# enordber/pepr

Measured on AMD Instinct MI355X. Metric: M site-lnL/sec (WAG+G4 full-tree likelihood evaluations x alignment patterns); the gene-trees/sec half of BASELINE.json's metric is search.gene_trees_per_sec, higher is better.
Workload: dtype f64

## Files before the change

pepr_amd/csrc/api.cpp:

```cpp
#include <algorithm>
#include <cstdlib>
#include <cstring>
#include <memory>
#include <new>
#include <thread>

#include "../../include/peprml.h"
#include "api_types.hpp"

using namespace pml;

static thread_local std::string g_err;

static std::mutex g_fp_mu; static unsigned g_fp_seen[16]; static int g_fp_n = 0;
void pml_fpguard::note(unsigned v) {
    v &= ~0x3Fu;
    std::lock_guard<std::mutex> lk(g_fp_mu);
    for (int i = 0; i < g_fp_n; ++i) if (g_fp_seen[i] == v) return;
    if (g_fp_n < 16) g_fp_seen[g_fp_n++] = v;
}

extern "C" {

const char *pml_version(void) { return "peprml 0.2 (gfx950)"; }
// ... 104 lines not shown
    try { return (expr); }                                                                     \
    catch (const std::bad_alloc &) { return b->owner->c.fail(PML_ENOMEM, "host allocation failed"); } \
    catch (const std::exception &e) { return b->owner->c.fail(PML_EINVAL, e.what()); }

int pml_batch_score(pml_batch *b, double *lnl) {
    if (!b || !lnl) return PML_EINVAL;
    pml_fpguard fpg;
    LOCKED(b);
    GUARD(b->b.score(std::vector<char>(), lnl));
}
int pml_batch_score_stored(pml_batch *b, double *lnl) {
    if (!b || !lnl) return PML_EINVAL;
    pml_fpguard fpg;
    LOCKED(b);
    GUARD(b->b.score(std::vector<char>(), lnl, true));
}
int pml_batch_site_lnl(pml_batch *b, int g, double *out) {
    if (!b || !out || g < 0 || g >= (int)b->b.genes.size()) return PML_EINVAL;
    pml_fpguard fpg;
    LOCKED(b);
    GUARD(b->b.site_lnl(g, out));
}
int pml_batch_set_alpha(pml_batch *b, int g, double alpha) {
    if (!b || g >= (int)b->b.genes.size() || !(alpha > 0)) return PML_EINVAL;
    pml_fpguard fpg;
    LOCKED(b);
    if (g < 0) for (int i = 0; i < (int)b->b.genes.size(); ++i) b->b.set_alpha(i, alpha);
    else b->b.set_alpha(g, alpha);
    return PML_OK;
}
int pml_batch_root_derivs(pml_batch *b, double *lnl, double *d1, double *d2) {
    if (!b || !lnl || !d1 || !d2) return PML_EINVAL;
    pml_fpguard fpg;
    LOCKED(b);
    GUARD(b->b.root_derivs(lnl, d1, d2));
}
int pml_batch_optimize(pml_batch *b, const pml_search_opts *opts, double *lnl, double *alpha) {
    if (!b || !lnl) return PML_EINVAL;
    pml_fpguard fpg;
    LOCKED(b);
    const bool oa = opts ? opts->optimize_alpha != 0 : true;
    const double eps = (opts && opts->epsilon > 0) ? opts->epsilon : 1e-4;
    int rc;
    try { rc = b->b.optimize(oa, eps, lnl); }
    catch (const std::exception &e) { return b->owner->c.fail(PML_EINVAL, e.what()); }
    if (rc) return rc;
    if (alpha) for (size_t g = 0; g < b->b.genes.size(); ++g) alpha[g] = b->b.genes[g].alpha;
    return PML_OK;
}
int pml_batch_search(pml_batch *b, const pml_search_opts *opts, double *lnl, double *alpha) {
    if (!b || !lnl) return PML_EINVAL;
    pml_fpguard fpg;
    LOCKED(b);
    int rc;
    try { rc = opts ? b->b.set_constraints(opts->nconstraints, opts->constraint_ntax, opts->constraint_names, opts->constraint_rows) : 0;
          if (!rc) rc = b->b.search(opts ? opts->nni != 0 : true, opts ? opts->spr_radius : 0,
                           opts ? opts->optimize_alpha != 0 : true,
                           (opts && opts->epsilon > 0) ? opts->epsilon : 1e-3, lnl); }
    catch (const std::exception &e) { return b->owner->c.fail(PML_EINVAL, e.what()); }
    if (rc) return rc;
    if (alpha) for (size_t g = 0; g < b->b.genes.size(); ++g) alpha[g] = b->b.genes[g].alpha;
    return PML_OK;
}
int pml_batch_newick(pml_batch *b, int g, int digits, char **out) {
    if (!b || !out || g < 0 || g >= (int)b->b.genes.size()) return PML_EINVAL;
    pml_fpguard fpg;
    LOCKED(b);
    const Gene &G = b->b.genes[g];
    *out = dup_string(G.tree.newick(G.aln.names, digits));
    return *out ? PML_OK : PML_ENOMEM;
}

enum { OP_SCORE, OP_OPTIMIZE, OP_SEARCH };

static size_t gene_bytes_bound(const pml_alignment &a, bool score_only) {
    const size_t mp = ((size_t)std::max(a.nsites, 1) + 31) / 32 * 32, nt = (size_t)std::max(a.ntax, 3);
    const size_t slots = (score_only ? nt - 2 : 3 * (nt - 2)) + NSCRATCH + MAXTAIL;
    return slots * CLV_ROWS * ((mp + 127) / 128 * 128) * 8 + slots * mp * 4 + nt * mp + 64 * mp + (1 << 16);
}

static int oneshot_on(Ctx &c, int op, int n, const pml_alignment *alns, const char *const *newicks,
                      const pml_model *model, const pml_search_opts *opts, int flags, pml_result *const *out, int share) {
    pml_fpguard fpg;
    std::vector<std::string> pstart; std::vector<const char *> pnw;
    static_assert(sizeof(pml_alignment) == sizeof(pml_alignment_view), "alignment view layout");
    if (op == OP_SEARCH && opts && opts->seed != 0) {
        std::vector<int> idx;
        for (int i = 0; i < n; ++i) if (!newicks || !newicks[i]) idx.push_back(i);
        if (!idx.empty()) {
            std::vector<pml_alignment_view> views;
            for (int i : idx) views.push_back(pml_alignment_view{alns[i].ntax, alns[i].nsites, alns[i].names, alns[i].rows});
            std::vector<Tree> trees; std::vector<EncodedAlignment> enc; std::vector<long long> len; std::vector<int> moves;
            if (int prc = parsimony_batch(&c, (int)idx.size(), views.data(), opts->seed, 20, trees, enc, len, moves)) return prc;
            pstart.resize(n); pnw.assign(n, nullptr);
            for (int i = 0; i < n; ++i) if (newicks && newicks[i]) pnw[i] = newicks[i];
            for (size_t k = 0; k < idx.size(); ++k) { pstart[idx[k]] = trees[k].newick(enc[k].names, 6); pnw[idx[k]] = pstart[idx[k]].c_str(); }
            newicks = pnw.data();
        }
    }
    Batch b;
    struct Drop { Batch &b; ~Drop() { b.destroy(); } } drop{b};
    b.share = share;
    int rc;
    try {
        rc = b.create(&c, n, reinterpret_cast<const pml_alignment_view *>(alns), newicks, model ? model->pi_mode : PML_PI_RAXML_3DP,
                      model ? model->ncat : 4, model ? model->alpha : 1.0, op == OP_SCORE);
        if (rc) return rc;
        std::vector<double> lnl(n);
        if (op == OP_SCORE) rc = b.score(std::vector<char>(), lnl.data());
        else if (op == OP_OPTIMIZE)
            rc = b.optimize(opts ? opts->optimize_alpha != 0 : true, (opts && opts->epsilon > 0) ? opts->epsilon : 1e-4, lnl.data());
        else {
            rc = opts ? b.set_constraints(opts->nconstraints, opts->constraint_ntax, opts->constraint_names, opts->constraint_rows) : 0;
            if (!rc) rc = b.search(opts ? opts->nni != 0 : true, opts ? opts->spr_radius : 0, opts ? opts->optimize_alpha != 0 : true,
                                   (opts && opts->epsilon > 0) ? opts->epsilon : 1e-3, lnl.data());
        }
        for (int i = 0; i < n && !rc; ++i) {
            const Gene &G = b.genes[i];
            pml_result &r = *out[i];
            r.lnl = lnl[i]; r.alpha = G.alpha; r.tree_length = G.tree.length();
            r.npatterns = G.aln.npat; r.nsites = G.aln.nsites;
            r.newick = dup_string(G.tree.newick(G.aln.names, op == OP_SCORE ? 10 : 20));
            if (op == OP_SCORE && (flags & PML_WANT_SITE_LNL)) {
                r.site_lnl = (double *)std::malloc(sizeof(double) * (G.aln.nsites > 0 ? G.aln.nsites : 1));
                if (!r.site_lnl) rc = c.fail(PML_ENOMEM, "host allocation failed");
                else rc = b.site_lnl(i, r.site_lnl);
            }
        }
    } catch (const std::bad_alloc &) { rc = c.fail(PML_ENOMEM, "host allocation failed"); }
    catch (const std::exception &e) { rc = c.fail(PML_EINVAL, e.what()); }
    return rc;
}

static Ctx *worker_ctx(pml_ctx *ctx, int k) {
    while ((int)ctx->workers.size() <= k) {
        std::unique_ptr<Ctx> w(new Ctx());
        if (w->init_worker(ctx->c)) { ctx->c.last_error = w->last_error; return nullptr; }
        ctx->workers.push_back(std::move(w));
    }
    return ctx->workers[k].get();
}
static int search_groups(int n, const pml_alignment *alns) {
    static const int env = std::getenv("PML_GROUPS") ? std::atoi(std::getenv("PML_GROUPS")) : 0;
    int maxcols = 0;
    for (int i = 0; i < n; ++i) maxcols = std::max(maxcols, alns[i].nsites);
    const int tiles = (maxcols + 127) / 128;
    int g = env > 0 ? std::min(env, 8) : 2;
    if (env <= 0) { while (g > 1 && n / g < 32) --g; }
    if (!std::getenv("PML_GROUPS_FORCE")) { while (g > 1 && tiles * g > 32) --g; }
    return std::max(g, 1);
}

static int oneshot_chunk(pml_ctx *ctx, int op, int n, const pml_alignment *alns, const char *const *newicks,
                         const pml_model *model, const pml_search_opts *opts, int flags, pml_result *out) {
    const int G = (op == OP_SEARCH) ? search_groups(n, alns) : 1;
    if (G <= 1) {
        std::vector<pml_result *> outs(n);
        for (int i = 0; i < n; ++i) outs[i] = out + i;
        return oneshot_on(ctx->c, op, n, alns, newicks, model, opts, flags, outs.data(), 1);
    }
    for (int k = 0; k < G; ++k) if (!worker_ctx(ctx, k)) return PML_EDEVICE;
    if (ctx->c.arena_cache) { hipFree(ctx->c.arena_cache); ctx->c.arena_cache = nullptr; ctx->c.arena_cache_bytes = 0; }
    std::vector<int> rcs(G, 0);
    std::vector<std::thread> th;
    for (int k = 0; k < G; ++k) th.emplace_back([&, k]() {
        std::vector<pml_alignment> a; std::vector<const char *> nw; std::vector<pml_result *> outs;
// ... 355 lines not shown
```

pepr_amd/csrc/engine.cpp:

```cpp
#include "engine.hpp"

#include <algorithm>
#include <atomic>
#include <chrono>
#include <cmath>
#include <thread>
#include <cstring>

namespace pml {

#define HIPCHK(expr)                                                                          \
    do {                                                                                      \
        hipError_t e_ = (expr);                                                               \
        if (e_ != hipSuccess)                                                                 \
            return ctx->fail(-5, std::string(#expr) + ": " + hipGetErrorString(e_));          \
    } while (0)

int Ctx::init(int dev, bool prof) {
    Ctx *ctx = this;
    int count = 0;
    if (hipGetDeviceCount(&count) != hipSuccess || count <= 0) return fail(-3, "no HIP device available");
    if (dev < 0 || dev >= count) return fail(-3, "device ordinal out of range");
    device = dev; profile = prof;
    HIPCHK(hipSetDevice(device));
// ... 52 lines not shown
    HIPCHK(hipMalloc((void **)&d_gmodel, n * sizeof(ModelDev)));
    HIPCHK(hipMalloc((void **)&d_geig, n * 2 * PFRAG * sizeof(double)));
    HIPCHK(hipMemcpyAsync(d_gmodel, h.data(), n * sizeof(ModelDev), hipMemcpyHostToDevice, ctx->stream));
    launch_eigfrags_n(d_gmodel, d_geig, (int)n, ctx->stream);
    if (int rc = ctx->sync(ctx->stream)) return rc;
    return 0;
}
int Ctx::ensure_model(int pm) {
    Ctx *ctx = this;
    if (pm == 2) return 0;
    if (pm < 0 || pm > 2) return fail(-1, "bad pi_mode");
    if (model_ready[pm]) return 0;
    model[pm].init(pm);
    ModelDev h;
    fill_model_dev(model[pm], h);
    HIPCHK(hipMalloc(&d_model[pm], sizeof(ModelDev)));
    HIPCHK(hipMalloc(&d_eigfrags[pm], sizeof(double) * 2 * PFRAG));
    HIPCHK(hipMemcpy(d_model[pm], &h, sizeof h, hipMemcpyHostToDevice));
    launch_eigfrags(d_model[pm], d_eigfrags[pm], stream);
    if (int rc = sync(stream)) return rc;
    model_ready[pm] = true;
    return 0;
}
hipEvent_t Ctx::get_event() {
    if (!pool.empty()) { hipEvent_t e = pool.back(); pool.pop_back(); return e; }
    hipEvent_t e; hipEventCreate(&e); return e;
}
void Ctx::tic(int kind, double bytes, double flops) {
    stats[kind].launches++; stats[kind].bytes += bytes; stats[kind].flops += flops;
    if (!profile) return;
    Ev ev{kind, get_event(), get_event()};
    hipEventRecord(ev.a, tic_stream ? tic_stream : stream);
    pending.push_back(ev);
}
void Ctx::toc() {
    if (!profile) return;
    hipEventRecord(pending.back().b, tic_stream ? tic_stream : stream);
}
void Ctx::resolve_events() {
    for (auto &e : pending) {
        float ms = 0;
        if (hipEventElapsedTime(&ms, e.a, e.b) == hipSuccess) stats[e.kind].ms += ms;
        pool.push_back(e.a); pool.push_back(e.b);
    }
    pending.clear();
}

static size_t align_up(size_t x, size_t a) { return (x + a - 1) / a * a; }

struct DetRec { int batch, ntax, npat, nsites, kind, a, b, pad; double x, y, z; };
static std::vector<DetRec> *g_det = nullptr;
static std::mutex g_det_mu;
static bool det_on() {
    static const bool on = [] {
        const char *p = std::getenv("PML_DET_LOG");
        if (!p) return false;
        g_det = new std::vector<DetRec>(); g_det->reserve(1 << 22);
        std::atexit([] {
            const char *q = std::getenv("PML_DET_LOG"); FILE *f = q ? std::fopen(q, "w") : nullptr;
            if (!f) return;
            for (const DetRec &r : *g_det) std::fprintf(f, "B%d g%d_%d_%d %c %d %d %a %a %a\n", r.batch, r.ntax, r.npat, r.nsites, (char)r.kind, r.a, r.b, r.x, r.y, r.z);
            std::fclose(f);
        });
        return true;
    }();
    return on;
}
void det_record(int batch, const Gene &G, char kind, int a, int b, double x, double y, double z) {
    if (!det_on()) return;
    std::lock_guard<std::mutex> lk(g_det_mu);
    g_det->push_back(DetRec{batch, G.aln.ntax, G.aln.npat, G.aln.nsites, kind, a, b, 0, x, y, z});
}
static std::atomic<int> g_batch_id{0};
static double now_ms();

int Batch::create(Ctx *c, int n, const pml_alignment_view *alns, const char *const *newicks, int pm, int nc,
                  double alpha, bool score_only) {
    ctx = c; pi_mode = pm; ncat = nc; score_only_batch = score_only;
    det_id = ++g_batch_id;
    virtual_cherries = std::getenv("PML_NO_CHERRY") == nullptr;
    virtual_pitch = virtual_cherries && std::getenv("PML_NO_PITCH") == nullptr;
    if (n <= 0) return ctx->fail(-1, "empty batch");
    if (nc != 1 && nc != 4) return ctx->fail(-1, "ncat must be 1 or 4");
    if (int rc = ctx->ensure_model(pm)) return rc;
    HIPCHK(hipSetDevice(ctx->device));
    genes.resize(n);
    const double t_create0 = now_ms();
    {
        const int nthreads = std::max(1, std::min({n, 16, (int)std::thread::hardware_concurrency()}));
        std::vector<std::string> errs(n);
        std::atomic<int> next{0};
        auto work = [&]() {
            for (int g = next++; g < n; g = next++) {
                Gene &G = genes[g];
                try {
                    if (!G.aln.encode(alns[g].ntax, alns[g].nsites, alns[g].names, alns[g].rows, errs[g])) continue;
                    if (newicks && newicks[g]) { if (!Tree::parse(newicks[g], G.aln.names, G.tree, errs[g])) continue; }
                    else G.tree = nj_tree(G.aln);
                } catch (const std::exception &e) { errs[g] = e.what(); }
            }
        };
        std::vector<std::thread> pool;
        for (int t = 1; t < nthreads; ++t) pool.emplace_back(work);
        work();
        for (auto &t : pool) t.join();
        for (int g = 0; g < n; ++g) if (!errs[g].empty()) return ctx->fail(-2, "gene " + std::to_string(g) + ": " + errs[g]);
    }
    if (std::getenv("PML_TRACE")) fprintf(stderr, "[pml] create: encode + start trees of %d genes %.1f ms\n", n, now_ms() - t_create0);
    if (int rc = layout(alpha, score_only)) return rc;
    return pm == 2 ? build_gene_models() : 0;
}

int Batch::layout(double alpha, bool score_only) {
    const int n = (int)genes.size();
    size_t total = 0;
    std::vector<size_t> off(n);
    for (int g = 0; g < n; ++g) {
        Gene &G = genes[g];
        const int nt = G.aln.ntax, mp = G.aln.mpad, ndir = 3 * (nt - 2);
        G.slot_cap = score_only ? (nt - 2) : ndir;
        G.slot_of.assign(ndir, -1); G.valid.assign(ndir, 0); G.pend_level.assign(ndir, -1);
        G.mark_all();
        off[g] = total;
        total += align_up((size_t)nt * mp, 256);
        total += align_up((size_t)mp * 8, 256);
        total += (size_t)(G.slot_cap + NSCRATCH) * clv_doubles(mp) * 8;
        total += align_up((size_t)(G.slot_cap + NSCRATCH) * mp * 4, 256);
        total += (size_t)MAXTAIL * clv_doubles(mp) * 8;
        total += (size_t)MAXTAIL * align_up((size_t)mp * 4, 256);
        total += (size_t)MAXTAIL * align_up((size_t)mp * 8, 256);
    }
    arena_bytes = total;
    const double t_alloc0 = now_ms();
    if (ctx->arena_cache && ctx->arena_cache_bytes >= total) {
        arena = ctx->arena_cache; arena_bytes = ctx->arena_cache_bytes;
        ctx->arena_cache = nullptr; ctx->arena_cache_bytes = 0;
    } else {
        if (ctx->arena_cache) { hipFree(ctx->arena_cache); ctx->arena_cache = nullptr; ctx->arena_cache_bytes = 0; }
        if (hipMalloc((void **)&arena, total) != hipSuccess) {
            arena = nullptr;
            return ctx->fail(-4, "device arena of " + std::to_string(total >> 20) + " MiB does not fit");
        }
    }
    if (std::getenv("PML_POISON_ARENA")) HIPCHK(hipMemsetAsync(arena, 0xFF, total, ctx->stream));
    for (int g = 0; g < n; ++g) {
        Gene &G = genes[g];
        const int nt = G.aln.ntax, mp = G.aln.mpad;
        char *p = arena + off[g];
        G.d_codes = (uint8_t *)p; p += align_up((size_t)nt * mp, 256);
        G.d_weight = (double *)p; p += align_up((size_t)mp * 8, 256);
        G.d_clv = (double *)p; p += (size_t)(G.slot_cap + NSCRATCH) * clv_doubles(mp) * 8;
        G.d_scl = (int *)p; p += align_up((size_t)(G.slot_cap + NSCRATCH) * mp * 4, 256);
        for (int k = 0; k < MAXTAIL; ++k) { G.d_sumtab[k] = (double *)p; p += clv_doubles(mp) * 8; }
        for (int k = 0; k < MAXTAIL; ++k) { G.d_sumscl[k] = (int *)p; p += align_up((size_t)mp * 4, 256); }
        for (int k = 0; k < MAXTAIL; ++k) { G.d_patlnl[k] = (double *)p; p += align_up((size_t)mp * 8, 256); }
        if (!G.aln.codes.empty()) {
            HIPCHK(hipMemcpyAsync(G.d_codes, G.aln.codes.data(), (size_t)nt * mp, hipMemcpyHostToDevice, ctx->stream));
            HIPCHK(hipMemcpyAsync(G.d_weight, G.aln.weight.data(), (size_t)mp * 8, hipMemcpyHostToDevice, ctx->stream));
        }
        set_alpha(g, alpha);
    }
    scalars_doubles = (size_t)8 * MAXTAIL * n;
    HIPCHK(hipMalloc((void **)&d_scalars, sizeof(double) * scalars_doubles));
    HIPCHK(hipHostMalloc((void **)&h_scalars, sizeof(double) * scalars_doubles, hipHostMallocDefault));
    std::memset(h_scalars, 0, sizeof(double) * scalars_doubles);
    { if (int rc_ = ctx->sync(ctx->stream)) return rc_; }
    if (std::getenv("PML_TRACE")) fprintf(stderr, "[pml] layout: arena %.1f GiB allocated + uploaded in %.1f ms\n", (double)total / (1 << 30), now_ms() - t_alloc0);
    return 0;
}

void Batch::destroy() {
    if (!ctx) return;
    hipSetDevice(ctx->device);
    if (arena) {
        if (ctx->arena_cache_bytes < arena_bytes) {
            if (ctx->arena_cache) hipFree(ctx->arena_cache);
            ctx->arena_cache = arena; ctx->arena_cache_bytes = arena_bytes;
        } else hipFree(arena);
    }
    if (h_stage) hipHostFree(h_stage);
    if (d_stage) hipFree(d_stage);
    if (d_frags) hipFree(d_frags);
    if (d_nsync) hipFree(d_nsync);
    if (d_nctl) {
        if (std::getenv("PML_TRACE")) {
            NewtonCtl h[2];
            if (hipMemcpy(h, d_nctl, sizeof h, hipMemcpyDeviceToHost) == hipSuccess && h[0].n_requests)
                fprintf(stderr, "[pml] branch Newton: %llu requests, %.2f evaluations each\n", h[0].n_requests, (double)h[0].n_evals / (double)h[0].n_requests);
        }
        hipFree(d_nctl); d_nctl = nullptr;
    }
    if (d_gmodel) { hipFree(d_gmodel); d_gmodel = nullptr; }
    if (d_geig) { hipFree(d_geig); d_geig = nullptr; }
    if (ev_stagger) { hipEventDestroy(ev_stagger); ev_stagger = nullptr; }
    if (d_nsync2) hipFree(d_nsync2);
    if (d_frags2) hipFree(d_frags2);
    d_nsync = d_nsync2 = nullptr; d_frags2 = nullptr; nsync_cap = nsync_cap2 = 0; frag_cap2 = 0;
    if (plan.h) hipHostFree(plan.h);
    if (plan.d) hipFree(plan.d);
    plan = Plan();
    if (h_scalars) hipHostFree(h_scalars);
    if (d_scalars) hipFree(d_scalars);
    if (h_chain) hipHostFree(h_chain);
    if (d_chain) hipFree(d_chain);
    if (d_lenpool) hipFree(d_lenpool);
    if (d_tailpool) { hipFree(d_tailpool); d_tailpool = nullptr; tailpool_cap = 0; }
    if (d_site2pat) { hipFree(d_site2pat); d_site2pat = nullptr; }
    h_chain = d_chain = nullptr; d_lenpool = nullptr; chain_cap = 0;
    arena = nullptr; h_stage = d_stage = nullptr; d_frags = nullptr; d_scalars = h_scalars = nullptr;
}

int GeneStore::create(Ctx *c, int n, const pml_alignment_view *alns) {
    ctx = c;
    HIPCHK(hipSetDevice(ctx->device));
    items.resize(n);
    std::vector<std::string> errs(n);
    std::atomic<int> next{0};
    auto work = [&]() {
        for (int g = next++; g < n; g = next++) {
            try { if (items[g].aln.encode(alns[g].ntax, alns[g].nsites, alns[g].names, alns[g].rows, errs[g])) pair_counts(items[g].aln, items[g].cmp, items[g].diff); }
            catch (const std::exception &e) { errs[g] = e.what(); }
        }
    };
    const int nthreads = std::max(1, std::min({n, 16, (int)std::thread::hardware_concurrency()}));
    std::vector<std::thread> pool;
    for (int t = 1; t < nthreads; ++t) pool.emplace_back(work);
    work();
    for (auto &t : pool) t.join();
    for (int g = 0; g < n; ++g) if (!errs[g].empty()) return ctx->fail(-2, "gene " + std::to_string(g) + ": " + errs[g]);
    size_t total = 0;
    for (auto &it : items) total += align_up((size_t)it.aln.ntax * it.aln.mpad, 256) + align_up((size_t)it.aln.mpad * 8, 256);
    if (hipMalloc((void **)&arena, total) != hipSuccess) { arena = nullptr; return ctx->fail(-4, "gene store does not fit on the device"); }
    char *p = arena;
    for (auto &it : items) {
        it.d_codes = (uint8_t *)p; p += align_up((size_t)it.aln.ntax * it.aln.mpad, 256);
        it.d_w = (double *)p; p += align_up((size_t)it.aln.mpad * 8, 256);
        HIPCHK(hipMemcpyAsync(it.d_codes, it.aln.codes.data(), (size_t)it.aln.ntax * it.aln.mpad, hipMemcpyHostToDevice, ctx->stream));
        HIPCHK(hipMemcpyAsync(it.d_w, it.aln.weight.data(), (size_t)it.aln.mpad * 8, hipMemcpyHostToDevice, ctx->stream));
    }
    { if (int rc_ = ctx->sync(ctx->stream)) return rc_; }
    return 0;
}
void GeneStore::destroy() { if (arena) { hipSetDevice(ctx->device); hipFree(arena); arena = nullptr; } items.clear(); }

int Batch::create_replicates(Ctx *c, const GeneStore &store, const std::vector<std::vector<int>> &sel, int pm, int nc, double alpha) {
    ctx = c; pi_mode = pm; ncat = nc; score_only_batch = false;
    virtual_cherries = std::getenv("PML_NO_CHERRY") == nullptr;
    virtual_pitch = virtual_cherries && std::getenv("PML_NO_PITCH") == nullptr;
    const int n = (int)sel.size();
    if (n <= 0) return ctx->fail(-1, "empty batch");
    if (pm == 2) return ctx->fail(-1, "PROTGAMMAWAGF (empirical frequencies) is built for score / optimize / search calls, not for device-gathered replicates");
    if (int rc = ctx->ensure_model(pm)) return rc;
    HIPCHK(hipSetDevice(ctx->device));
    genes.resize(n);
    struct SegH { int rep, gene, off; size_t rowmap_off; };
    std::vector<SegH> segs; std::vector<int> rowmaps;
    int max_npat = 0;
    for (int r = 0; r < n; ++r) {
        Gene &G = genes[r]; EncodedAlignment &A = G.aln;
        std::vector<std::string> names;
        for (int g : sel[r]) {
            if (g < 0 || g >= (int)store.items.size()) return ctx->fail(-1, "gene index out of range");
            names.insert(names.end(), store.items[g].aln.names.begin(), store.items[g].aln.names.end());
        }
        std::sort(names.begin(), names.end()); names.erase(std::unique(names.begin(), names.end()), names.end());
        const int nt = (int)names.size();
        if (nt < 3) return ctx->fail(-2, "replicate " + std::to_string(r) + ": fewer than 3 taxa");
        A.ntax = nt; A.names = names; A.nsites = 0; A.npat = 0;
        std::vector<int64_t> cmp((size_t)nt * nt, 0), diff((size_t)nt * nt, 0);
        for (int g : sel[r]) {
            const GeneStore::Item &it = store.items[g];
            std::vector<int> local(it.aln.ntax);
            SegH sh{r, g, A.npat, rowmaps.size()};
            rowmaps.resize(rowmaps.size() + nt, -1);
            for (int i = 0; i < it.aln.ntax; ++i) {
                local[i] = (int)(std::lower_bound(names.begin(), names.end(), it.aln.names[i]) - names.begin());
                rowmaps[sh.rowmap_off + local[i]] = i;
            }
            for (int i = 0; i < it.aln.ntax; ++i) for (int j = 0; j < it.aln.ntax; ++j) {
                cmp[(size_t)local[i] * nt + local[j]] += it.cmp[(size_t)i * it.aln.ntax + j]; diff[(size_t)local[i] * nt + local[j]] += it.diff[(size_t)i * it.aln.ntax + j];
            }
            segs.push_back(sh);
            A.npat += it.aln.npat; A.nsites += it.aln.nsites; max_npat = std::max(max_npat, it.aln.npat);
        }
        A.mpad = (A.npat + 31) / 32 * 32;
        G.tree = nj_from_counts(nt, cmp, diff);
    }
    if (int rc = layout(alpha, false)) return rc;
    for (auto &G : genes) {
        HIPCHK(hipMemsetAsync(G.d_codes, NCODES - 1, (size_t)G.aln.ntax * G.aln.mpad, ctx->stream));
        HIPCHK(hipMemsetAsync(G.d_weight, 0, (size_t)G.aln.mpad * 8, ctx->stream));
    }
    std::vector<GatherSeg> hs(segs.size());
    void *d_buf = nullptr;
    const size_t seg_bytes = align_up(hs.size() * sizeof(GatherSeg), 256), map_bytes = rowmaps.size() * sizeof(int);
    HIPCHK(hipMalloc(&d_buf, seg_bytes + map_bytes));
    const int *d_maps = (const int *)((char *)d_buf + seg_bytes);
    for (size_t i = 0; i < segs.size(); ++i) {
        const GeneStore::Item &it = store.items[segs[i].gene]; Gene &G = genes[segs[i].rep];
        hs[i] = GatherSeg{it.d_codes, it.d_w, G.d_codes, G.d_weight, d_maps + segs[i].rowmap_off, it.aln.mpad, it.aln.npat, G.aln.mpad, segs[i].off, G.aln.ntax, 0};
    }
    hipError_t e1 = hipMemcpyAsync(d_buf, hs.data(), hs.size() * sizeof(GatherSeg), hipMemcpyHostToDevice, ctx->stream);
    hipError_t e2 = hipMemcpyAsync((char *)d_buf + seg_bytes, rowmaps.data(), map_bytes, hipMemcpyHostToDevice, ctx->stream);
    if (e1 == hipSuccess && e2 == hipSuccess) launch_gather((const GatherSeg *)d_buf, (int)hs.size(), max_npat, ctx->stream);
    hipError_t e3 = ctx->sync(ctx->stream) ? hipErrorUnknown : hipSuccess;
    hipFree(d_buf);
    if (e1 != hipSuccess || e2 != hipSuccess || e3 != hipSuccess) return ctx->fail(-4, "replicate gather failed");
    return 0;
}

int Batch::fetch_results(bool pooled) {
    HIPCHK(hipMemcpyAsync(h_scalars, d_scalars, sizeof(double) * scalars_doubles, hipMemcpyDeviceToHost, ctx->stream));
    if (pooled && results_used > 0 && d_chain)
        HIPCHK(hipMemcpyAsync(h_chain, d_chain, sizeof(double) * 4 * results_used, hipMemcpyDeviceToHost, ctx->stream));
    return 0;
}
int Batch::chain_sync() {
    if (int rc = flush_deferred()) return rc;
    if (lanes_active) { if (int rc_ = ctx->sync(ctx->stream2)) return rc_; }
    if (int rc = fetch_results(true)) return rc;
    { if (int rc_ = ctx->sync(ctx->stream)) return rc_; }
    { if (int rc_ = ctx->sync(ctx->stream2)) return rc_; }
    HIPCHK(hipGetLastError());
    ctx->resolve_events();
    chain_off = 0;
    return 0;
}
int Batch::ensure_results(size_t nresults) {
    if (nresults > chain_cap) {
        if (h_chain) hipHostFree(h_chain);
        if (d_chain) hipFree(d_chain);
        h_chain = d_chain = nullptr; chain_cap = 0;
        const size_t cap = nresults * 3 / 2 + 64;
        HIPCHK(hipMalloc((void **)&d_chain, cap * 4 * sizeof(double)));
        HIPCHK(hipHostMalloc((void **)&h_chain, cap * 4 * sizeof(double), hipHostMallocDefault));
        chain_cap = cap;
    }
    results_used = nresults;
    return 0;
}
int Batch::ensure_tailpool(size_t bytes) {
    if (bytes <= tailpool_cap) return 0;
    if (d_tailpool) hipFree(d_tailpool);
    d_tailpool = nullptr; tailpool_cap = 0;
    if (hipMalloc((void **)&d_tailpool, bytes) != hipSuccess) { d_tailpool = nullptr; return ctx->fail(-4, "sumtable pool of " + std::to_string(bytes >> 20) + " MiB does not fit"); }
    tailpool_cap = bytes;
    return 0;
}
int Batch::chain_begin(size_t nresults) {
    if (int rc = ensure_results(nresults)) return rc;
    if (!d_lenpool) {
        size_t tot = 0; for (auto &G : genes) tot += (size_t)G.tree.nnodes() * 3;
        HIPCHK(hipMalloc((void **)&d_lenpool, tot * sizeof(double)));
        tot = 0; for (auto &G : genes) { G.d_len = d_lenpool + tot; tot += (size_t)G.tree.nnodes() * 3; }
    }
    for (auto &G : genes) G.len_pending.assign((size_t)G.tree.nnodes() * 3, 0);
    if (int rc = ensure_stage(std::min<size_t>(nresults * 4096 + (1 << 20), (size_t)256 << 20))) return rc;
    chain = true; chain_off = 0; flush_quota = 1;
    return 0;
}
int Batch::ensure_stage(size_t bytes) {
    if (bytes <= h_cap) return 0;
    if (chain) { if (int rc = chain_sync()) return rc; }
    const size_t cap = std::max(bytes * 3 / 2, (size_t)1 << 20);
    if (h_stage) hipHostFree(h_stage);
    if (d_stage) hipFree(d_stage);
    h_stage = d_stage = nullptr; h_cap = d_cap = 0;
    HIPCHK(hipHostMalloc(&h_stage, cap));
    HIPCHK(hipMalloc(&d_stage, cap));
    h_cap = d_cap = cap;
    return 0;
}
int Batch::ensure_frags(size_t sets) {
    double *&fr = lane ? d_frags2 : d_frags; size_t &fc = lane ? frag_cap2 : frag_cap;
    if (sets <= fc) return 0;
    if (chain) { if (int rc = chain_sync()) return rc; }
    const size_t cap = std::max(sets * 5 / 4, (size_t)256);
    if (fr) hipFree(fr);
    fr = nullptr; fc = 0;
    if (!lane) plan.valid = false;
    HIPCHK(hipMalloc((void **)&fr, cap * FRAG_STRIDE * sizeof(double)));
    fc = cap;
    return 0;
}

void Batch::set_alpha(int g, double a) {
    Gene &G = genes[g];
    a = std::min(std::max(a, ALPHA_MIN), ALPHA_MAX);
    G.alpha = a;
    if (ncat == 1) { for (double &r : G.rates) r = 1.0; }
    else gamma_rates(a, NCAT, G.rates);
    ++G.rates_epoch;
    invalidate_all(g);
}
void Batch::invalidate_all(int g) {
    Gene &G = genes[g];
    std::fill(G.valid.begin(), G.valid.end(), 0);
    if (G.slot_cap < (int)G.slot_of.size()) { std::fill(G.slot_of.begin(), G.slot_of.end(), -1); G.next_slot = 0; }
}
static void invalidate_from(Gene &G, int v, int from) {
    std::vector<std::pair<int, int>> st{{v, from}};
    const int nt = G.aln.ntax;
    while (!st.empty()) {
        auto [x, f] = st.back(); st.pop_back();
        if (x < nt) continue;
        for (int k = 0; k < 3; ++k) {
            const int w = G.tree.nbr[x][k];
            if (w == f || w < 0) continue;
            G.valid[(x - nt) * 3 + k] = 0;
            st.push_back({w, x});
        }
    }
}
void Batch::branch_changed(int g, int a, int b) {
    invalidate_from(genes[g], a, b); invalidate_from(genes[g], b, a);
}
int Batch::slot_for(Gene &G, int idx) {
    int s = G.slot_of[idx];
    if (s < 0) { if (G.next_slot >= G.slot_cap) return -1; s = G.slot_of[idx] = G.next_slot++; }
    return s;
}

bool Batch::is_cherry(int g, int node, int toward) const {
    const Gene &G = genes[g];
    const int nt = G.aln.ntax;
    if (!virtual_cherries || node < nt) return false;
    for (int k = 0; k < 3; ++k) { const int w = G.tree.nbr[node][k]; if (w != toward && w >= nt) return false; }
    return true;
}
int Batch::virt_kind(int g, int node, int toward) const {
    if (is_cherry(g, node, toward)) return 1;
    if (!virtual_pitch) return 0;
    const Gene &G = genes[g];
    const int nt = G.aln.ntax;
    if (node < nt) return 0;
    int ntip = 0, inner = -1;
    for (int k = 0; k < 3; ++k) { const int w = G.tree.nbr[node][k]; if (w == toward) continue; if (w < nt) ++ntip; else inner = w; }
    return (ntip == 1 && inner >= 0 && is_cherry(g, inner, node)) ? 2 : 0;
}
Side Batch::msg(int g, int node, int toward) const {
    const Gene &G = genes[g];
    if (node < G.aln.ntax) return {SIDE_TIP, node};
    const int idx = (node - G.aln.ntax) * 3 + G.tree.slot(node, toward);
    const int vk = virt_kind(g, node, toward);
    return {vk == 1 ? SIDE_CHERRY : (vk == 2 ? SIDE_PITCH : SIDE_MSG), idx};
}

int Batch::need(int g, int v, int to, std::vector<PendingOp> &ops) {
    Gene &G = genes[g];
    const int nt = G.aln.ntax;
    if (v < nt || virt_kind(g, v, to)) return 0;
    {
        const int idx0 = (v - nt) * 3 + G.tree.slot(v, to);
        if (G.valid[idx0]) return 0;
        if (G.pend_level[idx0] >= 0) return G.pend_level[idx0];
    }
    struct Frame { int v, to, k, stage, lv[2]; };
    std::vector<Frame> st;
    st.reserve(64);
    st.push_back({v, to, G.tree.slot(v, to), 0, {0, 0}});
    int ret = 0;
    while (!st.empty()) {
        Frame &f = st.back();
        const int idx = (f.v - nt) * 3 + f.k;
        if (f.stage == 0) {
            if (G.valid[idx]) { ret = 0; st.pop_back(); continue; }
            if (G.pend_level[idx] >= 0) { ret = G.pend_level[idx]; st.pop_back(); continue; }
        }
        int ch[2], ci = 0;
        for (int q = 0; q < 3; ++q) if (q != f.k) ch[ci++] = G.tree.nbr[f.v][q];
        if (f.stage >= 1) f.lv[f.stage - 1] = ret;
        if (f.stage < 2) {
            const int c = ch[f.stage];
            f.stage++;
            if (c < nt || virt_kind(g, c, f.v)) { ret = 0; continue; }
            const int fv = f.v;
            st.push_back({c, fv, G.tree.slot(c, fv), 0, {0, 0}});
            continue;
        }
        const int lvl = std::max(f.lv[0], f.lv[1]) + 1;
        PendingOp op; op.gene = g; op.out_kind = SIDE_MSG; op.out_id = idx; op.level = lvl; ci = 0;
        for (int q = 0; q < 3; ++q) if (q != f.k) { op.child[ci] = msg(g, G.tree.nbr[f.v][q], f.v); op.t[ci] = G.tree.len[f.v][q]; ci++; }
        ops.push_back(op);
        G.pend_level[idx] = lvl;
        ret = lvl;
        st.pop_back();
    }
    return ret;
}

static double now_ms() {
    return std::chrono::duration<double, std::milli>(std::chrono::steady_clock::now().time_since_epoch()).count();
}

void Batch::newton_gave_up() {
    ++ctx->newton_giveups;
    if (std::getenv("PML_TRACE") && d_nctl) {
        NewtonCtl h[2];
        if (hipMemcpy(h, d_nctl, sizeof h, hipMemcpyDeviceToHost) == hipSuccess)
            fprintf(stderr, "[pml] k_newton exchange gave up: slice %d of %d, evaluation %d, arrived mask %08x%08x, tickets taken in its partition %d, (left * 1024 + partition) %d; tickets %d %d done %d %d oticket %d %d %d %d %d %d %d %d odone %d\n",
                    h[0].dbg[1], h[0].dbg[2], h[0].dbg[3], (unsigned)h[0].dbg[5], (unsigned)h[0].dbg[4], (unsigned)h[0].dbg[6], h[0].dbg[7], h[0].ticket[0], h[0].ticket[1], h[0].done[0], h[0].done[1],
                    h[0].oticket[0], h[0].oticket[1], h[0].oticket[2], h[0].oticket[3], h[0].oticket[4], h[0].oticket[5], h[0].oticket[6], h[0].oticket[7], h[0].odone);
        hipMemset(&d_nctl[0].dbg[0], 0, sizeof(int));
    }
    safe_left = safe_hold; safe_hold = std::min(safe_hold * 2, 1024);
}
int Batch::clear_abort() {
    if (!d_nctl) return 0;
    for (int l = 0; l < 2; ++l) HIPCHK(hipMemsetAsync(&d_nctl[l].abort, 0, sizeof(int), l ? ctx->stream2 : ctx->stream));
    { if (int rc_ = ctx->sync(ctx->stream2)) return rc_; }
    { if (int rc_ = ctx->sync(ctx->stream)) return rc_; }
    return 0;
}

int Batch::flush_deferred() {
    if (deferred.empty()) return 0;
    struct Guard { Batch *b; ~Guard() { b->deferred.clear(); b->ctx->tic_stream = nullptr; } } guard{this};
    const size_t lo = deferred.front().base, hi = deferred.back().base + deferred.back().bytes;
    const hipStream_t cs = deferred.front().lane ? ctx->stream2 : ctx->stream;
    HIPCHK(hipMemcpyAsync((char *)d_stage + lo, (char *)h_stage + lo, hi - lo, hipMemcpyHostToDevice, cs));
    const ModelDev *md = pi_mode < 2 ? ctx->d_model[pi_mode] : nullptr;
    static const bool serialize = std::getenv("PML_SERIALIZE") != nullptr;
#define PML_SER() do { if (serialize) hipStreamSynchronize(st); } while (0)
    if (serialize) hipStreamSynchronize(cs);
    for (const Deferred &L : deferred) {
        const hipStream_t st = L.lane ? ctx->stream2 : ctx->stream;
        double *const frags_buf = L.lane ? d_frags2 : d_frags;
        char *ds = (char *)d_stage + L.base;
        ctx->tic_stream = st;
        if (L.nreq) {
            ctx->tic(K_PMAT, (double)L.nreq * PFRAG * 8);
            launch_pmat(md, (const PmatReq *)(ds + L.o_req), frags_buf, (int)L.nreq, st, d_gmodel != nullptr);
            ctx->toc(); PML_SER();
        }
        if (L.nruns) {
            ctx->tic(K_NEWVIEW, L.algo_bytes, L.algo_flops);
            launch_oplist((const NvOp *)(ds + L.o_ops), (const GeneRun *)(ds + L.o_runs), (int)L.nruns, L.max_mpad, L.any_pitch, L.any_chain, st, L.fused ? d_nctl + L.lane : nullptr);
            ctx->toc(); PML_SER();
        }
        if (L.stagger) hipEventRecord(ev_stagger, st);
        if (L.neval) {
            ctx->tic(K_REDUCE, 0);
            launch_reduce((const ReduceReq *)(ds + L.o_red), (int)L.neval, st);
            ctx->toc(); PML_SER();
        }
        if (L.nt_reg + L.nt_stream > 0) {
            ctx->tic(K_NEWTON, L.newton_bytes);
            if (L.seq) { launch_newton_seq(md, (const NewtonReq *)(ds + L.o_newt), (const int *)(ds + L.o_tick), L.nt_reg, L.nt_stream, d_nctl + L.lane, st); ++ctx->newton_seq_launches; }
            else launch_newton(md, (const NewtonReq *)(ds + L.o_newt), (const int *)(ds + L.o_tick), L.nt_reg, L.nt_stream, d_nctl + L.lane, st);
            ctx->toc(); PML_SER();
        }
        ctx->tic_stream = nullptr;
        if (hipError_t e = hipGetLastError(); e != hipSuccess) return ctx->fail(-5, std::string("kernel launch: ") + hipGetErrorString(e));
    }
#undef PML_SER
    static const size_t flush_max = std::getenv("PML_FLUSH_MAX") ? (size_t)std::atoi(std::getenv("PML_FLUSH_MAX")) : 8;
    flush_quota = std::min<size_t>(flush_quota * 2, flush_max);
    return 0;
}

int Batch::run(std::vector<PendingOp> &ops, const std::vector<Tail> &tails) {
    const double t_begin = now_ms();
    HIPCHK(hipSetDevice(ctx->device));
    std::stable_sort(ops.begin(), ops.end(), [](const PendingOp &a, const PendingOp &b) { return a.gene != b.gene ? a.gene < b.gene : a.part < b.part; });
    const size_t nops = ops.size(), ntail = tails.size();
    size_t neval = 0, nnewton = 0;
    for (auto &t : tails) { if (t.mode == MODE_EVALUATE) neval++; else if (t.mode != MODE_EVALUATE_CAT) nnewton++; }
    size_t nreq_max = 10 * nops + 9 * ntail;
    {
        std::vector<char> seen(genes.size(), 0);
        size_t keyed = 0, loose = 0;
        for (auto &o : ops) { if (!seen[o.gene]) { seen[o.gene] = 1; keyed += 5 * (size_t)genes[o.gene].aln.ntax; }
                              if (o.out_kind != SIDE_MSG) loose += (o.bv[0] < 0) + (o.bv[1] < 0); }
        for (auto &t : tails) { if (!seen[t.gene]) { seen[t.gene] = 1; keyed += 5 * (size_t)genes[t.gene].aln.ntax; }
                                if (t.mode >= MODE_EVALUATE && t.bv < 0) loose += 1; }
        nreq_max = std::min(nreq_max, keyed + loose);
    }
    bool any_pitch = false, any_chain = false;
    if (int rc = ensure_frags(std::max(nreq_max, (size_t)1))) return rc;
    double *&nsync_buf = lane ? d_nsync2 : d_nsync; size_t &nsync_c = lane ? nsync_cap2 : nsync_cap;
    if (nnewton > nsync_c) {
        if (chain) { if (int rc = chain_sync()) return rc; }
        if (nsync_buf) hipFree(nsync_buf);
        nsync_buf = nullptr; nsync_c = 0;
        const size_t cap = std::max(nnewton * 2, (size_t)256);
        HIPCHK(hipMalloc((void **)&nsync_buf, cap * NEWTON_SYNC_DOUBLES * sizeof(double)));
        HIPCHK(hipMemsetAsync(nsync_buf, 0, cap * NEWTON_SYNC_DOUBLES * sizeof(double), ctx->stream));
        { if (int rc_ = ctx->sync(ctx->stream)) return rc_; }
        nsync_c = cap;
    }
    if (nnewton && !d_nctl) {
        HIPCHK(hipMalloc((void **)&d_nctl, 2 * sizeof(NewtonCtl)));
        HIPCHK(hipMemsetAsync(d_nctl, 0, 2 * sizeof(NewtonCtl), ctx->stream));
        { if (int rc_ = ctx->sync(ctx->stream)) return rc_; }
    }
    const hipStream_t st = lane ? ctx->stream2 : ctx->stream;
    double *const frags_buf = lane ? d_frags2 : d_frags;
    ctx->tic_stream = st;
    const size_t ngenes = genes.size();
    std::vector<int> &nparts = run_nparts; nparts.assign(ngenes, 1);
    for (auto &o : ops) nparts[o.gene] = std::max(nparts[o.gene], o.part + 1);
    for (auto &t : tails) nparts[t.gene] = std::max(nparts[t.gene], t.part + 1);
    std::vector<size_t> &koff = run_koff; koff.assign(ngenes + 1, 0);
    for (size_t g = 0; g < ngenes; ++g) koff[g + 1] = koff[g] + (size_t)nparts[g];
    const size_t nkeys = koff[ngenes];
    const size_t o_req = 0;
    const size_t o_ops = align_up(o_req + nreq_max * sizeof(PmatReq), 256);
    const size_t o_runs = align_up(o_ops + (nops + ntail) * sizeof(NvOp), 256);
    const size_t o_red = align_up(o_runs + nkeys * sizeof(GeneRun), 256);
    const size_t o_newt = align_up(o_red + neval * sizeof(ReduceReq), 256);
    size_t ntick_max = 0;
    for (auto &t : tails) if (t.mode == MODE_SUMTABLE) ntick_max += (size_t)newton_split(genes[t.gene].aln.mpad);
    const size_t o_tick = align_up(o_newt + nnewton * sizeof(NewtonReq), 256);
    const size_t bytes = align_up(o_tick + ntick_max * sizeof(int), 256);
    if (chain && chain_off + bytes > h_cap) { if (int rc = chain_sync()) return rc; }
    if (int rc = ensure_stage(bytes)) return rc;
    const size_t base = chain ? chain_off : 0;
    if (chain) chain_off += bytes;
    char *hs = (char *)h_stage + base, *ds = (char *)d_stage + base;
    PmatReq *hreq = (PmatReq *)(hs + o_req);
    NvOp *hops = (NvOp *)(hs + o_ops);
    GeneRun *hruns = (GeneRun *)(hs + o_runs);
    ReduceReq *hred = (ReduceReq *)(hs + o_red);
    NewtonReq *hnewt = (NewtonReq *)(hs + o_newt);
    int *htick = (int *)(hs + o_tick);
    if (nnewton) ++newton_launch_seq;
    const unsigned tag_base = (newton_launch_seq & 0x3FFFFFu) << 10;
    static const bool fuse_env = std::getenv("PML_NO_FUSE") == nullptr && !(std::getenv("PML_CHAIN") && std::atoi(std::getenv("PML_CHAIN")) == 0);
    bool fuse_ok = fuse_env && !newton_safe_mode();
    if (fuse_ok && nnewton && !fuse_big_genes()) {
        int mm = 0; size_t nr = 0;
        std::vector<char> seen(genes.size(), 0);
        for (auto &o : ops) if (!seen[o.gene]) { seen[o.gene] = 1; nr += (size_t)nparts[o.gene]; mm = std::max(mm, genes[o.gene].aln.mpad); }
        for (auto &t : tails) if (!seen[t.gene]) { seen[t.gene] = 1; nr += (size_t)nparts[t.gene]; mm = std::max(mm, genes[t.gene].aln.mpad); }
        const size_t bpg = (size_t)(mm + TILE_PAT - 1) / TILE_PAT;
        if (bpg > 32 && nr * bpg > (size_t)fused_oplist_capacity()) fuse_ok = false;
    }
    std::vector<char> fused_req(nnewton, 0);
    bool any_fused = false;
    std::vector<int> tail_req(ntail, -1);

    size_t nout = 0, nruns = 0, ie = 0, in = 0, ireq = 0, iop = 0;
    last_src.clear();
    int max_mpad = 0, newton_maxm = 0;
    double algo_bytes = 0, algo_flops = 0;
    bool req_ok = req_off.size() == genes.size() + 1;
    for (size_t g = 0; req_ok && g < genes.size(); ++g) req_ok = req_off[g + 1] - req_off[g] == (size_t)9 * genes[g].tree.nnodes();
    if (!req_ok) {
        req_off.assign(genes.size() + 1, 0);
        for (size_t g = 0; g < genes.size(); ++g) req_off[g + 1] = req_off[g] + (size_t)3 * 3 * genes[g].tree.nnodes();
        req_stamp.assign(req_off.back(), 0); req_ptr.assign(req_off.back(), nullptr); req_launch = 0;
        val_bucket.assign(genes.size() * 3, {}); val_stamp.assign(genes.size() * 3, 0);
    }
    if (++req_launch == 0) {
        std::fill(req_stamp.begin(), req_stamp.end(), 0u); std::fill(val_stamp.begin(), val_stamp.end(), 0u); req_launch = 1;
    }
    bool req_overflow = false;
    auto add_req = [&](size_t g, double t, int kind, int v, int q) -> const double * {
        uint64_t tbits = 0; size_t key = 0;
        std::vector<std::pair<uint64_t, const double *>> *bucket = nullptr;
        if (!record_plan) {
            if (v >= 0) {
                const Tree &T = genes[g].tree;
                const int w = T.nbr[v][q], a = v * 3 + q, b = w * 3 + T.slot(w, v);
                key = req_off[g] + (size_t)kind * 3 * T.nnodes() + (size_t)std::min(a, b);
                if (req_stamp[key] == req_launch) return req_ptr[key];
            } else {
                std::memcpy(&tbits, &t, 8);
                const size_t bi = g * 3 + (size_t)kind;
                if (val_stamp[bi] != req_launch) { val_bucket[bi].clear(); val_stamp[bi] = req_launch; }
                bucket = &val_bucket[bi];
                for (auto &e : *bucket) if (e.first == tbits) return e.second;
            }
        }
        if (ireq >= nreq_max) { req_overflow = true; return frags_buf; }
        PmatReq &r = hreq[ireq];
        r.t = t; std::memcpy(r.rates, genes[g].rates, sizeof r.rates); r.kind = kind; r.pad = 0;
        r.tp = (chain && v >= 0 && genes[g].len_pending[(size_t)v * 3 + q]) ? genes[g].d_len + (size_t)v * 3 + q : nullptr;
        r.md = d_gmodel ? d_gmodel + g : nullptr;
        last_src.push_back({(int)g, v, q, kind});
        const double *out = frags_buf + (ireq++) * FRAG_STRIDE;
        if (!record_plan) { if (v >= 0) { req_stamp[key] = req_launch; req_ptr[key] = out; } else bucket->push_back({tbits, out}); }
        return out;
    };
    struct Resolved { OpSide s; int kind; const int *scl; double bytes; double flops = 0; bool inner = true; };
    auto resolve = [&](size_t g, const Side &sd, Resolved &R) -> int {
        Gene &G = genes[g];
        const int mp = G.aln.mpad, nt = G.aln.ntax;
        R.s = OpSide{nullptr, nullptr, nullptr, nullptr, nullptr, nullptr, nullptr}; R.scl = nullptr;
        R.flops = 0; R.inner = true;
        if (sd.kind == SIDE_TIP) { R.kind = SK_TIP; R.s.p0 = G.d_codes + (size_t)sd.id * mp; R.bytes = 1; R.inner = false; return 0; }
        if (sd.kind == SIDE_CHERRY) {
            const int v = nt + sd.id / 3, k = sd.id % 3;
            int tips[2], qs[2], ci = 0;
            for (int q = 0; q < 3; ++q) if (q != k) { tips[ci] = G.tree.nbr[v][q]; qs[ci] = q; ++ci; }
            R.kind = SK_CHERRY;
            R.s.p0 = G.d_codes + (size_t)tips[0] * mp; R.s.p1 = G.d_codes + (size_t)tips[1] * mp;
            R.s.t0 = add_req(g, G.tree.len[v][qs[0]], PM_TIPTABLE, v, qs[0]);
            R.s.t1 = add_req(g, G.tree.len[v][qs[1]], PM_TIPTABLE, v, qs[1]);
            R.bytes = 640 + 642;
            R.flops = 80;
            return 0;
        }
        if (sd.kind == SIDE_PITCH) {
            const int X = nt + sd.id / 3, k = sd.id % 3;
            int qc = -1, qC = -1;
            for (int q = 0; q < 3; ++q) if (q != k) { if (G.tree.nbr[X][q] < nt) qc = q; else qC = q; }
            const int C = G.tree.nbr[X][qC], kC = G.tree.slot(C, X);
            int tips[2], qs[2], ci = 0;
            for (int q = 0; q < 3; ++q) if (q != kC) { tips[ci] = G.tree.nbr[C][q]; qs[ci] = q; ++ci; }
            R.kind = SK_PITCH;
            R.s.p0 = G.d_codes + (size_t)tips[0] * mp; R.s.p1 = G.d_codes + (size_t)tips[1] * mp;
            R.s.p2 = G.d_codes + (size_t)G.tree.nbr[X][qc] * mp;
            R.s.t0 = add_req(g, G.tree.len[C][qs[0]], PM_TIPTABLE, C, qs[0]);
            R.s.t1 = add_req(g, G.tree.len[C][qs[1]], PM_TIPTABLE, C, qs[1]);
            R.s.t2 = add_req(g, G.tree.len[X][qc], PM_TIPTABLE, X, qc);
            R.s.f = add_req(g, G.tree.len[X][qC], PM_FRAGS, X, qC);
            any_pitch = true;
            R.bytes = 640 + (640 + 642) + 1 + 640;
            R.flops = 80 + 3280;
            return 0;
        }
        const int slot = sd.kind == SIDE_MSG ? G.slot_of[sd.id] : G.slot_cap + sd.id;
        if (slot < 0) return -1;
        R.kind = SK_CLV; R.s.p0 = G.d_clv + (size_t)slot * clv_doubles(mp); R.scl = G.d_scl + (size_t)slot * mp; R.bytes = 640;
        return 0;
    };

    std::vector<std::vector<int>> &tails_of = run_tails_of;
    if (tails_of.size() < nkeys) tails_of.resize(nkeys);
    for (auto &v : tails_of) v.clear();
    for (size_t i = 0; i < ntail; ++i) {
        if (tails[i].slot < 0 || tails[i].slot >= MAXTAIL) return ctx->fail(-1, "internal: bad tail slot");
        tails_of[koff[tails[i].gene] + (size_t)tails[i].part].push_back((int)i);
    }
    for (size_t g = 0; g < ngenes; ++g) for (int part = 0; part < nparts[g]; ++part) {
        const size_t key = koff[g] + (size_t)part;
        const bool has_ops = iop < nops && ops[iop].gene == (int)g && ops[iop].part == part;
        if (!has_ops && tails_of[key].empty()) continue;
        Gene &G = genes[g];
        const int mp = G.aln.mpad;
        GeneRun &run = hruns[nruns++];
        run.op_begin = (int)nout;
        max_mpad = std::max(max_mpad, mp);
        static const int chain_env = std::getenv("PML_CHAIN") ? std::atoi(std::getenv("PML_CHAIN")) : 2;
        const bool chain_reads = chain_env == 2 || (chain_env == 1 && record_plan), chain_nostore = chain_env >= 1 && record_plan && !record_stored;
        long last_nv = -1, last_nv_op = -1;
        auto chained_from = [&](const Side &sd, int kind) {
            return chain_reads && last_nv >= 0 && kind == SK_CLV && sd.kind == ops[last_nv_op].out_kind && sd.id == ops[last_nv_op].out_id;
        };
        auto consume_last = [&]() {
            any_chain = true;
            if (chain_nostore || ops[last_nv_op].transient) { hops[last_nv].flags |= OPF_NO_STORE; ops[last_nv_op].unstored = true; }
        };
        auto emit_tail = [&](const Tail &t) -> int {
            NvOp &d = hops[nout++];
            std::memset(&d, 0, sizeof d);
            Resolved L, R;
            if (resolve(g, t.a, L) || resolve(g, t.b, R)) return ctx->fail(-5, "internal: tail message has no slot");
            d.l = L.s; d.r = R.s; d.l_scl = L.scl; d.r_scl = R.scl;
            d.flags = L.kind | (R.kind << 2); d.mpad = mp; d.mode = t.mode;
            if (chained_from(t.a, L.kind)) { d.flags |= OPF_CHAIN_L; consume_last(); }
            else if (t.mode >= MODE_EVALUATE && chained_from(t.b, R.kind)) { d.flags |= OPF_CHAIN_R; consume_last(); }
            double *result = t.result_dev ? t.result_dev : d_scalars + 8 * (g * MAXTAIL + t.slot);
            if (t.mode == MODE_EVALUATE_CAT) {
                if (!t.patlnl_dev || !t.scl_dev) return ctx->fail(-1, "internal: table slice missing");
                d.pl = d.pr = add_req(g, t.t0, PM_FRAGS_PI, t.bv, t.bq);
                d.out = t.patlnl_dev; d.out_scl = t.scl_dev;
                algo_bytes += (double)G.aln.npat * (L.bytes + R.bytes + 36);
                algo_flops += (double)G.aln.npat * (3360 + L.flops + R.flops);
            } else if (t.mode == MODE_EVALUATE) {
                d.pl = d.pr = add_req(g, t.t0, PM_FRAGS_PI, t.bv, t.bq);
                double *pl = t.patlnl_dev ? t.patlnl_dev : G.d_patlnl[t.slot];
                d.out = pl; d.out_scl = nullptr;
                ReduceReq &rr = hred[ie++];
                rr.patlnl = pl; rr.weight = G.d_weight; rr.out = result; rr.mpad = mp; rr.pad = 0;
                algo_bytes += (double)G.aln.npat * (L.bytes + R.bytes + 8);
                algo_flops += (double)G.aln.npat * (3360 + L.flops + R.flops);
            } else {
                d.pl = eig_of((int)g); d.pr = d.pl + PFRAG;
                double *stab = t.sumtab_dev ? t.sumtab_dev : G.d_sumtab[t.slot];
                int *sscl = t.sumtab_dev ? reinterpret_cast<int *>(t.sumtab_dev + clv_doubles(mp)) : G.d_sumscl[t.slot];
                d.out = stab; d.out_scl = sscl;
                NewtonReq &nr = hnewt[in];
                nr.md = model_of((int)g); nr.tag_base = tag_base; nr.pad0 = 0;
                static const bool fuse_multi = !(std::getenv("PML_FUSE_MULTI") && std::atoi(std::getenv("PML_FUSE_MULTI")) == 0);
                if (fuse_ok && (fuse_multi || (tails_of[key].size() == 1 && t.after < 0)) && !t.patlnl_dev && newton_reg_form(mp)) {
                    d.flags |= OPF_FUSED_NEWTON; d.aux = (const NewtonReq *)(ds + o_newt) + in;
                    fused_req[in] = 1; any_fused = true; any_chain = true;
                }
                last_nv = -1; last_nv_op = -1;
                tail_req[&t - tails.data()] = (int)in;
                nr.ticket0 = 0; nr.pad = 0;
                nr.sumtab = stab; nr.weight = G.d_weight; nr.scl = sscl;
                std::memcpy(nr.rates, G.rates, sizeof nr.rates);
                nr.t0 = t.t0; nr.tol = newton_tol; nr.out = result; nr.mpad = mp; nr.max_iter = t.max_iter;
                nr.t_dev0 = t.t_dev0; nr.t_dev1 = t.t_dev1; nr.patlnl = t.patlnl_dev;
                nr.sync = nsync_buf + (size_t)in * NEWTON_SYNC_DOUBLES; newton_maxm = std::max(newton_maxm, mp);
                algo_bytes += (double)G.aln.npat * (L.bytes + R.bytes + 640);
                algo_flops += (double)G.aln.npat * (6480 + L.flops + R.flops);
                in++;
            }
            return 0;
        };
        size_t ti = 0; int emitted = 0;
        auto flush_tails = [&](bool all) -> int {
            while (ti < tails_of[key].size()) {
                const Tail &t = tails[tails_of[key][ti]];
                if (!all && (t.after < 0 || t.after > emitted)) break;
                if (int rc = emit_tail(t)) return rc;
                ++ti;
            }
            return 0;
        };
        if (int rc = flush_tails(false)) return rc;
        for (; iop < nops && ops[iop].gene == (int)g && ops[iop].part == part; ++iop) {
            PendingOp &o = ops[iop];
            const int s = o.out_kind == SIDE_MSG ? slot_for(G, o.out_id) : G.slot_cap + o.out_id;
            if (s < 0) return ctx->fail(-4, "CLV slots exhausted (score-only batch used for a multi-root request)");
            NvOp &d = hops[nout++];
            std::memset(&d, 0, sizeof d);
            d.mode = MODE_NEWVIEW;
            d.out = G.d_clv + (size_t)s * clv_doubles(mp);
            d.out_scl = G.d_scl + (size_t)s * mp;
            Resolved S[2];
            if (resolve(g, o.child[0], S[0]) || resolve(g, o.child[1], S[1])) return ctx->fail(-5, "internal: child message has no slot");
            d.mpad = mp;
            d.flags = S[0].kind | (S[1].kind << 2);
            const double *pm[2];
            for (int c = 0; c < 2; ++c) {
                int bv = o.bv[c], bq = o.bq[c];
                if (o.out_kind == SIDE_MSG) {
                    bv = G.aln.ntax + o.out_id / 3; const int k = o.out_id % 3;
                    int seen = 0;
                    for (bq = 0; bq < 3; ++bq) if (bq != k) { if (seen == c) break; ++seen; }
                }
                pm[c] = add_req(g, o.t[c], PM_FRAGS, bv, bq);
            }
            Side ch[2] = {o.child[0], o.child[1]};
            if (chained_from(ch[1], S[1].kind)) { std::swap(S[0], S[1]); std::swap(pm[0], pm[1]); std::swap(ch[0], ch[1]); }
            d.flags = S[0].kind | (S[1].kind << 2);
            if (chained_from(ch[0], S[0].kind)) { d.flags |= OPF_CHAIN_L; consume_last(); }
            d.l = S[0].s; d.r = S[1].s; d.l_scl = S[0].scl; d.r_scl = S[1].scl; d.pl = pm[0]; d.pr = pm[1];
            algo_bytes += (double)G.aln.npat * (S[0].bytes + S[1].bytes + 640);
            algo_flops += (double)G.aln.npat * ((S[0].inner && S[1].inner ? 6480 : (S[0].inner || S[1].inner ? 3280 : 80)) + S[0].flops + S[1].flops);
            last_nv = (long)nout - 1; last_nv_op = (long)iop;
            ++emitted;
            if (int rc = flush_tails(false)) return rc;
        }
        if (int rc = flush_tails(true)) return rc;
        run.op_end = (int)nout;
        static const int nt_policy = std::getenv("PML_NT_STORE") ? std::atoi(std::getenv("PML_NT_STORE")) : 1;
        const bool small_gene = mp <= 16 * TILE_PAT;
        for (int i = run.op_begin; i < run.op_end; ++i) {
            NvOp &d = hops[i];
            if (d.mode != MODE_NEWVIEW || nt_policy == 0 || (nt_policy == 1 && !small_gene)) continue;
            bool next_reads = false;
            if (nt_policy == 3 && i + 1 < run.op_end) {
                const NvOp &nx = hops[i + 1];
                next_reads = ((nx.flags & 3) == SK_CLV && nx.l.p0 == d.out) || (((nx.flags >> 2) & 3) == SK_CLV && nx.r.p0 == d.out);
            }
            if (!next_reads) d.flags |= OPF_NT_STORE;
        }
    }

    if (req_overflow) return ctx->fail(-5, "internal: transition-matrix request bound exceeded");
    int nt_reg = 0, nt_stream = 0;
    const bool seq_launch = nnewton > 0 && newton_safe_mode();
    {
        int cur = 0;
        for (int pass = 0; pass < 2; ++pass) {
            for (size_t i = 0; i < nnewton; ++i) {
                if (fused_req[i] || newton_reg_form(hnewt[i].mpad) != (pass == 0)) continue;
                const int S = seq_launch ? 1 : newton_split(hnewt[i].mpad);
                hnewt[i].ticket0 = cur - (pass == 0 ? 0 : nt_reg);
                for (int k = 0; k < S; ++k) htick[cur++] = (int)i;
            }
            if (pass == 0) nt_reg = cur; else nt_stream = cur - nt_reg;
        }
        if (nnewton && safe_left > 0 && !safe_now) --safe_left;
    }
    double newton_bytes = 0;
    for (size_t i = 0; i < ntail; ++i) if (tails[i].mode == MODE_SUMTABLE && !fused_req[tail_req[i]]) newton_bytes += (double)genes[tails[i].gene].aln.npat * 640;
    Deferred L;
    L.base = base; L.bytes = bytes; L.o_req = o_req; L.o_ops = o_ops; L.o_runs = o_runs; L.o_red = o_red; L.o_newt = o_newt;
    L.o_tick = o_tick; L.nt_reg = nt_reg; L.nt_stream = nt_stream; L.seq = seq_launch; L.fused = any_fused;
    L.nreq = ireq; L.nruns = nruns; L.neval = neval; L.nnewton = nnewton; L.max_mpad = max_mpad; L.newton_maxm = newton_maxm;
    L.any_pitch = any_pitch; L.any_chain = any_chain; L.algo_bytes = algo_bytes; L.algo_flops = algo_flops; L.newton_bytes = newton_bytes; L.lane = lane; L.stagger = record_stagger;
    record_stagger = false;
    deferred.push_back(L);
    const bool defer = chain && !lanes_active;
    if (!defer || deferred.size() >= flush_quota) { if (int rc = flush_deferred()) return rc; }
    ctx->tic_stream = nullptr;
    const double t_launched = now_ms();
    ctx->stats[K_HOST_BUILD].launches++; ctx->stats[K_HOST_BUILD].ms += t_launched - t_begin;
    if (!chain) {
        bool pooled = false;
        for (auto &t : tails) pooled = pooled || t.result_host != nullptr;
        if (int rc = fetch_results(pooled)) return rc;
        { if (int rc_ = ctx->sync(ctx->stream)) return rc_; }
        HIPCHK(hipGetLastError());
        const double t_done = now_ms();
        ctx->stats[K_HOST_WAIT].launches++; ctx->stats[K_HOST_WAIT].ms += t_done - t_launched;
        host_phase_ms[HP_RUN_SYNCED] += t_launched - t_begin;
        ctx->resolve_events();
        auto result_of = [&](const Tail &t) { return t.result_host ? t.result_host : (t.result_dev ? (const double *)nullptr : res(t.gene, t.slot)); };
        std::vector<int> bad;
        for (size_t i = 0; i < ntail; ++i) {
            const Tail &t = tails[i];
            if (t.mode != MODE_SUMTABLE) continue;
            const double *h = result_of(t);
            if (h && !std::isfinite(h[1])) bad.push_back(tail_req[i]);
        }
        bool bad_fused = false;
        for (int i : bad) bad_fused = bad_fused || fused_req[i];
        if (bad_fused && !in_retry) {
            newton_gave_up(); ctx->newton_reissued += (long long)bad.size();
            if (int rc = clear_abort()) return rc;
            for (auto &o : ops) { o.unstored = false; if (o.out_kind == SIDE_MSG) genes[o.gene].pend_level[o.out_id] = -1; }
            in_retry = true;
            const int rc = run(ops, tails);
            in_retry = false;
            return rc;
        }
        if (!bad.empty() && !seq_launch && !bad_fused) {
            newton_gave_up(); ctx->newton_reissued += (long long)bad.size();
            int nr = 0, ns = 0;
            for (int pass = 0; pass < 2; ++pass) for (int i : bad) if (newton_reg_form(hnewt[i].mpad) == (pass == 0)) { htick[nr + ns] = i; ++(pass == 0 ? nr : ns); }
            if (int rc = clear_abort()) return rc;
            HIPCHK(hipMemcpyAsync(ds + o_tick, hs + o_tick, bad.size() * sizeof(int), hipMemcpyHostToDevice, ctx->stream));
            launch_newton_seq(nullptr, (const NewtonReq *)(ds + o_newt), (const int *)(ds + o_tick), nr, ns, d_nctl + lane, ctx->stream);
            ++ctx->newton_seq_launches;
            if (int rc = fetch_results(pooled)) return rc;
            { if (int rc_ = ctx->sync(ctx->stream)) return rc_; }
            HIPCHK(hipGetLastError());
        }
        for (auto &t : tails) {
            if (t.mode == MODE_EVALUATE_CAT) continue;
            const double *h = result_of(t);
#ifndef ABL_KEEP_GOING
            if (h && !std::isfinite(t.mode == MODE_EVALUATE ? h[0] : h[1]))
                return ctx->fail(-5, t.mode == MODE_EVALUATE ? "device returned a non-finite likelihood" : "k_newton: non-finite branch likelihood (also from the no-exchange form)");
#endif
        }
    }
    for (auto &o : ops) if (o.out_kind == SIDE_MSG) { Gene &G = genes[o.gene]; G.valid[o.out_id] = o.unstored ? 0 : 1; G.pend_level[o.out_id] = -1; }
    if (record_plan) {
        record_plan = false;
        Plan &P = plan;
        if (P.bytes < bytes) {
            if (P.h) hipHostFree(P.h);
            if (P.d) hipFree(P.d);
            P.h = P.d = nullptr; P.bytes = 0;
            HIPCHK(hipHostMalloc(&P.h, bytes)); HIPCHK(hipMalloc(&P.d, bytes)); P.bytes = bytes;
        }
        std::memcpy(P.h, hs, bytes);
        HIPCHK(hipMemcpyAsync(P.d, ds, bytes, hipMemcpyDeviceToDevice, ctx->stream));
        P.o_req = o_req; P.o_ops = o_ops; P.o_runs = o_runs; P.o_red = o_red;
        P.nreq = ireq; P.nruns = nruns; P.neval = neval; P.max_mpad = max_mpad; P.algo_bytes = algo_bytes; P.algo_flops = algo_flops; P.stored = record_stored; P.any_pitch = any_pitch; P.any_chain = any_chain;
        P.rates_seen.resize(genes.size()); for (size_t g = 0; g < genes.size(); ++g) P.rates_seen[g] = genes[g].rates_epoch;
        P.src = last_src; P.outs.clear();
        for (auto &o : ops) if (o.out_kind == SIDE_MSG && !o.unstored) P.outs.push_back({o.gene, o.out_id});
        P.epoch = topo_epoch; P.valid = true;
    }
    return 0;
}

int Batch::replay_plan(double *lnl) {
    const double t_begin = now_ms();
    Plan &P = plan;
    HIPCHK(hipSetDevice(ctx->device));
    PmatReq *hreq = (PmatReq *)((char *)P.h + P.o_req);
    std::vector<char> moved(genes.size(), 0);
// ... 46 lines not shown
        const int r = G.tree.nbr[0][0];
        need(g, r, 0, ops);
        tails.push_back({g, msg(g, 0, r), msg(g, r, 0), MODE_EVALUATE, G.tree.len[0][0], 0, 0, -1, 0, 0});
    }
    if (int rc = run(ops, tails)) return rc;
    for (auto &t : tails) lnl[t.gene] = res(t.gene)[0];
    for (auto &t : tails) det_record(det_id, genes[t.gene], 'E', 0, 0, lnl[t.gene], genes[t.gene].alpha, 0);
    return 0;
}
int Batch::score(const std::vector<char> &active, double *lnl, bool stored) {
    for (int g = 0; g < (int)genes.size(); ++g) if (active.empty() || active[g]) invalidate_all(g);
    bool all = true;
    for (char a : active) all = all && a;
    if (all && !score_only_batch) {
        if (plan.valid && plan.epoch == topo_epoch && plan.stored == stored) return replay_plan(lnl);
        record_plan = true; record_stored = stored;
    }
    const int rc = evaluate(active, lnl);
    record_plan = false; record_stored = false;
    return rc;
}
int Batch::site_lnl(int g, double *out) {
    Gene &G = genes[g];
    if ((int)G.aln.site2pat.size() != G.aln.nsites) return ctx->fail(-1, "per-site lnL is not available for device-gathered replicates");
    std::vector<char> act(genes.size(), 0); act[g] = 1;
    std::vector<double> l(genes.size());
    if (int rc = evaluate(act, l.data())) return rc;
    std::vector<double> pat(G.aln.mpad);
    HIPCHK(hipMemcpy(pat.data(), G.d_patlnl[0], sizeof(double) * G.aln.mpad, hipMemcpyDeviceToHost));
    for (int s = 0; s < G.aln.nsites; ++s) out[s] = pat[G.aln.site2pat[s]];
    return 0;
}
int Batch::root_derivs(double *lnl, double *d1, double *d2) {
    std::vector<PendingOp> ops; std::vector<Tail> tails;
    for (int g = 0; g < (int)genes.size(); ++g) {
        Gene &G = genes[g];
        const int r = G.tree.nbr[0][0];
        need(g, r, 0, ops);
        tails.push_back({g, msg(g, 0, r), msg(g, r, 0), MODE_SUMTABLE, G.tree.len[0][0], 0});
    }
    if (int rc = run(ops, tails)) return rc;
    for (int g = 0; g < (int)genes.size(); ++g) { lnl[g] = res(g)[1]; d1[g] = res(g)[2]; d2[g] = res(g)[3]; }
    return 0;
}

int Batch::smooth_pass(const std::vector<char> &active, std::vector<double> &maxdelta, double thr) {
    const int n = (int)genes.size();
    maxdelta.assign(n, 0.0);
    struct SafeOff { bool &f; ~SafeOff() { f = false; } } safe_off{safe_now};
    double hp_t = now_ms();
    std::vector<std::vector<std::pair<int, int>>> &order = pass_order;
    std::vector<std::vector<uint8_t>> &next = pass_next;
    if ((int)order.size() != n) { order.assign(n, {}); next.assign(n, {}); }
    size_t maxlen = 0;
    struct F { int v, from, k; };
    std::vector<F> st; st.reserve(256);
    for (int g = 0; g < n; ++g) {
        order[g].clear();
        if (!active[g]) { next[g].clear(); continue; }
        Gene &G = genes[g];
        const Tree &T = G.tree; const int nt = T.ntax;
        if (G.dirty.size() != (size_t)T.nnodes() * 3) G.mark_all();
        next[g].assign((size_t)T.nnodes() * 3, 0);
        st.clear(); st.push_back({0, -1, 0});
        while (!st.empty()) {
            F &f = st.back();
            if (f.k >= 3) { st.pop_back(); continue; }
            const int k = f.k, w = T.nbr[f.v][k]; f.k++;
            if (w < 0 || w == f.from) continue;
            if (G.dirty[f.v * 3 + k]) order[g].push_back({f.v, w});
            if (w >= nt) { const int fv = f.v; st.push_back({w, fv, 0}); }
        }
        maxlen = std::max(maxlen, order[g].size());
    }
    ++cnt_passes;
    host_phase_ms[HP_PASS_SETUP] += now_ms() - hp_t; hp_t = now_ms();
    static const bool no_chain = std::getenv("PML_NO_CHAIN") != nullptr;
    size_t nres = 0; for (int g = 0; g < n; ++g) nres += order[g].size();
    struct Done { int gene, v, w; double old; size_t idx; };
    std::vector<Done> done; done.reserve(nres);
    for (int attempt = 0; attempt < 2; ++attempt) {
    done.clear();
    if (!no_chain) { if (int rc = chain_begin(nres)) return rc; }
    auto fail_out = [&](int rc) { if (chain) { chain_sync(); chain = false; } return rc; };
    static const bool lanes_on = std::getenv("PML_LANES") != nullptr;
    int nact = 0; for (int g = 0; g < n; ++g) nact += active[g] && !order[g].empty();
    const bool two_lanes = chain && lanes_on && nact >= 16;
    lanes_active = two_lanes;
    for (size_t step = 0; step < maxlen; ++step) {
        ++cnt_smooth;
        const size_t first = done.size();
        for (int ln = 0; ln < (two_lanes ? 2 : 1); ++ln) {
            std::vector<PendingOp> ops; std::vector<Tail> tails;
            for (int g = 0; g < n; ++g) {
                if (!active[g] || step >= order[g].size()) continue;
                if (two_lanes && (g & 1) != ln) continue;
                auto [v, w] = order[g][step];
                Gene &G = genes[g];
                need(g, v, w, ops); need(g, w, v, ops);
                Tail t{g, msg(g, v, w), msg(g, w, v), MODE_SUMTABLE, G.tree.len[v][G.tree.slot(v, w)], 32};
                if (chain) {
                    t.result_dev = d_chain + 4 * done.size();
                    t.t_dev0 = G.d_len + (size_t)v * 3 + G.tree.slot(v, w); t.t_dev1 = G.d_len + (size_t)w * 3 + G.tree.slot(w, v);
                }
                done.push_back({g, v, w, t.t0, done.size()});
                tails.push_back(t);
            }
            if (tails.empty()) continue;
            lane = ln;
            if (two_lanes && step == 0) {
                if (!ev_stagger) hipEventCreateWithFlags(&ev_stagger, hipEventDisableTiming);
                if (ln == 0) record_stagger = true;
                else hipStreamWaitEvent(ctx->stream2, ev_stagger, 0);
            }
            const int rc = run(ops, tails);
            lane = 0;
            if (rc) return fail_out(rc);
        }
        if (chain) {
            for (size_t i = first; i < done.size(); ++i) {
                Gene &G = genes[done[i].gene]; const int v = done[i].v, w = done[i].w;
                G.len_pending[(size_t)v * 3 + G.tree.slot(v, w)] = 1; G.len_pending[(size_t)w * 3 + G.tree.slot(w, v)] = 1;
                branch_changed(done[i].gene, v, w);
            }
        } else {
            for (size_t i = first; i < done.size(); ++i) {
                Gene &G = genes[done[i].gene]; const int v = done[i].v, w = done[i].w;
                const double nl = res(done[i].gene)[0], old = done[i].old, dl = std::fabs(nl - old);
                maxdelta[done[i].gene] = std::max(maxdelta[done[i].gene], dl);
                if (nl != old) { G.tree.set_len(v, w, nl); branch_changed(done[i].gene, v, w); }
                if (dl > thr) { std::swap(G.dirty, next[done[i].gene]); G.mark_node(v); G.mark_node(w); std::swap(G.dirty, next[done[i].gene]); }
            }
        }
    }
    host_phase_ms[HP_PASS_STEPS] += now_ms() - hp_t;
    if (chain) {
        const double t0 = now_ms();
        if (int rc = chain_sync()) { chain = false; return rc; }
        ctx->stats[K_HOST_WAIT].launches++; ctx->stats[K_HOST_WAIT].ms += now_ms() - t0;
        host_phase_ms[HP_PASS_SYNC] += now_ms() - t0; hp_t = now_ms();
        chain = false; lanes_active = false;
        bool gave_up = false;
        for (auto &d : done) gave_up = gave_up || !std::isfinite(h_chain[4 * d.idx + 1]);
        if (gave_up) {
            if (attempt == 1 || safe_now) return ctx->fail(-5, "k_newton: non-finite branch likelihood (also from the no-exchange form)");
            newton_gave_up(); ctx->newton_reissued += (long long)done.size();
            if (int rc = clear_abort()) return rc;
            for (int g = 0; g < n; ++g) if (active[g]) { std::fill(genes[g].len_pending.begin(), genes[g].len_pending.end(), 0); invalidate_all(g); }
            safe_now = true;
            continue;
        }
        for (auto &d : done) {
            Gene &G = genes[d.gene];
            const double nl = h_chain[4 * d.idx], dl = std::fabs(nl - d.old);
            det_record(det_id, G, 'S', d.v, d.w, d.old, nl, h_chain[4 * d.idx + 1]);
            maxdelta[d.gene] = std::max(maxdelta[d.gene], dl);
            G.tree.set_len(d.v, d.w, nl);
            if (dl > thr) { std::swap(G.dirty, next[d.gene]); G.mark_node(d.v); G.mark_node(d.w); std::swap(G.dirty, next[d.gene]); }
        }
        for (auto &G : genes) std::fill(G.len_pending.begin(), G.len_pending.end(), 0);
    }
    break;
    }
    safe_now = false;
    for (int g = 0; g < n; ++g) if (active[g]) genes[g].dirty.swap(next[g]);
    host_phase_ms[HP_PASS_POST] += now_ms() - hp_t;
    return 0;
}

int Batch::gamma20(std::vector<double> &lnl20, std::vector<double> &alpha20, std::vector<double> &rescale20) {
    const int n = (int)genes.size();
    HIPCHK(hipSetDevice(ctx->device));
    double rates[G20_RATES]; g20_rates(rates);
    std::vector<size_t> off(n); size_t bytes = 0;
    for (int g = 0; g < n; ++g) { off[g] = bytes; bytes += align_up((size_t)genes[g].aln.mpad * (G20_RATES * 8 + (G20_RATES / 4) * 4), 256); }
    if (int rc = ensure_tailpool(bytes)) return rc;
    auto table = [&](int g) { return reinterpret_cast<double *>(d_tailpool + off[g]); };
    auto counts = [&](int g) { return reinterpret_cast<int *>(d_tailpool + off[g] + (size_t)genes[g].aln.mpad * G20_RATES * 8); };
    struct RatesBack { Batch *b; ~RatesBack() { for (int g = 0; g < (int)b->genes.size(); ++g) b->set_alpha(g, b->genes[g].alpha); } };
    for (int j = 0; j < G20_RATES / 4; ++j) {
        RatesBack back{this};
        std::vector<PendingOp> ops; std::vector<Tail> tails;
        for (int g = 0; g < n; ++g) {
            Gene &G = genes[g];
            for (int c = 0; c < 4; ++c) G.rates[c] = rates[4 * j + c];
            ++G.rates_epoch; invalidate_all(g);
            const int r = G.tree.nbr[0][0];
            need(g, r, 0, ops);
            Tail t{g, msg(g, 0, r), msg(g, r, 0), MODE_EVALUATE_CAT, G.tree.len[0][0], 0, 0, -1, 0, 0};
            t.patlnl_dev = table(g) + (size_t)4 * j * G.aln.mpad; t.scl_dev = counts(g) + (size_t)j * G.aln.mpad;
            tails.push_back(t);
        }
        if (int rc = run(ops, tails)) return rc;
    }
    if (int rc = ensure_results((size_t)n)) return rc;
    if (int rc = ensure_stage((size_t)n * sizeof(G20Req))) return rc;
    std::vector<double> la(n, 0.0), lm(n, 0.0), f(n, 0.0);
    auto objective = [&](const std::vector<char> &act) -> int {
        G20Req *h = (G20Req *)h_stage; int k = 0;
        std::vector<int> who;
        for (int g = 0; g < n; ++g) {
            if (!act[g]) continue;
            G20Req &r = h[k++];
            r.table = table(g); r.cnt = counts(g); r.weight = genes[g].d_weight; r.out = d_chain + 4 * g; r.patlnl = nullptr;
            r.mpad = genes[g].aln.mpad; r.pad = 0;
            g20_weights(std::exp(la[g]), std::exp(lm[g]), r.w);
            who.push_back(g);
        }
        if (!k) return 0;
        HIPCHK(hipMemcpyAsync(d_stage, h_stage, (size_t)k * sizeof(G20Req), hipMemcpyHostToDevice, ctx->stream));
        launch_g20((const G20Req *)d_stage, k, ctx->stream);
        results_used = (size_t)n;
        if (int rc = fetch_results(true)) return rc;
        { if (int rc_ = ctx->sync(ctx->stream)) return rc_; }
        HIPCHK(hipGetLastError());
        for (int g : who) { f[g] = -h_chain[4 * g]; if (!std::isfinite(f[g])) return ctx->fail(-5, "device returned a non-finite Gamma20 likelihood"); }
        return 0;
    };
    std::vector<char> all(n, 1), active(n, 1);
    if (int rc = objective(all)) return rc;
    const double LO = std::log(0.01), HI = std::log(10.0), TOL = 1e-3;
    for (int round = 0; round < 10; ++round) {
        bool any = false; for (char a : active) any |= a;
        if (!any) break;
// ... 100 lines not shown
```

pepr_amd/csrc/engine.hpp:

```cpp
#pragma once
#include <hip/hip_runtime.h>

#include <mutex>
#include <string>
#include <vector>

#include "host.hpp"
#include "kernels.h"

namespace pml {

constexpr int MAXTAIL = 4;

enum { K_PMAT = 0, K_NEWVIEW = 1, K_EVALUATE = 2, K_SUMTABLE = 3, K_NEWTON = 4, K_REDUCE = 5, K_HOST_BUILD = 6, K_HOST_WAIT = 7, K_COUNT = 8 };

struct Ctx {
    int device = 0;
    bool profile = false;
    hipStream_t stream = nullptr;
    hipStream_t stream2 = nullptr;
    std::mutex mu;
    std::string last_error;
    Model model[2];
    bool model_ready[2] = {false, false};
    ModelDev *d_model[2] = {nullptr, nullptr};
    double *d_eigfrags[2] = {nullptr, nullptr};
    struct KStat { long long launches = 0; double ms = 0; double bytes = 0; double flops = 0; } stats[K_COUNT];
    long long newton_giveups = 0, newton_reissued = 0, newton_seq_launches = 0;
    struct Ev { int kind; hipEvent_t a, b; };
    std::vector<Ev> pending;
    std::vector<hipEvent_t> pool;
    char *arena_cache = nullptr; size_t arena_cache_bytes = 0;

    int init(int dev, bool prof);
    int init_worker(const Ctx &parent);
    bool owns_stream = true;
    hipEvent_t ev_sync = nullptr;
    int sync(hipStream_t s);
    void destroy();
    int ensure_model(int pi_mode);
    hipEvent_t get_event();
    hipStream_t tic_stream = nullptr;
    void tic(int kind, double bytes, double flops = 0);
    void toc();
    void resolve_events();
    int fail(int code, const std::string &msg) { last_error = msg; return code; }
};

struct Gene {
    EncodedAlignment aln;
    Tree tree;
    double alpha = 1.0;
    double rates[NCAT] = {1, 1, 1, 1};
    unsigned rates_epoch = 0;
    uint8_t *d_codes = nullptr;
    double *d_weight = nullptr;
    double *d_clv = nullptr;
    int *d_scl = nullptr;
    double *d_sumtab[MAXTAIL] = {};
    int *d_sumscl[MAXTAIL] = {};
    double *d_patlnl[MAXTAIL] = {};
    int slot_cap = 0, next_slot = 0;
    std::vector<int> slot_of;
    std::vector<uint8_t> valid;
    std::vector<int> pend_level;
    std::vector<Constraint> cons;
    std::vector<uint8_t> dirty;
    double *d_len = nullptr;
    std::vector<uint8_t> len_pending;
    void mark_node(int v) { for (int k = 0; k < 3; ++k) { const int w = tree.nbr[v][k]; if (w < 0) continue; dirty[v * 3 + k] = 1; dirty[w * 3 + tree.slot(w, v)] = 1; } }
    void mark_all() { dirty.assign((size_t)tree.nnodes() * 3, 1); }
    void mark_none() { dirty.assign((size_t)tree.nnodes() * 3, 0); }
};

void det_record(int batch, const Gene &G, char kind, int a, int b, double x, double y, double z);

struct pml_alignment_view { int ntax, nsites; const char *const *names; const char *const *rows; };

struct GeneStore {
    struct Item { EncodedAlignment aln; std::vector<int64_t> cmp, diff; uint8_t *d_codes = nullptr; double *d_w = nullptr; };
    Ctx *ctx = nullptr; std::vector<Item> items; char *arena = nullptr;
    int create(Ctx *c, int n, const pml_alignment_view *alns);
    void destroy();
};

constexpr int NNI_PARTS = 6;
constexpr int NSCRATCH = 4 * NNI_PARTS > 8 ? 4 * NNI_PARTS : 8;
enum { SIDE_TIP = 0, SIDE_MSG = 1, SIDE_SCRATCH = 2, SIDE_CHERRY = 3, SIDE_PITCH = 4 };
struct Side { int kind, id; };
struct PendingOp { int gene, out_kind, out_id, level; Side child[2]; double t[2]; int bv[2] = {-1, -1}, bq[2] = {0, 0};
                   bool unstored = false;
                   bool transient = false;
                   int part = 0;  };

struct Batch {
    Ctx *ctx = nullptr;
    int pi_mode = 0, ncat = 4, det_id = 0;
    ModelDev *d_gmodel = nullptr; double *d_geig = nullptr;
    const ModelDev *model_of(int g) const { return d_gmodel ? d_gmodel + g : ctx->d_model[pi_mode]; }
    const double *eig_of(int g) const { return d_geig ? d_geig + (size_t)g * 2 * PFRAG : ctx->d_eigfrags[pi_mode]; }
    int build_gene_models();
    int share = 1;
    double newton_tol = 1e-8;
    std::vector<Gene> genes;
    char *arena = nullptr; size_t arena_bytes = 0;
    void *h_stage = nullptr; size_t h_cap = 0;
    void *d_stage = nullptr; size_t d_cap = 0;
    double *d_frags = nullptr; size_t frag_cap = 0;
    double *d_frags2 = nullptr; size_t frag_cap2 = 0;
    double *d_nsync2 = nullptr; size_t nsync_cap2 = 0;
    int lane = 0;
    hipEvent_t ev_stagger = nullptr; bool record_stagger = false;
    double *d_scalars = nullptr; double *h_scalars = nullptr;
    size_t scalars_doubles = 0, results_used = 0;
    int fetch_results(bool pooled);
    double *d_nsync = nullptr; size_t nsync_cap = 0;
    NewtonCtl *d_nctl = nullptr;
    int safe_left = 0, safe_hold = 4; bool safe_now = false;
    unsigned newton_launch_seq = 0;
    bool in_retry = false;
    bool newton_safe_mode() { return safe_now || safe_left > 0; }
    void newton_gave_up();
    int clear_abort();
    struct ReqSrc { int gene, v, q, fold; };
    struct Plan {
        bool valid = false; unsigned epoch = 0;
        void *h = nullptr, *d = nullptr; size_t bytes = 0;
        size_t o_req = 0, o_ops = 0, o_runs = 0, o_red = 0, nreq = 0, nruns = 0, neval = 0;
        int max_mpad = 0; double algo_bytes = 0, algo_flops = 0; bool any_pitch = false, any_chain = false;
        bool stored = false;
        std::vector<ReqSrc> src; std::vector<std::pair<int, int>> outs;
        std::vector<unsigned> rates_seen;
    } plan;
    long cnt_smooth = 0, cnt_nni = 0, cnt_spr = 0, cnt_eval = 0, cnt_passes = 0;
    enum { HP_PASS_SETUP, HP_PASS_STEPS, HP_PASS_SYNC, HP_PASS_POST, HP_NNI_BUILD, HP_NNI_RUN, HP_NNI_SELECT, HP_ALPHA_HOST, HP_RUN_SYNCED, HP_N };
    double host_phase_ms[HP_N] = {0};
    unsigned topo_epoch = 0;
    bool score_only_batch = false;
    int replay_plan(double *lnl);
    bool record_plan = false, record_stored = false;
    std::vector<ReqSrc> last_src;
    std::vector<size_t> req_off; std::vector<uint32_t> req_stamp; std::vector<const double *> req_ptr; uint32_t req_launch = 0;
    std::vector<std::vector<int>> run_tails_of; std::vector<int> run_nparts; std::vector<size_t> run_koff;
    std::vector<std::vector<std::pair<int, int>>> pass_order; std::vector<std::vector<uint8_t>> pass_next;
    std::vector<std::vector<std::pair<uint64_t, const double *>>> val_bucket; std::vector<uint32_t> val_stamp;
    bool chain = false; size_t chain_off = 0;
    double *d_lenpool = nullptr;
    double *d_chain = nullptr, *h_chain = nullptr; size_t chain_cap = 0;
    struct Deferred { size_t base, bytes, o_req, o_ops, o_runs, o_red, o_newt, o_tick, nreq, nruns, neval, nnewton; int nt_reg, nt_stream; bool seq, fused;
                      int max_mpad, newton_maxm, lane; bool any_pitch, any_chain, stagger; double algo_bytes, newton_bytes, algo_flops; };
    std::vector<Deferred> deferred; size_t flush_quota = 1; bool lanes_active = false;
    int flush_deferred();
    int chain_begin(size_t nresults);
    int ensure_results(size_t nresults);
    char *d_tailpool = nullptr; size_t tailpool_cap = 0;
    int ensure_tailpool(size_t bytes);
    int chain_sync();

    int create(Ctx *c, int n, const pml_alignment_view *alns, const char *const *newicks,
               int pi_mode, int ncat, double alpha, bool score_only);
    int create_replicates(Ctx *c, const GeneStore &store, const std::vector<std::vector<int>> &sel, int pi_mode, int ncat, double alpha);
    int layout(double alpha, bool score_only);
    void destroy();

    void set_alpha(int g, double alpha);
    void invalidate_all(int g);
    void branch_changed(int g, int a, int b);
    int evaluate(const std::vector<char> &active, double *lnl);
    int score(const std::vector<char> &active, double *lnl, bool stored = false);
    int site_lnl(int g, double *out);
    int root_derivs(double *lnl, double *d1, double *d2);
    int smooth_pass(const std::vector<char> &active, std::vector<double> &maxdelta, double thr);
    int opt_alpha(const std::vector<char> &active, double *lnl, double tol = 1e-4);
    int optimize(bool opt_alpha_flag, double eps, double *lnl, const std::vector<char> *mask = nullptr);
    int light_smooth(const std::vector<char> &active, double *lnl);
    int nni_round(const std::vector<char> &active, std::vector<double> &lnl, std::vector<int> &applied);
    int spr_round(const std::vector<char> &active, int radius, std::vector<double> &lnl, std::vector<int> &moves);
    int search(bool nni, int spr_radius, bool opt_alpha_flag, double eps, double *lnl);
    int gamma20(std::vector<double> &lnl20, std::vector<double> &alpha20, std::vector<double> &rescale20);
    int sh_support(int nboot, unsigned long long seed, std::vector<std::vector<double>> &support, std::vector<std::vector<std::pair<int, int>>> &edges_out);
    int *d_site2pat = nullptr; std::vector<size_t> site2pat_off;
    int set_constraints(int ncons, int ntax, const char *const *names, const char *const *rows);

    int need(int g, int v, int to, std::vector<PendingOp> &ops);
    struct Tail { int gene; Side a, b; int mode; double t0; int max_iter; int slot = 0; int after = -1;
                  int bv = -1, bq = 0;
                  double *result_dev = nullptr;
                  double *t_dev0 = nullptr, *t_dev1 = nullptr;
                  double *patlnl_dev = nullptr;
                  double *sumtab_dev = nullptr;
                  int *scl_dev = nullptr;
                  const double *result_host = nullptr;
                  int part = 0;                                };
    double *res(int g, int slot = 0) const { return h_scalars + 8 * ((size_t)g * MAXTAIL + slot); }
    Side msg(int g, int node, int toward) const;
    bool is_cherry(int g, int node, int toward) const;
    int virt_kind(int g, int node, int toward) const;
    bool virtual_pitch = true;
    bool virtual_cherries = true;
    int run(std::vector<PendingOp> &ops, const std::vector<Tail> &tails);
    int ensure_stage(size_t bytes);
    int ensure_frags(size_t sets);
    int slot_for(Gene &g, int idx);
};

int parsimony_batch(Ctx *ctx, int n, const pml_alignment_view *alns, unsigned seed, int radius, std::vector<Tree> &trees_out,
                    std::vector<EncodedAlignment> &alns_out, std::vector<long long> &lengths_out, std::vector<int> &moves_out);

}
```

pepr_amd/csrc/kernels.h:

```cpp
#pragma once
#include <hip/hip_runtime.h>
#include <cstdint>

namespace pml {

constexpr int NS = 20;
constexpr int NCAT = 4;
constexpr int CLV_ROWS = NCAT * NS;
constexpr int PFRAG = NCAT * 25 * 16;
constexpr int PAT_PER_WAVE = 32;
constexpr int TILE_PAT = 128;
constexpr size_t clv_doubles(int mpad) { return (size_t)((mpad + TILE_PAT - 1) / TILE_PAT) * TILE_PAT * (NCAT * NS); }
constexpr size_t clv_index(int row, int p) { return ((size_t)(p >> 7) * (NCAT * NS) + (size_t)row) * TILE_PAT + (size_t)(p & (TILE_PAT - 1)); }
constexpr int NCODES = 23;
constexpr int TIPTAB_KK = 6;
constexpr int TIPTAB_DOUBLES = NCAT * NCODES * 4 * TIPTAB_KK;
constexpr int FRAG_STRIDE = TIPTAB_DOUBLES;

struct ModelDev {
    double eval[NS];
    double U[NS * NS];
    double Uinv[NS * NS];
    double pi[NS];
    double UinvT[NS * NS];
};

struct PmatReq {
    double t;
    double rates[NCAT];
    int kind;
    int pad;
    const double *tp;
    const ModelDev *md;
};
enum { PM_FRAGS = 0, PM_FRAGS_PI = 1, PM_TIPTABLE = 2 };

enum { SK_CLV = 0, SK_TIP = 1, SK_CHERRY = 2, SK_PITCH = 3 };
constexpr int OPF_NT_STORE = 16;
constexpr int OPF_CHAIN_L = 32, OPF_CHAIN_R = 64, OPF_NO_STORE = 128;
constexpr int OPF_FUSED_NEWTON = 256;
struct OpSide {
    const void *p0, *p1, *p2;
    const double *t0, *t1, *t2;
    const double *f;
};

struct NvOp {
    double *out;
    OpSide l, r;
    int *out_scl;
    const int *l_scl;
    const int *r_scl;
    const double *pl;
    const double *pr;
    int mpad;
    int flags;
    int mode;
    int pad;
    const void *aux;
};
static_assert(sizeof(NvOp) == 184, "NvOp layout");

struct GeneRun {
    int op_begin, op_end;
};

struct ReduceReq {
    const double *patlnl;
    const double *weight;
    double *out;
    int mpad;
    int pad;
};

struct NewtonReq {
    const double *sumtab;
    const double *weight;
    const int *scl;
    double rates[NCAT];
    double t0;
    double tol;
    double *out;
    double *sync;
    const ModelDev *md;
    unsigned tag_base;
    unsigned pad0;
    double *t_dev0, *t_dev1;
    double *patlnl;
    int mpad;
    int max_iter;
    int ticket0;
    int pad;
};
constexpr int NEWTON_MAX_SPLIT = 64;
constexpr int NEWTON_SLICE_PAT = 128;
__host__ __device__ constexpr int newton_split(int mpad) { return (mpad + NEWTON_SLICE_PAT - 1) / NEWTON_SLICE_PAT < NEWTON_MAX_SPLIT ? ((mpad + NEWTON_SLICE_PAT - 1) / NEWTON_SLICE_PAT < 1 ? 1 : (mpad + NEWTON_SLICE_PAT - 1) / NEWTON_SLICE_PAT) : NEWTON_MAX_SPLIT; }
__host__ __device__ constexpr int newton_slice(int mpad) { return mpad <= NEWTON_SLICE_PAT * NEWTON_MAX_SPLIT ? NEWTON_SLICE_PAT : ((mpad / 32 + newton_split(mpad) - 1) / newton_split(mpad)) * 32; }
__host__ __device__ constexpr bool newton_reg_form(int mpad) { return newton_slice(mpad) <= NEWTON_SLICE_PAT; }
struct NewtonCtl { int ticket[2]; int done[2]; int abort; int odone; int pad[2]; int oticket[8]; int dbg[8];
                   unsigned long long n_requests, n_evals; };
constexpr int NEWTON_SYNC_DOUBLES = 2 * NEWTON_MAX_SPLIT * 6;

enum { MODE_NEWVIEW = 0, MODE_SUMTABLE = 1, MODE_EVALUATE = 2, MODE_EVALUATE_CAT = 3 };

constexpr int G20_RATES = 20;
struct G20Req {
    const double *table;
    const int *cnt;
    const double *weight;
    double w[G20_RATES];
    double *out;
    double *patlnl;
    int mpad, pad;
};
void launch_g20(const G20Req *reqs, int n, hipStream_t s);

struct GatherSeg {
    const uint8_t *src; const double *w; uint8_t *dst; double *dst_w; const int *rowmap;
    int src_mpad, npat, dst_mpad, dst_off, ntax_dst, pad;
};
void launch_gather(const GatherSeg *segs, int nsegs, int max_npat, hipStream_t s);

struct ShReq { const double *l0, *l1, *l2; const int *site2pat; double *out; unsigned long long seed; int nsites, nboot; };
void launch_sh(const ShReq *reqs, int n, hipStream_t s);

void launch_pmat(const ModelDev *model, const PmatReq *reqs, double *frags, int n, hipStream_t s, bool per_request = false);
void launch_eigfrags(const ModelDev *model, double *frags2, hipStream_t s);
void launch_eigfrags_n(const ModelDev *models, double *frags2, int n, hipStream_t s);
void launch_oplist(const NvOp *ops, const GeneRun *runs, int nruns, int max_mpad, bool any_pitch, bool chained, hipStream_t s, NewtonCtl *ctl = nullptr);
int fused_oplist_capacity();
bool fuse_big_genes();
void launch_reduce(const ReduceReq *reqs, int n, hipStream_t s);
void launch_newton(const ModelDev *model, const NewtonReq *reqs, const int *tickets, int nreg, int nstream, NewtonCtl *ctl, hipStream_t s);
void launch_newton_seq(const ModelDev *model, const NewtonReq *reqs, const int *req_list, int nreg, int nstream, NewtonCtl *ctl, hipStream_t s);

}
```

pepr_amd/csrc/kernels.hip:

```cpp
#include "kernels.h"

#include <algorithm>
#include <cstdlib>

namespace pml {

#define TWO_P256 1.15792089237316195423570985008687907853269984665640564039457584007913129639936e77
#define TWO_M256 8.63616855509444462538635186280017219262570580443837358382049248904e-78
#define LOG_2_256 177.445678223345993274051579105116

__device__ __forceinline__ double mfma4(double a, double b, double c) {
#ifdef ABL_NO_MFMA
    return __builtin_fma(a, b, c);
#endif
    return __builtin_amdgcn_mfma_f64_4x4x4f64(a, b, c, 0, 0, 0);
}

__device__ __forceinline__ unsigned code_mask(unsigned code) {
    return code < 20u ? (1u << code) : (code == 20u ? 0xCu : (code == 21u ? 0x60u : 0xFFFFFu));
}

template <int CTRL>
__device__ __forceinline__ double quad_swap(double v) {
    int lo = __double2loint(v), hi = __double2hiint(v);
    lo = __builtin_amdgcn_update_dpp(0, lo, CTRL, 0xF, 0xF, true);
    hi = __builtin_amdgcn_update_dpp(0, hi, CTRL, 0xF, 0xF, true);
    return __hiloint2double(hi, lo);
}
__device__ __forceinline__ double quad_sum(double v) { v += quad_swap<0xB1>(v); v += quad_swap<0x4E>(v); return v; }

__device__ __forceinline__ void frag_decode(int idx, int &c, int &row, int &col) {
    const int e = idx & 15, f = idx >> 4;
    c = f / 25;
    const int st = (f % 25) / 5, kk = f % 5;
    row = 4 * st + (e & 3); col = 4 * kk + (e >> 2);
}

constexpr int PMAT_THREADS = 256;
template <bool PER_REQ>
__global__ __launch_bounds__(PMAT_THREADS, 2) void k_pmat(const ModelDev *__restrict__ md0,
                                                          const PmatReq *__restrict__ reqs,
                                                          double *__restrict__ frags, int n) {
    __shared__ double sE[PMAT_THREADS / 64][NCAT * NS];
    const int lane = threadIdx.x & 63;
    const int wv = __builtin_amdgcn_readfirstlane(threadIdx.x >> 6);
    const int i4 = lane & 3, k4 = lane >> 4, cb = (lane >> 2) & 3;
    double Au[5][5], Bu[5][5];
    double lam0, lam1, pi_row[5];
    const int cat0 = lane / NS, cat1 = (64 + (lane & 15)) / NS;
    auto load_model = [&](const ModelDev *__restrict__ md) {
#pragma unroll
        for (int a = 0; a < 5; ++a)
#pragma unroll
            for (int b = 0; b < 5; ++b) {
                Au[a][b] = md->U[(4 * a + i4) * NS + 4 * b + k4];
                Bu[a][b] = md->Uinv[(4 * a + k4) * NS + 4 * b + i4];
            }
        lam0 = md->eval[lane % NS]; lam1 = md->eval[(64 + (lane & 15)) % NS];
#pragma unroll
        for (int a = 0; a < 5; ++a) pi_row[a] = md->pi[4 * a + k4];
    };
    if (!PER_REQ) load_model(md0);
    const int nwaves = gridDim.x * (PMAT_THREADS / 64);
    for (int rq = blockIdx.x * (PMAT_THREADS / 64) + wv; rq < n; rq += nwaves) {
        const PmatReq &req = reqs[rq];
        if (PER_REQ) load_model(req.md);
        const double tlen = req.tp ? *req.tp : req.t;
        const int kind = req.kind;
        double *sEw = sE[wv];
        sEw[lane] = exp(lam0 * (tlen * req.rates[cat0]));
        if (lane < 16) sEw[64 + lane] = exp(lam1 * (tlen * req.rates[cat1]));
        __builtin_amdgcn_fence(__ATOMIC_RELEASE, "wavefront");
        __builtin_amdgcn_wave_barrier();
        double ek[5];
#pragma unroll
        for (int kk = 0; kk < 5; ++kk) ek[kk] = sEw[cb * NS + 4 * kk + k4];
        __builtin_amdgcn_wave_barrier();
        double *out = frags + (size_t)rq * FRAG_STRIDE;
        double T[5][5];
#pragma unroll
        for (int st = 0; st < 5; ++st) {
            double a[5];
#pragma unroll
            for (int kk = 0; kk < 5; ++kk) a[kk] = Au[st][kk] * ek[kk];
#pragma unroll
            for (int nt = 0; nt < 5; ++nt) {
                double d = 0.0;
#pragma unroll
                for (int kk = 0; kk < 5; ++kk) d = mfma4(a[kk], Bu[kk][nt], d);
                T[st][nt] = d < 0.0 ? 0.0 : d;
            }
        }
        if (kind != PM_TIPTABLE) {
#pragma unroll
            for (int st = 0; st < 5; ++st) {
                const double scale = kind == PM_FRAGS_PI ? pi_row[st] : 1.0;
#pragma unroll
                for (int nt = 0; nt < 5; ++nt)
                    out[((cb * 25 + st * 5 + nt) << 4) + (i4 << 2) + k4] = T[st][nt] * scale;
            }
        } else {
            auto put = [&](int code, double v0, double v1, double v2, double v3, double v4) {
                typedef double dv2 __attribute__((ext_vector_type(2)));
                dv2 *rec = reinterpret_cast<dv2 *>(out + ((cb * NCODES + code) * 4 + k4) * TIPTAB_KK);
                rec[0] = (dv2){v0, v1}; rec[1] = (dv2){v2, v3}; rec[2] = (dv2){v4, 0.0};
            };
#pragma unroll
            for (int nt = 0; nt < 5; ++nt) put(4 * nt + i4, T[0][nt], T[1][nt], T[2][nt], T[3][nt], T[4][nt]);
            double bz[5], zq[5], any[5];
#pragma unroll
            for (int st = 0; st < 5; ++st) {
                bz[st] = T[st][0] + quad_swap<0xB1>(T[st][0]);
                zq[st] = T[st][1] + quad_swap<0xD8>(T[st][1]);
                any[st] = quad_sum(T[st][0] + T[st][1] + T[st][2] + T[st][3] + T[st][4]);
            }
            if (i4 == 2) put(20, bz[0], bz[1], bz[2], bz[3], bz[4]);
            if (i4 == 1) put(21, zq[0], zq[1], zq[2], zq[3], zq[4]);
            if (i4 == 0) put(22, any[0], any[1], any[2], any[3], any[4]);
        }
    }
}

__global__ __launch_bounds__(256) void k_eigfrags(const ModelDev *__restrict__ models,
                                                  double *__restrict__ frags2_all) {
    const ModelDev *__restrict__ md = models + blockIdx.x;
    double *__restrict__ frags2 = frags2_all + (size_t)blockIdx.x * 2 * PFRAG;
    for (int idx = threadIdx.x; idx < PFRAG; idx += 256) {
        int c, i, s;
        frag_decode(idx, c, i, s);
        frags2[idx] = md->pi[s] * md->U[s * NS + i];
        frags2[PFRAG + idx] = md->Uinv[i * NS + s];
    }
}

#define PML_TMIN 1.0e-6
#define PML_TMAX 34.5

typedef unsigned long long u64;
typedef __attribute__((address_space(1))) u64 gu64;
#ifdef PML_OPTIME
extern __device__ unsigned long long g_optime[256][2];
#endif
__device__ __forceinline__ void st_granule(u64 *p, u64 v) {
    __hip_atomic_store((gu64 *)p, v, __ATOMIC_RELAXED, __HIP_MEMORY_SCOPE_AGENT);
}
__device__ __forceinline__ u64 ld_granule(const u64 *p) {
    return __hip_atomic_load((const gu64 *)p, __ATOMIC_RELAXED, __HIP_MEMORY_SCOPE_AGENT);
}

__device__ __forceinline__ double uni(double v) {
    return __hiloint2double(__builtin_amdgcn_readfirstlane(__double2hiint(v)), __builtin_amdgcn_readfirstlane(__double2loint(v)));
}
__device__ __forceinline__ double wave_sum(double v) {
#pragma unroll
    for (int o = 32; o > 0; o >>= 1) v += __shfl_down(v, o);
    return v;
}

__device__ __forceinline__ void newton_term(double x, double e, double lr, double &f, double &f1, double &f2) {
#pragma clang fp contract(off)
    const double xe = x * e;
    const double xl = xe * lr;
    f = f + xe; f1 = f1 + xl; f2 = __builtin_fma(xl, lr, f2);
}
__device__ __forceinline__ void newton_finish(double f, double f1, double f2, double w, double ss, double &a0, double &a1, double &a2) {
#pragma clang fp contract(off)
    const double r1 = f1 / f;
    const double lg = log(f * 0.25);
    a0 = w * (lg - ss * LOG_2_256); a1 = w * r1; a2 = w * (f2 / f - r1 * r1);
}

__device__ __forceinline__ bool newton_exchange(u64 *gran, int S, int wg, int nevals, unsigned tag_base, double (&tot)[3],
                                                NewtonCtl *ctl, long long timeout_ticks) {
    const int lane = threadIdx.x & 63;
    const u64 want = (u64)(tag_base + (unsigned)nevals + 1u);
    u64 *slot = gran + (size_t)((nevals & 1) * NEWTON_MAX_SPLIT) * 6;
    if (lane < 6) {
        const int c = lane >> 1;
        const u64 bits = (u64)__double_as_longlong(c == 0 ? tot[0] : (c == 1 ? tot[1] : tot[2]));
        st_granule(slot + wg * 6 + lane, (want << 32) | ((lane & 1) ? (bits >> 32) : (bits & 0xFFFFFFFFull)));
    }
    u64 x[6] = {0, 0, 0, 0, 0, 0};
#ifdef PML_OPTIME
    const long long t_poll0 = clock64();
#endif
    const long long t_start = wall_clock64();
    unsigned polls = 0;
    bool bad = false;
    for (;;) {
        bool ok = true;
        if (lane < S) {
#pragma unroll
            for (int k = 0; k < 6; ++k) { x[k] = ld_granule(slot + lane * 6 + k); ok = ok && (x[k] >> 32) == want; }
        }
        if (__all(ok)) break;
        ++polls;
        if (polls < 16u) __builtin_amdgcn_s_sleep(1);
        else if (polls < 32u) __builtin_amdgcn_s_sleep(8);
        else if (polls < 64u) __builtin_amdgcn_s_sleep(32);
        else __builtin_amdgcn_s_sleep(127);
        if ((polls & 15u) == 0u || timeout_ticks == 0) {
            if (__hip_atomic_load(&ctl->abort, __ATOMIC_RELAXED, __HIP_MEMORY_SCOPE_AGENT) != 0) { bad = true; break; }
// ... 122 lines not shown
#pragma unroll
    for (int st = 0; st < 5; ++st) {
        if (st + PML_FRAG_AHEAD < 5) {
#pragma unroll
            for (int kk = 0; kk < 5; ++kk) a[(st + PML_FRAG_AHEAD) % 3][kk] = FRAG_RD(frag_c[((st + PML_FRAG_AHEAD) * 5 + kk) * 16]);
        }
        double acc0 = 0.0, acc1 = 0.0;
#pragma unroll
        for (int kk = 0; kk < 5; ++kk) {
            acc0 = mfma4(a[st % 3][kk], o.v[kk].x, acc0);
            acc1 = mfma4(a[st % 3][kk], o.v[kk].y, acc1);
#if PML_CONSUME_LATE
            if (kk == 0 && st > 0) consume(st - 1, p0, p1);
#endif
        }
#if PML_CONSUME_LATE
        p0 = acc0; p1 = acc1;
#else
        consume(st, acc0, acc1);
#endif
        __builtin_amdgcn_sched_barrier(0);
    }
#if PML_CONSUME_LATE
    consume(4, p0, p1);
#endif
}

struct Rows5 { dvec2 a, b; double c; };
__device__ __forceinline__ Rows5 load_rows(const double *tab, unsigned code, int c, int q) {
#ifdef ABL_NO_ROWS
    { Rows5 r1; r1.a = (dvec2){0.9, 0.9}; r1.b = (dvec2){0.9, 0.9}; r1.c = 0.9 + 1e-9 * code; return r1; }
#endif
    gcptr p = (gcptr)tab + (size_t)((c * NCODES + code) * 4 + q) * (TIPTAB_KK * 8);
    Rows5 r;
    r.a = *reinterpret_cast<const GLOBAL_AS dvec2 *>(p);
    r.b = *reinterpret_cast<const GLOBAL_AS dvec2 *>(p + 16);
    r.c = *reinterpret_cast<const GLOBAL_AS double *>(p + 32);
    return r;
}
__device__ __forceinline__ void load_cherry(Operand &o, const OpSide &sd, unsigned ca, unsigned cb, int c, int q) {
    const Rows5 a0 = load_rows(sd.t0, ca & 0xFFu, c, q), a1 = load_rows(sd.t0, ca >> 8, c, q);
    const Rows5 b0 = load_rows(sd.t1, cb & 0xFFu, c, q), b1 = load_rows(sd.t1, cb >> 8, c, q);
    o.v[0] = (dvec2){a0.a.x * b0.a.x, a1.a.x * b1.a.x};
    o.v[1] = (dvec2){a0.a.y * b0.a.y, a1.a.y * b1.a.y};
    o.v[2] = (dvec2){a0.b.x * b0.b.x, a1.b.x * b1.b.x};
    o.v[3] = (dvec2){a0.b.y * b0.b.y, a1.b.y * b1.b.y};
    o.v[4] = (dvec2){a0.c * b0.c, a1.c * b1.c};
}
struct CherryRaw { Rows5 a0, a1, b0, b1; };
__device__ __forceinline__ void issue_cherry(CherryRaw &r, const OpSide &sd, unsigned ca, unsigned cb, int c, int q) {
    r.a0 = load_rows(sd.t0, ca & 0xFFu, c, q); r.a1 = load_rows(sd.t0, ca >> 8, c, q);
    r.b0 = load_rows(sd.t1, cb & 0xFFu, c, q); r.b1 = load_rows(sd.t1, cb >> 8, c, q);
}
__device__ __forceinline__ void finish_cherry(Operand &o, const CherryRaw &r) {
    o.v[0] = (dvec2){r.a0.a.x * r.b0.a.x, r.a1.a.x * r.b1.a.x};
    o.v[1] = (dvec2){r.a0.a.y * r.b0.a.y, r.a1.a.y * r.b1.a.y};
    o.v[2] = (dvec2){r.a0.b.x * r.b0.b.x, r.a1.b.x * r.b1.b.x};
    o.v[3] = (dvec2){r.a0.b.y * r.b0.b.y, r.a1.b.y * r.b1.b.y};
    o.v[4] = (dvec2){r.a0.c * r.b0.c, r.a1.c * r.b1.c};
}
template <bool EARLY = true>
__device__ __forceinline__ void load_pitch(Operand &o, const OpSide &sd, const double *__restrict__ f_inner,
                                           unsigned ca, unsigned cb, unsigned cc, int c, int q) {
    Operand w;
    load_cherry(w, sd, ca, cb, c, q);
    Rows5 r0, r1;
    if (EARLY) { r0 = load_rows(sd.t2, cc & 0xFFu, c, q); r1 = load_rows(sd.t2, cc >> 8, c, q); }
    double v[5][2];
    contract(v, f_inner + c * 25 * 16, w);
    if (!EARLY) { r0 = load_rows(sd.t2, cc & 0xFFu, c, q); r1 = load_rows(sd.t2, cc >> 8, c, q); }
    o.v[0] = (dvec2){v[0][0] * r0.a.x, v[0][1] * r1.a.x};
    o.v[1] = (dvec2){v[1][0] * r0.a.y, v[1][1] * r1.a.y};
    o.v[2] = (dvec2){v[2][0] * r0.b.x, v[2][1] * r1.b.x};
    o.v[3] = (dvec2){v[3][0] * r0.b.y, v[3][1] * r1.b.y};
    o.v[4] = (dvec2){v[4][0] * r0.c, v[4][1] * r1.c};
}

#ifndef PML_CHAIN_UNROLL
#define PML_CHAIN_UNROLL 1
#endif
#ifndef PML_TIPLOOK
#define PML_TIPLOOK 1
#endif
template <bool PREFETCH, bool CHAIN, bool FUSE>
__device__ __forceinline__ void chunk_op(const NvOp &op, const double *__restrict__ sP, const unsigned char *__restrict__ sT,
                                         int p, int lane, Operand (&X)[4], ivec2 &xsc) {
    const int q = lane >> 4;
    constexpr size_t rowbytes = (size_t)TILE_PAT * 8;
    const size_t tabrow = (size_t)op.mpad * 8;
    const unsigned lane_off = (unsigned)(p >> 7) * (unsigned)(CLV_ROWS * rowbytes) + (unsigned)((size_t)q * rowbytes) + (unsigned)(p & (TILE_PAT - 1)) * 8u;
    const int lk = op.flags & 3, rk = (op.flags >> 2) & 3;
    const bool nt_store = (op.flags & OPF_NT_STORE) != 0;
    const int mode = op.mode;
    const bool chL = CHAIN && (op.flags & OPF_CHAIN_L) != 0, chR = CHAIN && (op.flags & OPF_CHAIN_R) != 0;
    const bool fusedN = FUSE && (op.flags & OPF_FUSED_NEWTON) != 0;
    const bool keep = !(CHAIN && (op.flags & OPF_NO_STORE) != 0) && !fusedN;
    constexpr bool TIPLOOK = PML_TIPLOOK != 0;
    constexpr bool PF_L = PREFETCH && !CHAIN;
#ifndef PML_PIN_DESC
#define PML_PIN_DESC 1
#endif
    OpSide sdl = op.l, sdr = op.r;
    const int *l_scl = op.l_scl, *r_scl = op.r_scl; int *out_scl = op.out_scl; double *outp = op.out;
#if PML_PIN_DESC
#define PML_PIN(x) asm volatile("" : "+s"(x))
    PML_PIN(sdl.p0); PML_PIN(sdl.p1); PML_PIN(sdl.p2); PML_PIN(sdl.t0); PML_PIN(sdl.t1); PML_PIN(sdl.t2); PML_PIN(sdl.f);
    PML_PIN(sdr.p0); PML_PIN(sdr.p1); PML_PIN(sdr.p2); PML_PIN(sdr.t0); PML_PIN(sdr.t1); PML_PIN(sdr.t2); PML_PIN(sdr.f);
    PML_PIN(l_scl); PML_PIN(r_scl); PML_PIN(out_scl); PML_PIN(outp);
#endif
    gcptr Lp = (gcptr)sdl.p0, Rp = (gcptr)sdr.p0;
    gptr O = (gptr)outp;
    const __amdgpu_buffer_rsrc_t orsrc = __builtin_amdgcn_make_buffer_rsrc((void *)outp, 0, 0x7FFFFFFF, 0x00020000);
    const double *fL = sP + (q * 4 + (lane & 3));
    const double *fR = fL + PFRAG;
    unsigned mx0 = 0u, mx1 = 0u;
    double site0 = 0.0, site1 = 0.0;
    unsigned cl = 0, cl2 = 0, cl3 = 0, cr = 0, cr2 = 0, cr3 = 0;
    const double *fLi = fL + 2 * PFRAG;
    const bool both_pitch = lk == SK_PITCH && rk == SK_PITCH;
    const double *fRg = sdr.f + (q * 4 + (lane & 3));
#ifdef ABL_NO_CODES
#define CODE_LD(ptr) ((((unsigned)p * 5u + 1u + (unsigned)(size_t)(ptr)) % 20u) | ((((unsigned)p * 3u + 2u) % 20u) << 8))
#else
#define CODE_LD(ptr) (*reinterpret_cast<const GLOBAL_AS unsigned short *>(ptr))
#endif
    if (lk != SK_CLV) cl = CODE_LD(Lp + p);
    if (lk >= SK_CHERRY) cl2 = CODE_LD((gcptr)sdl.p1 + p);
    if (lk == SK_PITCH) cl3 = CODE_LD((gcptr)sdl.p2 + p);
    if (rk != SK_CLV) cr = CODE_LD(Rp + p);
    if (rk >= SK_CHERRY) cr2 = CODE_LD((gcptr)sdr.p1 + p);
    if (rk == SK_PITCH) cr3 = CODE_LD((gcptr)sdr.p2 + p);

    const bool lookL = TIPLOOK && mode < MODE_EVALUATE && lk == SK_TIP && !__any((cl & 0xFFu) >= 20u || (cl >> 8) >= 20u);
    const bool lookR = TIPLOOK && mode < MODE_EVALUATE && rk == SK_TIP && !__any((cr & 0xFFu) >= 20u || (cr >> 8) >= 20u);
    const double *tL0 = sP + ((cl & 0xFFu) >> 2) * 16 + (cl & 3u) * 4 + q, *tL1 = sP + ((cl >> 8) >> 2) * 16 + ((cl >> 8) & 3u) * 4 + q;
    const double *tR0 = sP + PFRAG + ((cr & 0xFFu) >> 2) * 16 + (cr & 3u) * 4 + q, *tR1 = sP + PFRAG + ((cr >> 8) >> 2) * 16 + ((cr >> 8) & 3u) * 4 + q;
    Operand curL, curR, nxtL, nxtR;
    CherryRaw rawR;
    if (lk == SK_TIP && !lookL) load_tip(curL, sT, cl, q);
    else if (lk == SK_CLV && !chL) load_clv(curL, Lp, lane_off, rowbytes, 0);
    if (rk == SK_TIP && !lookR) load_tip(curR, sT, cr, q);
    else if (rk == SK_CLV && !chR) load_clv(curR, Rp, lane_off, rowbytes, 0);
    constexpr int CAT_UNROLL = (CHAIN && PML_CHAIN_UNROLL) ? NCAT : 1;
#pragma unroll CAT_UNROLL
    for (int c = 0; c < NCAT; ++c) {
        Operand Y;
        constexpr bool DIRECT = CHAIN && CAT_UNROLL == NCAT;
#ifndef PML_DIRECT_FUSE
#define PML_DIRECT_FUSE 0
#endif
        constexpr bool DIRECT_IN = DIRECT && (!FUSE || PML_DIRECT_FUSE);
        if (CHAIN && !DIRECT_IN) {
            if (CAT_UNROLL == NCAT) { if (chL) curL = X[c]; if (chR) curR = X[c]; }
            else { if (chL) curL = X[0]; if (chR) curR = X[0]; }
        }
        if (PREFETCH && c + 1 < NCAT) {
            if (PF_L && lk == SK_CLV && !chL) load_clv(nxtL, Lp, lane_off, rowbytes, c + 1);
            if (rk == SK_CLV && !chR) load_clv(nxtR, Rp, lane_off, rowbytes, c + 1);
        }
#ifndef PML_PF_ROWS
#define PML_PF_ROWS 0
#endif
        constexpr bool PF_ROWS = PML_PF_ROWS && DIRECT && !FUSE;
        const bool pfR = PF_ROWS && rk == SK_CHERRY && lk == SK_CLV && mode < MODE_EVALUATE;
#if PML_PF_ROWS == 1
        if (pfR) { if (c == 0) issue_cherry(rawR, sdr, cr, cr2, 0, q); finish_cherry(curR, rawR); }
#else
        if (pfR) issue_cherry(rawR, sdr, cr, cr2, c, q);
#endif
        if (lk == SK_CHERRY) load_cherry(curL, sdl, cl, cl2, c, q);
        else if (lk == SK_PITCH) load_pitch<!FUSE>(curL, sdl, fLi, cl, cl2, cl3, c, q);
        if (pfR) {}
        else if (rk == SK_CHERRY) load_cherry(curR, sdr, cr, cr2, c, q);
        else if (rk == SK_PITCH) { if (both_pitch) load_pitch<!FUSE>(curR, sdr, fRg, cr, cr2, cr3, c, q); else load_pitch<!FUSE>(curR, sdr, fLi, cr, cr2, cr3, c, q); }
        if (mode >= MODE_EVALUATE) {
            if (DIRECT_IN && chL) contract_stream(fR + c * 25 * 16, curR, [&](int st, double y0, double y1) { site0 += X[c].v[st].x * y0; site1 += X[c].v[st].y * y1; });
            else if (DIRECT_IN && chR) contract_stream(fR + c * 25 * 16, X[c], [&](int st, double y0, double y1) { site0 += curL.v[st].x * y0; site1 += curL.v[st].y * y1; });
            else contract_stream(fR + c * 25 * 16, curR, [&](int st, double y0, double y1) {
                site0 += curL.v[st].x * y0; site1 += curL.v[st].y * y1;
            });
            if (mode == MODE_EVALUATE_CAT) {
                double a0 = site0, a1 = site1;
                a0 += __shfl_xor(a0, 16); a0 += __shfl_xor(a0, 32);
                a1 += __shfl_xor(a1, 16); a1 += __shfl_xor(a1, 32);
                if (q == 0) *reinterpret_cast<GLOBAL_AS dvec2 *>(O + (size_t)c * tabrow + 8 * p) = (dvec2){a0, a1};
                site0 = 0.0; site1 = 0.0;
            }
        } else {
// ... 46 lines not shown
    }
    if (mode == MODE_NEWVIEW) {
        mx0 = max(mx0, (unsigned)__shfl_xor((int)mx0, 16)); mx0 = max(mx0, (unsigned)__shfl_xor((int)mx0, 32));
        mx1 = max(mx1, (unsigned)__shfl_xor((int)mx1, 16)); mx1 = max(mx1, (unsigned)__shfl_xor((int)mx1, 32));
        constexpr unsigned HI_TWO_M256 = (1023u - 256u) << 20;
        const bool n0 = mx0 < HI_TWO_M256, n1 = mx1 < HI_TWO_M256;
        if (__any(n0 || n1)) {
            if (CHAIN) {
                const double f0 = n0 ? TWO_P256 : 1.0, f1 = n1 ? TWO_P256 : 1.0;
#pragma unroll
                for (int c = 0; c < NCAT; ++c)
#pragma unroll
                    for (int k = 0; k < 5; ++k) { X[c].v[k].x *= f0; X[c].v[k].y *= f1; }
            }
            if (keep && (n0 || n1)) {
#pragma unroll 1
                for (int r = 0; r < NCAT * 5; ++r) {
                    GLOBAL_AS dvec2 *ptr = reinterpret_cast<GLOBAL_AS dvec2 *>(O + (size_t)((r / 5) * NS + (r % 5) * 4) * rowbytes + lane_off);
                    dvec2 v = *ptr;
                    if (n0) v.x *= TWO_P256;
                    if (n1) v.y *= TWO_P256;
                    *ptr = v;
                }
            }
        }
        if (q == 0) { sc.x += n0 ? 1 : 0; sc.y += n1 ? 1 : 0; if (keep) *reinterpret_cast<GLOBAL_AS ivec2 *>((gptr)out_scl + 4 * p) = sc; }
        if (CHAIN) xsc = sc;
    } else if (mode == MODE_SUMTABLE || mode == MODE_EVALUATE_CAT) {
        if (fusedN) xsc = sc;
        else if (q == 0) *reinterpret_cast<GLOBAL_AS ivec2 *>((gptr)out_scl + 4 * p) = sc;
    } else {
        site0 += __shfl_xor(site0, 16); site0 += __shfl_xor(site0, 32);
        site1 += __shfl_xor(site1, 16); site1 += __shfl_xor(site1, 32);
        if (q == 0) {
            const double l0 = log(site0 * 0.25) - sc.x * LOG_2_256;
            const double l1 = log(site1 * 0.25) - sc.y * LOG_2_256;
            *reinterpret_cast<GLOBAL_AS dvec2 *>(O + 8 * p) = (dvec2){l0, l1};
        }
    }
}

constexpr int PAT_PER_WG = 4 * PAT_PER_WAVE;
constexpr int TIPTAB = NCODES * NS;

__device__ __forceinline__ void stage_frags_dma(const NvOp &op, double *dst, int lane, int wave) {
    for (int i = wave; i < 25; i += 4) {
        const int e = i * 128 + lane * 2;
        const double *g = (e < PFRAG) ? (op.pl ? op.pl : op.pr) + e : (op.pr ? op.pr : op.pl) + (e - PFRAG);
        __builtin_amdgcn_global_load_lds((const GLOBAL_AS void *)g, (__attribute__((address_space(3))) void *)(dst + i * 128), 16, 0, 0);
    }
}

#ifndef PML_CHAIN_WAVES
#define PML_CHAIN_WAVES 2
#endif
__device__ __forceinline__ void dma_chunk(const double *set, double *lds_set, int k, int lane) {
    const GLOBAL_AS char *src = (const GLOBAL_AS char *)set + k * 4096 + lane * 16;
    __attribute__((address_space(3))) char *dst = (__attribute__((address_space(3))) char *)lds_set + k * 4096;
    if (k < 3) {
        __builtin_amdgcn_global_load_lds((const GLOBAL_AS void *)src, (__attribute__((address_space(3))) void *)dst, 16, 0, 0);
        __builtin_amdgcn_global_load_lds((const GLOBAL_AS void *)src, (__attribute__((address_space(3))) void *)dst, 16, 1024, 0);
        __builtin_amdgcn_global_load_lds((const GLOBAL_AS void *)src, (__attribute__((address_space(3))) void *)dst, 16, 2048, 0);
        __builtin_amdgcn_global_load_lds((const GLOBAL_AS void *)src, (__attribute__((address_space(3))) void *)dst, 16, 3072, 0);
    } else if (lane < 32) __builtin_amdgcn_global_load_lds((const GLOBAL_AS void *)src, (__attribute__((address_space(3))) void *)dst, 16, 0, 0);
}
__device__ __forceinline__ void stage_frags_dma3(const NvOp &op, double *dst, int lane, int wave) {
    const int wv = __builtin_amdgcn_readfirstlane(wave);
    const double *pl = op.pl, *pr = op.pr;
    const int lk = op.flags & 3, rk = (op.flags >> 2) & 3;
    const double *inner = (lk == SK_PITCH) ? op.l.f : (rk == SK_PITCH) ? op.r.f : nullptr;
    dma_chunk(pl ? pl : pr, dst, wv, lane);
    dma_chunk(pr ? pr : pl, dst + PFRAG, (wv + 1) & 3, lane);
    if (inner != nullptr) dma_chunk(inner, dst + 2 * PFRAG, (wv + 2) & 3, lane);
}

struct FusedShared {
    double exl[NCAT * NS][2];
    double red[3];
    double fb[3][PAT_PER_WAVE * 4];
    double ss[PAT_PER_WAVE * 4];
    double bc[4];
};
static_assert(sizeof(FusedShared) <= PFRAG * sizeof(double), "fused Newton scratch fits one fragment region");
__device__ __forceinline__ void newton_fused(const NvOp &op, double *scratch, const Operand (&X)[4], const ivec2 xsc,
                                             bool active, int blk, NewtonCtl *ctl, long long timeout_ticks) {
    const NewtonReq &r = *reinterpret_cast<const NewtonReq *>(op.aux);
    FusedShared &sh = *reinterpret_cast<FusedShared *>(scratch);
    const int tid = threadIdx.x, lane = tid & 63, wave = tid >> 6, q = lane >> 4, pl = wave * PAT_PER_WAVE + 2 * (lane & 15);
    const int mpad = r.mpad, S = newton_split(mpad);
    const ModelDev *__restrict__ md = r.md;
    u64 *gran = reinterpret_cast<u64 *>(r.sync);
    __syncthreads();
    if (q == 0) { sh.ss[pl] = active ? (double)xsc.x : 0.0; sh.ss[pl + 1] = active ? (double)xsc.y : 0.0; }
    if (tid == 0) sh.bc[3] = 0.0;
    double sw = 0.0;
    if (wave < 2) { const int pf = blk * (PAT_PER_WAVE * 4) + wave * 64 + lane; if (pf < mpad) sw = r.weight[pf]; }
    int nevals = 0;
    auto eval_at = [&](double t, double &L, double &d1, double &d2) -> bool {
        if (tid < NCAT * NS) {
            const double lr = md->eval[tid % NS] * r.rates[tid / NS];
            sh.exl[tid][0] = exp(lr * t); sh.exl[tid][1] = lr;
        }
        __syncthreads();
        double fa = 0.0, fa1 = 0.0, fa2 = 0.0, fb = 0.0, fb1 = 0.0, fb2 = 0.0;
#pragma unroll
        for (int c = 0; c < NCAT; ++c)
#pragma unroll
            for (int st = 0; st < 5; ++st) {
                const int row = c * NS + 4 * st + q;
                const double e = sh.exl[row][0], lr = sh.exl[row][1];
                newton_term(X[c].v[st].x, e, lr, fa, fa1, fa2);
                newton_term(X[c].v[st].y, e, lr, fb, fb1, fb2);
            }
        fa += __shfl_xor(fa, 16); fa += __shfl_xor(fa, 32); fa1 += __shfl_xor(fa1, 16); fa1 += __shfl_xor(fa1, 32); fa2 += __shfl_xor(fa2, 16); fa2 += __shfl_xor(fa2, 32);
        fb += __shfl_xor(fb, 16); fb += __shfl_xor(fb, 32); fb1 += __shfl_xor(fb1, 16); fb1 += __shfl_xor(fb1, 32); fb2 += __shfl_xor(fb2, 16); fb2 += __shfl_xor(fb2, 32);
        if (q == 0) {
            sh.fb[0][pl] = fa; sh.fb[1][pl] = fa1; sh.fb[2][pl] = fa2;
            sh.fb[0][pl + 1] = fb; sh.fb[1][pl + 1] = fb1; sh.fb[2][pl + 1] = fb2;
        }
        __syncthreads();
        double tot[3] = {0.0, 0.0, 0.0};
        if (wave < 2) {
            double a0 = 0.0, a1 = 0.0, a2 = 0.0;
            if (sw != 0.0) {
                const int j = wave * 64 + lane;
                newton_finish(sh.fb[0][j], sh.fb[1][j], sh.fb[2][j], sw, sh.ss[j], a0, a1, a2);
            }
            tot[0] = wave_sum(a0); tot[1] = wave_sum(a1); tot[2] = wave_sum(a2);
            if (wave == 0 && lane == 0) { sh.red[0] = tot[0]; sh.red[1] = tot[1]; sh.red[2] = tot[2]; }
        }
        __syncthreads();
        if (wave == 1) {
#pragma unroll
            for (int i = 0; i < 3; ++i) tot[i] = sh.red[i] + __shfl(tot[i], 0);
            bool bad = false;
            if (S > 1) bad = newton_exchange(gran, S, blk, nevals, r.tag_base, tot, ctl, timeout_ticks);
            if (lane == 0) { sh.bc[0] = tot[0]; sh.bc[1] = tot[1]; sh.bc[2] = tot[2]; if (bad) sh.bc[3] = 1.0; }
        }
        __syncthreads();
        ++nevals;
        L = uni(sh.bc[0]); d1 = uni(sh.bc[1]); d2 = uni(sh.bc[2]);
        return sh.bc[3] == 0.0;
    };
    double t, L, d1, d2;
    const bool ok = newton_drive(r.t0, r.max_iter, r.tol, eval_at, t, L, d1, d2);
    if (tid == 64 && blk == 0) {
        atomicAdd(&ctl->n_requests, 1ull); atomicAdd(&ctl->n_evals, (unsigned long long)nevals);
        if (!ok) { t = r.t0; L = __builtin_nan(""); }
        r.out[0] = t; r.out[1] = L; r.out[2] = d1; r.out[3] = d2;
        if (r.t_dev0) { *r.t_dev0 = t; *r.t_dev1 = t; }
    }
}

#ifdef PML_OPTIME
__device__ unsigned long long g_optime[256][2];
}
extern "C" void pml_abl_optime(unsigned long long *out, int reset) {
    (void)hipDeviceSynchronize();
    (void)hipMemcpyFromSymbol(out, HIP_SYMBOL(pml::g_optime), sizeof(unsigned long long) * 512);
    if (reset) { static unsigned long long z[512]; (void)hipMemcpyToSymbol(HIP_SYMBOL(pml::g_optime), z, sizeof z); }
}
namespace pml {
#endif
template <int VARIANT>
__global__ __launch_bounds__(256, (VARIANT == 1) ? 4 : (VARIANT >= 8) ? PML_CHAIN_WAVES : 3) void k_oplist(
        const NvOp *__restrict__ ops, const GeneRun *__restrict__ runs, int nruns, int blocks_per_gene, int any_pitch,
        NewtonCtl *ctl, long long timeout_ticks) {
#ifdef PML_OPTIME
    const long long t_life0 = clock64();
#endif
    constexpr bool PREFETCH = !(VARIANT & 1);
    constexpr bool CHAIN = VARIANT >= 8;
    constexpr bool FUSE = VARIANT == 15;
    constexpr bool DBUF3 = CHAIN && (VARIANT & 2) != 0;
    constexpr bool DBUF = ((VARIANT & 2) != 0 && VARIANT < 4) || DBUF3;
    constexpr int PARITY_STRIDE = (DBUF3 ? 3 : 2) * PFRAG;
    Operand X[4]; ivec2 xsc = {0, 0};
#pragma unroll
    for (int c = 0; c < 4; ++c)
#pragma unroll
        for (int k = 0; k < 5; ++k) X[c].v[k] = (dvec2){0.0, 0.0};
    extern __shared__ double sP[];
    const int nfrag_regions = DBUF3 ? 6 : (DBUF ? 4 : 2) + (any_pitch ? 1 : 0);
    unsigned char *sT = reinterpret_cast<unsigned char *>(sP + nfrag_regions * PFRAG);
    const int tid = threadIdx.x, lane = tid & 63, wave = tid >> 6;
    const bool one_part = blocks_per_gene < 0;
    if (one_part) blocks_per_gene = -blocks_per_gene;
    const int xcd = one_part ? 0 : (blockIdx.x & 7);
    int slot = one_part ? (int)blockIdx.x : (int)(blockIdx.x >> 3);
    const bool ticketed = FUSE && ctl != nullptr;
    if (ticketed) {
        __shared__ int s_slot;
        if (tid == 0) s_slot = __hip_atomic_fetch_add(&ctl->oticket[xcd], 1, __ATOMIC_RELAXED, __HIP_MEMORY_SCOPE_AGENT);
        __syncthreads();
        slot = s_slot;
    }
    auto leave = [&]() {
        if (!ticketed) return;
        __syncthreads();
        if (tid == 0) {
            const int d = __hip_atomic_fetch_add(&ctl->odone, 1, __ATOMIC_RELAXED, __HIP_MEMORY_SCOPE_AGENT);
            if (d == (int)gridDim.x - 1) {
#pragma unroll
                for (int k = 0; k < 8; ++k) __hip_atomic_store(&ctl->oticket[k], 0, __ATOMIC_RELAXED, __HIP_MEMORY_SCOPE_AGENT);
                __hip_atomic_store(&ctl->odone, 0, __ATOMIC_RELAXED, __HIP_MEMORY_SCOPE_AGENT);
            }
        }
    };
    const int gi = one_part ? slot / blocks_per_gene : xcd + 8 * (slot / blocks_per_gene), blk = slot % blocks_per_gene;
    if (gi >= nruns) { leave(); return; }
    const GeneRun run = runs[gi];
    if (run.op_begin >= run.op_end) { leave(); return; }
    const int mpad = ops[run.op_begin].mpad;
    if (blk * PAT_PER_WG >= mpad) { leave(); return; }
    const int p = (blk * 4 + wave) * PAT_PER_WAVE + 2 * (lane & 15);
    const bool active = (blk * 4 + wave) * PAT_PER_WAVE < mpad;

#ifdef PML_OPTIME
    const long long t_start1 = clock64();
#endif
    for (int i = tid; i < TIPTAB; i += 256) sT[i] = (unsigned char)((code_mask(i / NS) >> (i % NS)) & 1u);
    if (DBUF) { if (DBUF3) stage_frags_dma3(ops[run.op_begin], sP, lane, wave); else stage_frags_dma(ops[run.op_begin], sP, lane, wave); }
    __syncthreads();
#ifdef PML_OPTIME
    const long long t_start2 = clock64();
    long long t_newton = 0, t_bar = 0, t_ops = 0;
#endif
    for (int oi = run.op_begin; oi < run.op_end; ++oi) {
        const NvOp &op = ops[oi];
        const double *buf = sP;
        if (DBUF) {
            const int par = (oi - run.op_begin) & 1;
            buf = sP + par * PARITY_STRIDE;
            if (oi + 1 < run.op_end) {
                if (DBUF3) stage_frags_dma3(ops[oi + 1], sP + (par ^ 1) * PARITY_STRIDE, lane, wave);
                else stage_frags_dma(ops[oi + 1], sP + (par ^ 1) * PARITY_STRIDE, lane, wave);
            }
        } else {
            if (oi > run.op_begin) __syncthreads();
            const double2 *gl = reinterpret_cast<const double2 *>(op.pl);
            const double2 *gr = reinterpret_cast<const double2 *>(op.pr);
            double2 *s2 = reinterpret_cast<double2 *>(sP);
            for (int i = tid; i < PFRAG / 2; i += 256) {
                if (op.mode < MODE_EVALUATE && op.pl) s2[i] = gl[i];
                if (op.pr) s2[PFRAG / 2 + i] = gr[i];
            }
            if (any_pitch) {
                const int lk = op.flags & 3, rk = (op.flags >> 2) & 3;
                const double2 *il = reinterpret_cast<const double2 *>(op.l.f), *ir = reinterpret_cast<const double2 *>(op.r.f);
                for (int i = tid; i < PFRAG / 2; i += 256) {
                    if (lk == SK_PITCH) s2[PFRAG + i] = il[i];
                    else if (rk == SK_PITCH) s2[PFRAG + i] = ir[i];
                }
            }
            __syncthreads();
        }
#ifdef PML_OPTIME
        const long long t_op0 = clock64();
#endif
#ifndef ABL_NO_OP
        if (active) chunk_op<PREFETCH, CHAIN, FUSE>(op, buf, sT, p, lane, X, xsc);
#endif
#ifdef PML_OPTIME
        if (lane == 0 && active) {
            const int k = (op.flags & 15) | ((op.mode & 3) << 4) | ((op.flags & (OPF_CHAIN_L | OPF_CHAIN_R)) ? 64 : 0) | ((op.flags & OPF_NO_STORE) ? 128 : 0);
            atomicAdd(&g_optime[k][0], (unsigned long long)(clock64() - t_op0)); atomicAdd(&g_optime[k][1], 1ull);
        }
        t_ops += clock64() - t_op0;
        const long long t_n0 = clock64();
#endif
        if (FUSE && (op.flags & OPF_FUSED_NEWTON) != 0) {
            if (__hip_atomic_load(&ctl->abort, __ATOMIC_RELAXED, __HIP_MEMORY_SCOPE_AGENT) != 0) {
                const NewtonReq &r = *reinterpret_cast<const NewtonReq *>(op.aux);
                if (tid == 0 && blk == 0) { r.out[0] = r.t0; r.out[1] = __builtin_nan(""); r.out[2] = 0.0; r.out[3] = 0.0; }
            } else newton_fused(op, const_cast<double *>(buf), X, xsc, active, blk, ctl, timeout_ticks);
        }
#ifdef PML_OPTIME
        const long long t_b0 = clock64(); t_newton += t_b0 - t_n0;
#endif
#ifndef ABL_NO_BARRIER
        if (DBUF) __syncthreads();
#endif
#ifdef PML_OPTIME
        t_bar += clock64() - t_b0;
#endif
    }
#ifdef PML_OPTIME
    if (lane == 0 && active) {
        const int b = FUSE ? 230 : 238;
        const long long t_end = clock64();
        atomicAdd(&g_optime[b][0], (unsigned long long)(t_end - t_life0)); atomicAdd(&g_optime[b][1], 1ull);
        atomicAdd(&g_optime[b + 1][0], (unsigned long long)(t_start1 - t_life0)); atomicAdd(&g_optime[b + 2][0], (unsigned long long)(t_start2 - t_start1));
        atomicAdd(&g_optime[b + 3][0], (unsigned long long)t_ops); atomicAdd(&g_optime[b + 4][0], (unsigned long long)t_newton); atomicAdd(&g_optime[b + 5][0], (unsigned long long)t_bar);
    }
#endif
    leave();
}

struct Operand1 { double v[5]; };

__device__ __forceinline__ void load_clv1(Operand1 &o, gcptr base, unsigned lane_off, size_t rowbytes, int c) {
#pragma unroll
    for (int kk = 0; kk < 5; ++kk)
        o.v[kk] = __builtin_nontemporal_load(reinterpret_cast<const GLOBAL_AS double *>(base + (size_t)(c * NS + kk * 4) * rowbytes + lane_off));
}
__device__ __forceinline__ void load_tip1(Operand1 &o, const unsigned char *__restrict__ T, unsigned code, int q) {
    const unsigned char *t0 = T + code * NS + q;
#pragma unroll
    for (int kk = 0; kk < 5; ++kk) o.v[kk] = (double)t0[kk * 4];
}
__device__ __forceinline__ void contract1(double (&acc)[5], const double *__restrict__ frag_c, const Operand1 &o) {
#pragma unroll
    for (int st = 0; st < 5; ++st) acc[st] = 0.0;
#pragma unroll
    for (int kk = 0; kk < 5; ++kk) {
        double a[5];
#pragma unroll
        for (int st = 0; st < 5; ++st) a[st] = frag_c[(st * 5 + kk) * 16];
#pragma unroll
        for (int st = 0; st < 5; ++st) acc[st] = mfma4(a[st], o.v[kk], acc[st]);
        __builtin_amdgcn_sched_barrier(0);
    }
}
template <typename F>
__device__ __forceinline__ void contract_stream1(const double *__restrict__ frag_c, const Operand1 &o, F &&consume) {
#pragma unroll
    for (int st = 0; st < 5; ++st) {
        double a[5];
#pragma unroll
        for (int kk = 0; kk < 5; ++kk) a[kk] = frag_c[(st * 5 + kk) * 16];
        double acc = 0.0;
#pragma unroll
        for (int kk = 0; kk < 5; ++kk) acc = mfma4(a[kk], o.v[kk], acc);
        consume(st, acc);
        __builtin_amdgcn_sched_barrier(0);
    }
}
__device__ __forceinline__ void load_cherry1(Operand1 &o, const OpSide &sd, unsigned ca, unsigned cb, int c, int q) {
    const Rows5 a = load_rows(sd.t0, ca, c, q), b = load_rows(sd.t1, cb, c, q);
    o.v[0] = a.a.x * b.a.x; o.v[1] = a.a.y * b.a.y; o.v[2] = a.b.x * b.b.x; o.v[3] = a.b.y * b.b.y; o.v[4] = a.c * b.c;
}
__device__ __forceinline__ void load_pitch1(Operand1 &o, const OpSide &sd, const double *__restrict__ f_inner,
                                            unsigned ca, unsigned cb, unsigned cc, int c, int q) {
    Operand1 w;
    load_cherry1(w, sd, ca, cb, c, q);
    double v[5];
    contract1(v, f_inner + c * 25 * 16, w);
    const Rows5 r = load_rows(sd.t2, cc, c, q);
    o.v[0] = v[0] * r.a.x; o.v[1] = v[1] * r.a.y; o.v[2] = v[2] * r.b.x; o.v[3] = v[3] * r.b.y; o.v[4] = v[4] * r.c;
}

__device__ __forceinline__ void chunk_op1(const NvOp &op, const double *__restrict__ sP, const unsigned char *__restrict__ sT,
                                          int p, int lane, Operand1 (&X)[4], int &xsc) {
    const int q = lane >> 4;
    constexpr size_t rowbytes = (size_t)TILE_PAT * 8;
    const size_t tabrow = (size_t)op.mpad * 8;
    const unsigned lane_off = (unsigned)(p >> 7) * (unsigned)(CLV_ROWS * rowbytes) + (unsigned)((size_t)q * rowbytes) + (unsigned)(p & (TILE_PAT - 1)) * 8u;
    const int lk = op.flags & 3, rk = (op.flags >> 2) & 3;
    const bool nt_store = (op.flags & OPF_NT_STORE) != 0;
    const int mode = op.mode;
    const bool chL = (op.flags & OPF_CHAIN_L) != 0, chR = (op.flags & OPF_CHAIN_R) != 0;
    const bool keep = (op.flags & OPF_NO_STORE) == 0;
    gcptr Lp = (gcptr)op.l.p0, Rp = (gcptr)op.r.p0;
    gptr O = (gptr)op.out;
    const __amdgpu_buffer_rsrc_t orsrc = __builtin_amdgcn_make_buffer_rsrc((void *)op.out, 0, 0x7FFFFFFF, 0x00020000);
    const double *fL = sP + (q * 4 + (lane & 3));
    const double *fR = fL + PFRAG;
    double mx = 0.0, site = 0.0;
// ... 411 lines not shown
    if (delta > 0.0) {
        const unsigned long long base = (r.seed + 1ull) * 0x9E3779B97F4A7C15ull, ns = (unsigned long long)r.nsites;
        for (int b = tid; b < r.nboot; b += 256) {
            double s0 = 0.0, s1 = 0.0, s2 = 0.0;
            const unsigned long long k0 = base + (unsigned long long)b * ns;
            for (int j = 0; j < r.nsites; ++j) {
                const int p = r.site2pat[(int)(mix64(k0 + (unsigned long long)j) % ns)];
                s0 += r.l0[p]; s1 += r.l1[p]; s2 += r.l2[p];
            }
            s0 -= orig[0]; s1 -= orig[1]; s2 -= orig[2];
            const double best = fmax(s0, fmax(s1, s2));
            const double second = (best == s0) ? fmax(s1, s2) : (best == s1 ? fmax(s0, s2) : fmax(s0, s1));
            if (best - second < delta) cnt[0] += 1.0;
        }
    }
    __shared__ double red1[1][4];
    block_sum<1, 4>(cnt, red1);
    if (tid == 0) *r.out = (r.nboot > 0) ? cnt[0] / (double)r.nboot : 0.0;
}

__global__ __launch_bounds__(256) void k_g20(const G20Req *__restrict__ reqs) {
    __shared__ double red[1][4];
    __shared__ double w[G20_RATES];
    const G20Req &r = reqs[blockIdx.x];
    if (threadIdx.x < G20_RATES) w[threadIdx.x] = r.w[threadIdx.x];
    __syncthreads();
    const size_t M = (size_t)r.mpad;
    double acc[1] = {0.0};
    for (int p = threadIdx.x; p < r.mpad; p += 256) {
        const double wt = r.weight[p];
        double l = 0.0;
        if (wt != 0.0) {
            int m = r.cnt[p];
#pragma unroll
            for (int j = 1; j < G20_RATES / 4; ++j) m = min(m, r.cnt[(size_t)j * M + p]);
            double sum = 0.0;
#pragma unroll
            for (int j = 0; j < G20_RATES / 4; ++j) {
                const int d = r.cnt[(size_t)j * M + p] - m;
                const double f = ldexp(1.0, -256 * d);
#pragma unroll
                for (int c = 0; c < 4; ++c) sum += w[4 * j + c] * r.table[(size_t)(4 * j + c) * M + p] * f;
            }
            l = log(sum) - m * LOG_2_256;
            acc[0] += wt * l;
        }
        if (r.patlnl) r.patlnl[p] = l;
    }
    block_sum<1, 4>(acc, red);
    if (threadIdx.x == 0) *r.out = acc[0];
}

void launch_g20(const G20Req *reqs, int n, hipStream_t s) {
    if (n <= 0) return;
    hipLaunchKernelGGL(k_g20, dim3((unsigned)n), dim3(256), 0, s, reqs);
}
void launch_sh(const ShReq *reqs, int n, hipStream_t s) {
    if (n <= 0) return;
    hipLaunchKernelGGL(k_sh, dim3((unsigned)n), dim3(256), 0, s, reqs);
}
void launch_gather(const GatherSeg *segs, int nsegs, int max_npat, hipStream_t s) {
    if (nsegs <= 0 || max_npat <= 0) return;
    hipLaunchKernelGGL(k_gather, dim3((unsigned)nsegs, (unsigned)((max_npat + 255) / 256)), dim3(256), 0, s, segs);
}
void launch_pmat(const ModelDev *model, const PmatReq *reqs, double *frags, int n, hipStream_t s, bool per_request) {
    if (n <= 0) return;
    const int per_block = PMAT_THREADS / 64;
    const int blocks = std::min((n + per_block - 1) / per_block, 512);
    if (per_request) hipLaunchKernelGGL(k_pmat<true>, dim3(blocks), dim3(PMAT_THREADS), 0, s, model, reqs, frags, n);
    else hipLaunchKernelGGL(k_pmat<false>, dim3(blocks), dim3(PMAT_THREADS), 0, s, model, reqs, frags, n);
}
void launch_eigfrags(const ModelDev *model, double *frags2, hipStream_t s) {
    hipLaunchKernelGGL(k_eigfrags, dim3(1), dim3(256), 0, s, model, frags2);
}
void launch_eigfrags_n(const ModelDev *models, double *frags2, int n, hipStream_t s) {
    if (n > 0) hipLaunchKernelGGL(k_eigfrags, dim3((unsigned)n), dim3(256), 0, s, models, frags2);
}
static int oplist_variant() {
    static int v = -1;
    if (v < 0) { const char *e = getenv("PML_OPLIST_VARIANT"); v = e ? atoi(e) : 1; }
    return v;
}
static long long newton_timeout_ticks();
static void launch_oplist_one(const NvOp *ops, const GeneRun *runs, int nruns, int bpg, bool one_part, bool any_pitch, bool chained, hipStream_t s, NewtonCtl *ctl);
int fused_oplist_capacity();
bool fuse_big_genes();
void launch_oplist(const NvOp *ops, const GeneRun *runs, int nruns, int max_mpad, bool any_pitch, bool chained, hipStream_t s, NewtonCtl *ctl) {
    if (nruns <= 0) return;
    const int bpg = (max_mpad + PAT_PER_WG - 1) / PAT_PER_WG;
    if (!ctl) { launch_oplist_one(ops, runs, nruns, bpg, false, any_pitch, chained, s, nullptr); return; }
    if (bpg <= 32) { launch_oplist_one(ops, runs, nruns, bpg, false, any_pitch, true, s, ctl); return; }
    if (fuse_big_genes()) { launch_oplist_one(ops, runs, nruns, bpg, true, any_pitch, true, s, ctl); return; }
    const int cap = fused_oplist_capacity();
    const int genes_per_launch = std::max(1, cap / bpg);
    for (int off = 0; off < nruns; off += genes_per_launch)
        launch_oplist_one(ops, runs + off, std::min(genes_per_launch, nruns - off), bpg, true, any_pitch, true, s, ctl);
}
bool fuse_big_genes() {
    static const bool on = !(std::getenv("PML_FUSE_BIG") && std::atoi(std::getenv("PML_FUSE_BIG")) == 0);
    return on;
}
int fused_oplist_capacity() {
    static const int cap = [] {
        int dev = 0, cus = 256, nb = 2; hipDeviceProp_t p;
        if (hipGetDevice(&dev) == hipSuccess && hipGetDeviceProperties(&p, dev) == hipSuccess) cus = p.multiProcessorCount;
        const size_t lds15 = (size_t)6 * PFRAG * sizeof(double) + 512;
        (void)hipFuncSetAttribute(reinterpret_cast<const void *>(k_oplist<15>), hipFuncAttributeMaxDynamicSharedMemorySize, (int)lds15);
        if (hipOccupancyMaxActiveBlocksPerMultiprocessor(&nb, reinterpret_cast<const void *>(k_oplist<15>), 256, lds15) != hipSuccess || nb < 1) nb = 1;
        if (nb > 2) nb = 2;
        return cus * nb;
    }();
    return cap;
}
static void launch_oplist_one(const NvOp *ops, const GeneRun *runs, int nruns, int bpg_in, bool one_part, bool any_pitch, bool chained, hipStream_t s, NewtonCtl *ctl) {
    const long long to = newton_timeout_ticks();
    const int bpg = one_part ? -bpg_in : bpg_in;
    const dim3 grid((unsigned)(one_part ? nruns * bpg_in : ((nruns + 7) / 8) * 8 * bpg_in)), block(256);
    int v = oplist_variant();
    if (any_pitch && (v == 2 || v == 3)) v = 1;
    if (chained) {
        static const int cv = std::getenv("PML_CHAIN_VARIANT") ? std::atoi(std::getenv("PML_CHAIN_VARIANT")) : 11;
        v = cv == 9 ? 9 : (cv == 16 ? 16 : (cv == 10 ? 10 : 11));
        if (ctl) v = 15;
    }
    if (v == 16) {
        const size_t lds16 = (size_t)6 * PFRAG * sizeof(double) + 512;
        static const hipError_t big16 = hipFuncSetAttribute(reinterpret_cast<const void *>(k_oplist16), hipFuncAttributeMaxDynamicSharedMemorySize, (int)lds16);
        if (big16 == hipSuccess) {
            hipLaunchKernelGGL(k_oplist16, grid, dim3(OPL16_THREADS), lds16, s, ops, runs, nruns, bpg_in);
            return;
        }
        v = 11;
    }
    const bool dbuf = (v == 2 || v == 3);
    size_t lds = (size_t)((dbuf ? 4 : 2) + (any_pitch ? 1 : 0)) * PFRAG * sizeof(double) + 512;
    if (v == 11 || v == 15 || v == 10) {
        lds = (size_t)6 * PFRAG * sizeof(double) + 512;
        static const hipError_t big11 = [&] {
            const hipError_t a = hipFuncSetAttribute(reinterpret_cast<const void *>(k_oplist<11>), hipFuncAttributeMaxDynamicSharedMemorySize, (int)lds);
            const hipError_t b = hipFuncSetAttribute(reinterpret_cast<const void *>(k_oplist<15>), hipFuncAttributeMaxDynamicSharedMemorySize, (int)lds);
            (void)hipFuncSetAttribute(reinterpret_cast<const void *>(k_oplist<10>), hipFuncAttributeMaxDynamicSharedMemorySize, (int)lds);
            return a != hipSuccess ? a : b;
        }();
        if (big11 != hipSuccess && v == 11) {
            v = 9; lds = (size_t)(2 + (any_pitch ? 1 : 0)) * PFRAG * sizeof(double) + 512;
        }
    }
    const int ap = any_pitch ? 1 : 0;
    switch (v) {
        case 0: hipLaunchKernelGGL(k_oplist<0>, grid, block, lds, s, ops, runs, nruns, bpg, ap, ctl, to); break;
        case 2: hipLaunchKernelGGL(k_oplist<2>, grid, block, lds, s, ops, runs, nruns, bpg, ap, ctl, to); break;
        case 3: hipLaunchKernelGGL(k_oplist<3>, grid, block, lds, s, ops, runs, nruns, bpg, ap, ctl, to); break;
        case 5: hipLaunchKernelGGL(k_oplist<5>, grid, block, lds, s, ops, runs, nruns, bpg, ap, ctl, to); break;
        case 9: hipLaunchKernelGGL(k_oplist<9>, grid, block, lds, s, ops, runs, nruns, bpg, ap, ctl, to); break;
        case 10: hipLaunchKernelGGL(k_oplist<10>, grid, block, lds, s, ops, runs, nruns, bpg, ap, ctl, to); break;
        case 11: hipLaunchKernelGGL(k_oplist<11>, grid, block, lds, s, ops, runs, nruns, bpg, ap, ctl, to); break;
        case 15: hipLaunchKernelGGL(k_oplist<15>, grid, block, lds, s, ops, runs, nruns, bpg, ap, ctl, to); break;
        default: hipLaunchKernelGGL(k_oplist<1>, grid, block, lds, s, ops, runs, nruns, bpg, ap, ctl, to); break;
    }
}
void launch_reduce(const ReduceReq *reqs, int n, hipStream_t s) {
    if (n <= 0) return;
    hipLaunchKernelGGL(k_reduce, dim3(n), dim3(256), 0, s, reqs);
}
static long long newton_timeout_ticks() {
    static const long long v = [] { const char *e = std::getenv("PML_NEWTON_TIMEOUT_US"); return e ? std::atoll(e) * 100LL : 2000000LL * 100LL; }();
    return v;
}
void launch_newton(const ModelDev *model, const NewtonReq *reqs, const int *tickets, int nreg, int nstream, NewtonCtl *ctl, hipStream_t s) {
    const long long to = newton_timeout_ticks();
    if (nreg > 0) hipLaunchKernelGGL((k_newton<true, false>), dim3((unsigned)nreg), dim3(NEWTON_THREADS), 0, s, model, reqs, tickets, ctl, to);
    if (nstream > 0) hipLaunchKernelGGL((k_newton<false, false>), dim3((unsigned)nstream), dim3(NEWTON_THREADS), 0, s, model, reqs, tickets + nreg, ctl, to);
}
void launch_newton_seq(const ModelDev *model, const NewtonReq *reqs, const int *req_list, int nreg, int nstream, NewtonCtl *ctl, hipStream_t s) {
    if (nreg > 0) hipLaunchKernelGGL((k_newton<true, true>), dim3((unsigned)nreg), dim3(NEWTON_THREADS), 0, s, model, reqs, req_list, ctl, 0LL);
    if (nstream > 0) hipLaunchKernelGGL((k_newton<false, true>), dim3((unsigned)nstream), dim3(NEWTON_THREADS), 0, s, model, reqs, req_list + nreg, ctl, 0LL);
}

}
```

pepr_amd/csrc/parsimony.hip:

```cpp
#include <algorithm>
#include <cstring>
#include <functional>

#include "engine.hpp"

namespace pml {

struct FOp { int kind, out, l, r, y, x, score, pad; };
enum { F_SET = 0, F_COUNT = 1, F_COSTX = 2, F_PATH = 3, F_SETCOUNT = 4 };
struct FRun {
    const FOp *ops; unsigned *pool; const int *w; int *partial;
    int nops, mpad, nwaves, pad;
};
struct FRed { const int *partial; int *out; int nscores, nwaves; };

typedef const unsigned __attribute__((address_space(1))) *gcu32;
typedef unsigned __attribute__((address_space(1))) *gu32;

__device__ __forceinline__ unsigned fitch(unsigned l, unsigned r) { const unsigned x = l & r; return x ? x : (l | r); }

__device__ __forceinline__ int wave_sum(int v) {
    v += __builtin_amdgcn_update_dpp(0, v, 0xB1, 0xF, 0xF, true);
    v += __builtin_amdgcn_update_dpp(0, v, 0x4E, 0xF, 0xF, true);
    v += __builtin_amdgcn_update_dpp(0, v, 0x141, 0xF, 0xF, true);
// ... 62 lines not shown
    return z ^ (z >> 31);
}

namespace {
struct PGene {
    EncodedAlignment aln; Tree tree; std::vector<int> order;
    int nvec = 0, ngroups = 1, nwaves = 0;
    unsigned *d_pool = nullptr; int *d_w = nullptr;
    int vtip(int i) const { return i; }
    int vmsg(int v, int k) const { return aln.ntax + (v - aln.ntax) * 3 + k; }
    int vpath(int grp, int depth, int radius) const { return aln.ntax + 3 * (aln.ntax - 2) + grp * (radius + 2) + depth; }
    int vside(int v, int to) const { return v < aln.ntax ? v : vmsg(v, tree.slot(v, to)); }
    void refresh_ops(int root_tip, std::vector<FOp> &ops, int *nscore) const {
        const int r = tree.nbr[root_tip][0];
        std::function<void(int, int)> post = [&](int v, int from) {
            if (v < aln.ntax) return;
            const int k = tree.slot(v, from), x = tree.nbr[v][(k + 1) % 3], y = tree.nbr[v][(k + 2) % 3];
            post(x, v); post(y, v);
            FOp o{nscore ? F_SETCOUNT : F_SET, vmsg(v, k), vside(x, v), vside(y, v), 0, 0, nscore ? (*nscore)++ : 0, 0};
            ops.push_back(o);
        };
        std::function<void(int, int)> pre = [&](int v, int from) {
            if (v < aln.ntax) return;
            const int k = tree.slot(v, from);
            for (int j = 1; j <= 2; ++j) {
                const int h = tree.nbr[v][(k + j) % 3], o = tree.nbr[v][(k + 3 - j) % 3];
                ops.push_back(FOp{F_SET, vmsg(v, (k + j) % 3), vside(from, v), vside(o, v), 0, 0, 0, 0});
                pre(h, v);
            }
        };
        post(r, root_tip);
        if (nscore) ops.push_back(FOp{F_COUNT, 0, vside(r, root_tip), vtip(root_tip), 0, 0, (*nscore)++, 0});
        pre(r, root_tip);
    }
};
struct Stage {
    Ctx *ctx; void *d = nullptr; size_t cap = 0;
    int ensure(size_t bytes) {
        if (bytes <= cap) return 0;
        if (d) hipFree(d);
        cap = bytes + bytes / 2; d = nullptr;
        PCHK(hipMalloc(&d, cap));
        return 0;
    }
    ~Stage() { if (d) hipFree(d); }
};
}

static int fitch_step(Ctx *ctx, Stage &st, Stage &sc, const std::vector<PGene *> &owner, const std::vector<std::vector<FOp>> &ops_of,
                      const std::vector<int> &nscores, std::vector<std::vector<int>> &scores) {
    const size_t nr = owner.size();
    if (!nr) return 0;
    size_t nops = 0, npart = 0, nsc = 0; int max_mpad = 0, max_sc = 0;
    for (size_t i = 0; i < nr; ++i) { nops += ops_of[i].size(); npart += (size_t)nscores[i] * owner[i]->nwaves; nsc += nscores[i];
                                      max_mpad = std::max(max_mpad, owner[i]->aln.mpad); max_sc = std::max(max_sc, nscores[i]); }
    const size_t o_runs = 0, o_reds = o_runs + nr * sizeof(FRun), o_ops = o_reds + nr * sizeof(FRed), total = o_ops + nops * sizeof(FOp);
    if (int rc = st.ensure(total)) return rc;
    if (int rc = sc.ensure((npart + nsc) * sizeof(int))) return rc;
    std::vector<char> h(total);
    FRun *runs = (FRun *)(h.data() + o_runs); FRed *reds = (FRed *)(h.data() + o_reds); FOp *ops = (FOp *)(h.data() + o_ops);
    int *d_part = (int *)sc.d, *d_out = d_part + npart;
    size_t po = 0, pp = 0, ps = 0;
    for (size_t i = 0; i < nr; ++i) {
        std::memcpy(ops + po, ops_of[i].data(), ops_of[i].size() * sizeof(FOp));
        runs[i] = FRun{(const FOp *)((char *)st.d + o_ops) + po, owner[i]->d_pool, owner[i]->d_w, d_part + pp, (int)ops_of[i].size(), owner[i]->aln.mpad, owner[i]->nwaves, 0};
        reds[i] = FRed{d_part + pp, d_out + ps, nscores[i], owner[i]->nwaves};
        po += ops_of[i].size(); pp += (size_t)nscores[i] * owner[i]->nwaves; ps += nscores[i];
    }
    PCHK(hipMemcpyAsync(st.d, h.data(), total, hipMemcpyHostToDevice, ctx->stream));
    hipLaunchKernelGGL(k_fitch, dim3((max_mpad + 255) / 256, (unsigned)nr), dim3(256), 0, ctx->stream, (const FRun *)((char *)st.d + o_runs));
    if (nsc) hipLaunchKernelGGL(k_fitch_reduce, dim3(std::min(64, (max_sc + 255) / 256), (unsigned)nr), dim3(256), 0, ctx->stream, (const FRed *)((char *)st.d + o_reds));
    PCHK(hipGetLastError());
    std::vector<int> flat(nsc);
    if (nsc) PCHK(hipMemcpyAsync(flat.data(), d_out, nsc * sizeof(int), hipMemcpyDeviceToHost, ctx->stream));
    if (int rc_ = ctx->sync(ctx->stream)) return rc_;
    scores.assign(nr, {});
    ps = 0;
    for (size_t i = 0; i < nr; ++i) { scores[i].assign(flat.begin() + ps, flat.begin() + ps + nscores[i]); ps += nscores[i]; }
    return 0;
}

int parsimony_batch(Ctx *ctx, int n, const pml_alignment_view *alns, unsigned seed, int radius,
                    std::vector<Tree> &trees_out, std::vector<EncodedAlignment> &alns_out, std::vector<long long> &lengths_out, std::vector<int> &moves_out) {
    std::vector<PGene> G(n);
    Stage st{ctx}, sc{ctx};
    size_t total_blocks = 0;
    for (int g = 0; g < n; ++g) {
        std::string err;
        if (!G[g].aln.encode(alns[g].ntax, alns[g].nsites, alns[g].names, alns[g].rows, err)) return ctx->fail(-2, "gene " + std::to_string(g) + ": " + err);
        if (G[g].aln.ntax < 3) return ctx->fail(-2, "gene " + std::to_string(g) + ": parsimony needs at least 3 taxa");
        total_blocks += (G[g].aln.mpad + 255) / 256;
    }
    const int want_groups = radius > 0 ? (int)std::max<size_t>(1, std::min<size_t>(64, (2048 + total_blocks - 1) / std::max<size_t>(total_blocks, 1))) : 1;
    struct Free { std::vector<PGene> &G; ~Free() { for (auto &g : G) { if (g.d_pool) hipFree(g.d_pool); if (g.d_w) hipFree(g.d_w); } } } freer{G};
    for (int g = 0; g < n; ++g) {
        PGene &pg = G[g]; const int nt = pg.aln.ntax, mp = pg.aln.mpad;
        pg.ngroups = want_groups; pg.nwaves = ((mp + 255) / 256) * 4;
        pg.nvec = nt + 3 * (nt - 2) + pg.ngroups * (radius + 2);
        PCHK(hipMalloc((void **)&pg.d_pool, (size_t)pg.nvec * mp * sizeof(unsigned)));
        PCHK(hipMalloc((void **)&pg.d_w, (size_t)mp * sizeof(int)));
        std::vector<unsigned> tips((size_t)nt * mp); std::vector<int> w(mp);
        for (size_t i = 0; i < tips.size(); ++i) tips[i] = code_mask(pg.aln.codes[i]);
        for (int p = 0; p < mp; ++p) w[p] = (int)pg.aln.weight[p];
        PCHK(hipMemcpy(pg.d_pool, tips.data(), tips.size() * sizeof(unsigned), hipMemcpyHostToDevice));
        PCHK(hipMemcpy(pg.d_w, w.data(), w.size() * sizeof(int), hipMemcpyHostToDevice));
        pg.order.resize(nt);
        for (int i = 0; i < nt; ++i) pg.order[i] = i;
        if (seed) { uint64_t s = seed; for (int i = nt - 1; i >= 1; --i) std::swap(pg.order[i], pg.order[(int)(splitmix(s) % (uint64_t)(i + 1))]); }
        Tree &t = pg.tree; t.ntax = nt;
        t.nbr.assign(2 * nt - 2, {-1, -1, -1}); t.len.assign(2 * nt - 2, {0.1, 0.1, 0.1});
        for (int k = 0; k < 3; ++k) { t.nbr[nt][k] = pg.order[k]; t.nbr[pg.order[k]][0] = nt; }
    }
    std::vector<PGene *> owner; std::vector<std::vector<FOp>> ops_of; std::vector<int> nscores; std::vector<std::vector<int>> scores;
    int max_tax = 0; for (auto &g : G) max_tax = std::max(max_tax, g.aln.ntax);
    for (int s = 3; s < max_tax; ++s) {
        owner.clear(); ops_of.clear(); nscores.clear();
        std::vector<std::vector<std::pair<int, int>>> edges;
        for (auto &pg : G) {
            if (s >= pg.aln.ntax) continue;
            const Tree &t = pg.tree; const int x = pg.order[s];
            std::vector<FOp> ops; pg.refresh_ops(pg.order[0], ops, nullptr);
            std::vector<std::pair<int, int>> ed;
            for (int v = 0; v < t.nnodes(); ++v) {
                if (t.nbr[v][0] < 0) continue;
                for (int k = 0; k < 3; ++k) { const int u = t.nbr[v][k]; if (u < 0 || u < v) continue;
                    ops.push_back(FOp{F_COSTX, 0, pg.vside(v, u), pg.vside(u, v), 0, pg.vtip(x), (int)ed.size(), 0}); ed.push_back({v, u}); }
            }
            owner.push_back(&pg); ops_of.push_back(std::move(ops)); nscores.push_back((int)ed.size()); edges.push_back(std::move(ed));
        }
        if (int rc = fitch_step(ctx, st, sc, owner, ops_of, nscores, scores)) return rc;
        for (size_t i = 0; i < owner.size(); ++i) {
            PGene &pg = *owner[i]; Tree &t = pg.tree; const int nt = pg.aln.ntax, x = pg.order[s], w = nt + s - 2;
            int best = 0;
            for (int e = 1; e < (int)scores[i].size(); ++e) if (scores[i][e] < scores[i][best]) best = e;
            const int bv = edges[i][best].first, bu = edges[i][best].second;
            t.nbr[bv][t.slot(bv, bu)] = w; t.nbr[bu][t.slot(bu, bv)] = w;
            t.nbr[w] = {bv, bu, x}; t.nbr[x][0] = w;
        }
    }
    moves_out.assign(n, 0);
    std::vector<char> active(n, 0);
    for (int g = 0; g < n; ++g) active[g] = radius > 0 && G[g].aln.ntax > 4;
    struct Cand { int v, k, g, h, base; };
    for (int round = 0;; ++round) {
        owner.clear(); ops_of.clear(); nscores.clear();
        for (int g = 0; g < n; ++g) if (active[g] && round < 20 * G[g].aln.ntax) { std::vector<FOp> ops; G[g].refresh_ops(0, ops, nullptr); owner.push_back(&G[g]); ops_of.push_back(std::move(ops)); nscores.push_back(0); } else active[g] = 0;
        if (owner.empty()) break;
        if (int rc = fitch_step(ctx, st, sc, owner, ops_of, nscores, scores)) return rc;
        std::vector<int> gene_of_owner;
        for (int g = 0; g < n; ++g) if (active[g]) gene_of_owner.push_back(g);
        size_t cursor = 0;
        while (cursor < gene_of_owner.size()) {
            owner.clear(); ops_of.clear(); nscores.clear();
            std::vector<std::vector<Cand>> cands; std::vector<int> run_gene;
            size_t staged = 0;
            for (; cursor < gene_of_owner.size() && (staged == 0 || staged < (8u << 20)); ++cursor) {
                const int g = gene_of_owner[cursor]; PGene &pg = G[g]; const Tree &t = pg.tree; const int nt = pg.aln.ntax;
                std::vector<std::vector<FOp>> gops(pg.ngroups); std::vector<std::vector<Cand>> gc(pg.ngroups);
                int prune_no = 0;
                for (int v = nt; v < t.nnodes(); ++v) for (int k = 0; k < 3; ++k) {
                    const int sub = t.nbr[v][k], x = t.nbr[v][(k + 1) % 3], y = t.nbr[v][(k + 2) % 3];
                    if (x < nt && y < nt) continue;
                    const int grp = prune_no++ % pg.ngroups;
                    auto &ops = gops[grp]; auto &cs = gc[grp];
                    const int P = pg.vside(sub, v), base = (int)cs.size();
                    ops.push_back(FOp{F_COSTX, 0, pg.vside(x, v), pg.vside(y, v), 0, P, base, 0}); cs.push_back(Cand{v, k, -1, -1, base});
// ... 54 lines not shown
```

Measured before the change: 167.8.

## Fuse consecutive Newton branch-optimization steps into one persistent pass launch

Deferred Newton steps that each end in a fused Newton operation are chained into a single oplist kernel launch. Per-gene segments are linked, and the kernel walks them on the device. P-matrices that depend on a branch length optimized earlier in the same pass are rebuilt inside the kernel from LDS-held results. The aim is to cut per-step launch overhead and host round trips during branch optimization. In exchange the staging and bookkeeping get more complex (fragment and sync offsets, step serials, abort propagation), and the default flush cap rises. Separately, hipSetDevice calls are added for correctness with multiple devices.

```diff
diff --git a/pepr_amd/csrc/api.cpp b/pepr_amd/csrc/api.cpp
--- a/pepr_amd/csrc/api.cpp
+++ b/pepr_amd/csrc/api.cpp
@@ -210,6 +210,7 @@
 static int oneshot_on(Ctx &c, int op, int n, const pml_alignment *alns, const char *const *newicks,
                       const pml_model *model, const pml_search_opts *opts, int flags, pml_result *const *out, int share) {
     pml_fpguard fpg;
+    if (hipSetDevice(c.device) != hipSuccess) return c.fail(PML_EDEVICE, "hipSetDevice failed");
     std::vector<std::string> pstart; std::vector<const char *> pnw;
     static_assert(sizeof(pml_alignment) == sizeof(pml_alignment_view), "alignment view layout");
     if (op == OP_SEARCH && opts && opts->seed != 0) {
diff --git a/pepr_amd/csrc/engine.cpp b/pepr_amd/csrc/engine.cpp
--- a/pepr_amd/csrc/engine.cpp
+++ b/pepr_amd/csrc/engine.cpp
@@ -158,8 +158,8 @@
     virtual_pitch = virtual_cherries && std::getenv("PML_NO_PITCH") == nullptr;
     if (n <= 0) return ctx->fail(-1, "empty batch");
     if (nc != 1 && nc != 4) return ctx->fail(-1, "ncat must be 1 or 4");
+    HIPCHK(hipSetDevice(ctx->device));
     if (int rc = ctx->ensure_model(pm)) return rc;
-    HIPCHK(hipSetDevice(ctx->device));
     genes.resize(n);
     const double t_create0 = now_ms();
     {
@@ -326,8 +326,8 @@
     const int n = (int)sel.size();
     if (n <= 0) return ctx->fail(-1, "empty batch");
     if (pm == 2) return ctx->fail(-1, "PROTGAMMAWAGF (empirical frequencies) is built for score / optimize / search calls, not for device-gathered replicates");
+    HIPCHK(hipSetDevice(ctx->device));
     if (int rc = ctx->ensure_model(pm)) return rc;
-    HIPCHK(hipSetDevice(ctx->device));
     genes.resize(n);
     struct SegH { int rep, gene, off; size_t rowmap_off; };
     std::vector<SegH> segs; std::vector<int> rowmaps;
@@ -430,7 +430,7 @@
         HIPCHK(hipMalloc((void **)&d_lenpool, tot * sizeof(double)));
         tot = 0; for (auto &G : genes) { G.d_len = d_lenpool + tot; tot += (size_t)G.tree.nnodes() * 3; }
     }
-    for (auto &G : genes) G.len_pending.assign((size_t)G.tree.nnodes() * 3, 0);
+    for (auto &G : genes) { G.len_pending.assign((size_t)G.tree.nnodes() * 3, 0); G.len_step.assign((size_t)G.tree.nnodes() * 3, 0); }
     if (int rc = ensure_stage(std::min<size_t>(nresults * 4096 + (1 << 20), (size_t)256 << 20))) return rc;
     chain = true; chain_off = 0; flush_quota = 1;
     return 0;
@@ -589,13 +589,61 @@
     return 0;
 }
 
+static size_t flush_max_steps() {
+    static const size_t v = std::min<size_t>(std::getenv("PML_FLUSH_MAX") ? (size_t)std::max(1, std::atoi(std::getenv("PML_FLUSH_MAX"))) : 16, PASS_MAX_STEPS);
+    return v;
+}
 int Batch::flush_deferred() {
     if (deferred.empty()) return 0;
-    struct Guard { Batch *b; ~Guard() { b->deferred.clear(); b->ctx->tic_stream = nullptr; } } guard{this};
-    const size_t lo = deferred.front().base, hi = deferred.back().base + deferred.back().bytes;
+    struct Guard { Batch *b; ~Guard() { b->deferred.clear(); b->ctx->tic_stream = nullptr; b->frag_off = 0; b->nsync_off = 0; } } guard{this};
+    const size_t lo = deferred.front().base;
+    size_t hi = deferred.back().base + deferred.back().bytes;
     const hipStream_t cs = deferred.front().lane ? ctx->stream2 : ctx->stream;
+    const ModelDev *md = pi_mode < 2 ? ctx->d_model[pi_mode] : nullptr;
+    if (deferred.front().pass) {
+        size_t nreq_tot = 0; for (const Deferred &L : deferred) nreq_tot += L.nreq;
+        const size_t o_creq = align_up(hi, 256), o_heads = align_up(o_creq + nreq_tot * sizeof(PmatReq), 256);
+        const size_t end = align_up(o_heads + genes.size() * sizeof(long long), 256);
+        if (!chain || hi != chain_off || end > h_cap) return ctx->fail(-5, "internal: no room for the tables of a pass launch");
+        PmatReq *creq = (PmatReq *)((char *)h_stage + o_creq);
+        long long *heads = (long long *)((char *)h_stage + o_heads);
+        pass_last.assign(genes.size(), nullptr);
+        size_t nheads = 0, cum = 0; int max_mpad = 0; bool any_pitch = false; double algo_bytes = 0, algo_flops = 0;
+        for (const Deferred &L : deferred) {
+            if (!L.pass || L.lane != 0 || L.frag_base != deferred.front().frag_base + cum || L.run_gene.size() != L.nruns)
+                return ctx->fail(-5, "internal: the steps of a pass launch do not line up");
+            std::memcpy(creq + cum, (char *)h_stage + L.base + L.o_req, L.nreq * sizeof(PmatReq));
+            PassSeg *segs = (PassSeg *)((char *)h_stage + L.base + L.o_seg);
+            for (size_t r = 0; r < L.nruns; ++r) {
+                PassSeg &sg = segs[r];
+                sg.reqs_off = (long long)(o_creq + cum * sizeof(PmatReq));
+                if (sg.step != (int)(L.serial - deferred.front().serial) || sg.step >= PASS_MAX_STEPS) return ctx->fail(-5, "internal: pass step numbering");
+                const long long off = (long long)((char *)&sg - (char *)h_stage);
+                PassSeg *&last = pass_last[L.run_gene[r]];
+                if (last) last->next_off = off; else heads[nheads++] = off;
+                last = &sg;
+            }
+            cum += L.nreq; max_mpad = std::max(max_mpad, L.max_mpad); any_pitch = any_pitch || L.any_pitch;
+            algo_bytes += L.algo_bytes; algo_flops += L.algo_flops;
+        }
+        chain_off = end; hi = end;
+        HIPCHK(hipMemcpyAsync((char *)d_stage + lo, (char *)h_stage + lo, hi - lo, hipMemcpyHostToDevice, cs));
+        double *const fr = d_frags + deferred.front().frag_base * FRAG_STRIDE;
+        ctx->tic_stream = cs;
+        if (nreq_tot) {
+            ctx->tic(K_PMAT, (double)nreq_tot * PFRAG * 8);
+            launch_pmat(md, (const PmatReq *)((char *)d_stage + o_creq), fr, (int)nreq_tot, cs, d_gmodel != nullptr);
+            ctx->toc();
+        }
+        ctx->tic(K_NEWVIEW, algo_bytes, algo_flops);
+        launch_oplist((const NvOp *)d_stage, nullptr, (int)nheads, max_mpad, any_pitch, true, cs, d_nctl, (const long long *)((char *)d_stage + o_heads));
+        ctx->toc();
+        ctx->tic_stream = nullptr;
+        if (hipError_t e = hipGetLastError(); e != hipSuccess) return ctx->fail(-5, std::string("kernel launch: ") + hipGetErrorString(e));
+        flush_quota = std::min<size_t>(flush_quota * 2, flush_max_steps());
+        return 0;
+    }
     HIPCHK(hipMemcpyAsync((char *)d_stage + lo, (char *)h_stage + lo, hi - lo, hipMemcpyHostToDevice, cs));
-    const ModelDev *md = pi_mode < 2 ? ctx->d_model[pi_mode] : nullptr;
     static const bool serialize = std::getenv("PML_SERIALIZE") != nullptr;
 #define PML_SER() do { if (serialize) hipStreamSynchronize(st); } while (0)
     if (serialize) hipStreamSynchronize(cs);
@@ -630,8 +678,7 @@
         if (hipError_t e = hipGetLastError(); e != hipSuccess) return ctx->fail(-5, std::string("kernel launch: ") + hipGetErrorString(e));
     }
 #undef PML_SER
-    static const size_t flush_max = std::getenv("PML_FLUSH_MAX") ? (size_t)std::atoi(std::getenv("PML_FLUSH_MAX")) : 8;
-    flush_quota = std::min<size_t>(flush_quota * 2, flush_max);
+    flush_quota = std::min<size_t>(flush_quota * 2, std::getenv("PML_FLUSH_MAX") ? flush_max_steps() : 8);
     return 0;
 }
 
@@ -653,13 +700,33 @@
         nreq_max = std::min(nreq_max, keyed + loose);
     }
     bool any_pitch = false, any_chain = false;
-    if (int rc = ensure_frags(std::max(nreq_max, (size_t)1))) return rc;
+    const size_t ngenes = genes.size();
+    std::vector<int> &nparts = run_nparts; nparts.assign(ngenes, 1);
+    for (auto &o : ops) nparts[o.gene] = std::max(nparts[o.gene], o.part + 1);
+    for (auto &t : tails) nparts[t.gene] = std::max(nparts[t.gene], t.part + 1);
+    static const bool fuse_env = std::getenv("PML_NO_FUSE") == nullptr && !(std::getenv("PML_CHAIN") && std::atoi(std::getenv("PML_CHAIN")) == 0);
+    bool fuse_ok = fuse_env && !newton_safe_mode();
+    if (fuse_ok && nnewton && !fuse_big_genes()) {
+        int mm = 0; size_t nr = 0;
+        std::vector<char> seen(genes.size(), 0);
+        for (auto &o : ops) if (!seen[o.gene]) { seen[o.gene] = 1; nr += (size_t)nparts[o.gene]; mm = std::max(mm, genes[o.gene].aln.mpad); }
+        for (auto &t : tails) if (!seen[t.gene]) { seen[t.gene] = 1; nr += (size_t)nparts[t.gene]; mm = std::max(mm, genes[t.gene].aln.mpad); }
+        const size_t bpg = (size_t)(mm + TILE_PAT - 1) / TILE_PAT;
+        if (bpg > 32 && nr * bpg > (size_t)fused_oplist_capacity()) fuse_ok = false;
+    }
+    static const bool pass_env = !(std::getenv("PML_PASS_FUSE") && std::atoi(std::getenv("PML_PASS_FUSE")) == 0);
+    const bool pass_step = pass_env && pass_allowed && chain && !lanes_active && lane == 0 && fuse_ok && nnewton > 0 && ntail == nnewton && !record_plan;
+    if (!deferred.empty() && deferred.back().pass != pass_step) { if (int rc = flush_deferred()) return rc; }
+    if (int rc = ensure_frags(std::max((pass_step ? frag_off : 0) + nreq_max, (size_t)1))) return rc;
     double *&nsync_buf = lane ? d_nsync2 : d_nsync; size_t &nsync_c = lane ? nsync_cap2 : nsync_cap;
-    if (nnewton > nsync_c) {
+    const size_t flush_max = flush_max_steps();
+    const size_t nsync_want = nnewton * (pass_step ? flush_max : 1);
+    if (nsync_want <= nsync_c && (pass_step ? nsync_off : 0) + nnewton > nsync_c) { if (int rc = chain_sync()) return rc; }
+    if (nsync_want > nsync_c) {
         if (chain) { if (int rc = chain_sync()) return rc; }
         if (nsync_buf) hipFree(nsync_buf);
         nsync_buf = nullptr; nsync_c = 0;
-        const size_t cap = std::max(nnewton * 2, (size_t)256);
+        const size_t cap = std::max(nsync_want * 2, (size_t)256);
         HIPCHK(hipMalloc((void **)&nsync_buf, cap * NEWTON_SYNC_DOUBLES * sizeof(double)));
         HIPCHK(hipMemsetAsync(nsync_buf, 0, cap * NEWTON_SYNC_DOUBLES * sizeof(double), ctx->stream));
         { if (int rc_ = ctx->sync(ctx->stream)) return rc_; }
@@ -673,10 +740,7 @@
     const hipStream_t st = lane ? ctx->stream2 : ctx->stream;
     double *const frags_buf = lane ? d_frags2 : d_frags;
     ctx->tic_stream = st;
-    const size_t ngenes = genes.size();
-    std::vector<int> &nparts = run_nparts; nparts.assign(ngenes, 1);
-    for (auto &o : ops) nparts[o.gene] = std::max(nparts[o.gene], o.part + 1);
-    for (auto &t : tails) nparts[t.gene] = std::max(nparts[t.gene], t.part + 1);
+    const size_t frag_base = pass_step ? frag_off : 0, sync_base = pass_step ? nsync_off : 0;
     std::vector<size_t> &koff = run_koff; koff.assign(ngenes + 1, 0);
     for (size_t g = 0; g < ngenes; ++g) koff[g + 1] = koff[g] + (size_t)nparts[g];
     const size_t nkeys = koff[ngenes];
@@ -688,9 +752,13 @@
     size_t ntick_max = 0;
     for (auto &t : tails) if (t.mode == MODE_SUMTABLE) ntick_max += (size_t)newton_split(genes[t.gene].aln.mpad);
     const size_t o_tick = align_up(o_newt + nnewton * sizeof(NewtonReq), 256);
-    const size_t bytes = align_up(o_tick + ntick_max * sizeof(int), 256);
-    if (chain && chain_off + bytes > h_cap) { if (int rc = chain_sync()) return rc; }
-    if (int rc = ensure_stage(bytes)) return rc;
+    const size_t o_seg = align_up(o_tick + ntick_max * sizeof(int), 256);
+    const size_t o_bl = align_up(o_seg + (pass_step ? nkeys * sizeof(PassSeg) : 0), 256);
+    const size_t bytes = align_up(o_bl + (pass_step ? nreq_max * sizeof(int) : 0), 256);
+    size_t tail_reserve = 0;
+    if (pass_step) { tail_reserve = (nreq_max + 4) * sizeof(PmatReq) + ngenes * sizeof(long long) + 1024; for (auto &D : deferred) tail_reserve += D.nreq * sizeof(PmatReq); }
+    if (chain && chain_off + bytes + tail_reserve > h_cap) { if (int rc = chain_sync()) return rc; }
+    if (int rc = ensure_stage(bytes + tail_reserve)) return rc;
     const size_t base = chain ? chain_off : 0;
     if (chain) chain_off += bytes;
     char *hs = (char *)h_stage + base, *ds = (char *)d_stage + base;
@@ -700,18 +768,13 @@
     ReduceReq *hred = (ReduceReq *)(hs + o_red);
     NewtonReq *hnewt = (NewtonReq *)(hs + o_newt);
     int *htick = (int *)(hs + o_tick);
-    if (nnewton) ++newton_launch_seq;
+    if (nnewton) { ++newton_launch_seq; if ((newton_launch_seq & 0x3FFFFFu) == 0) ++newton_launch_seq; }
     const unsigned tag_base = (newton_launch_seq & 0x3FFFFFu) << 10;
-    static const bool fuse_env = std::getenv("PML_NO_FUSE") == nullptr && !(std::getenv("PML_CHAIN") && std::atoi(std::getenv("PML_CHAIN")) == 0);
-    bool fuse_ok = fuse_env && !newton_safe_mode();
-    if (fuse_ok && nnewton && !fuse_big_genes()) {
-        int mm = 0; size_t nr = 0;
-        std::vector<char> seen(genes.size(), 0);
-        for (auto &o : ops) if (!seen[o.gene]) { seen[o.gene] = 1; nr += (size_t)nparts[o.gene]; mm = std::max(mm, genes[o.gene].aln.mpad); }
-        for (auto &t : tails) if (!seen[t.gene]) { seen[t.gene] = 1; nr += (size_t)nparts[t.gene]; mm = std::max(mm, genes[t.gene].aln.mpad); }
-        const size_t bpg = (size_t)(mm + TILE_PAT - 1) / TILE_PAT;
-        if (bpg > 32 && nr * bpg > (size_t)fused_oplist_capacity()) fuse_ok = false;
-    }
+    PassSeg *hseg = (PassSeg *)(hs + o_seg);
+    int *hbl = (int *)(hs + o_bl);
+    size_t nbl = 0;
+    std::vector<int> run_gene;
+    const unsigned long long my_serial = ++step_serial;
     std::vector<char> fused_req(nnewton, 0);
     bool any_fused = false;
     std::vector<int> tail_req(ntail, -1);
@@ -749,13 +812,18 @@
                 for (auto &e : *bucket) if (e.first == tbits) return e.second;
             }
         }
-        if (ireq >= nreq_max) { req_overflow = true; return frags_buf; }
+        if (ireq >= nreq_max) { req_overflow = true; return frags_buf + frag_base * FRAG_STRIDE; }
         PmatReq &r = hreq[ireq];
-        r.t = t; std::memcpy(r.rates, genes[g].rates, sizeof r.rates); r.kind = kind; r.pad = 0;
+        r.t = t; std::memcpy(r.rates, genes[g].rates, sizeof r.rates); r.kind = kind; r.in_pass = 0;
         r.tp = (chain && v >= 0 && genes[g].len_pending[(size_t)v * 3 + q]) ? genes[g].d_len + (size_t)v * 3 + q : nullptr;
         r.md = d_gmodel ? d_gmodel + g : nullptr;
+        if (pass_step && r.tp && !deferred.empty() && genes[g].len_step[(size_t)v * 3 + q] >= deferred.front().serial) {
+            r.in_pass = (int)(genes[g].len_step[(size_t)v * 3 + q] - deferred.front().serial) + 1;
+            r.md = model_of((int)g);
+            pass_build.push_back((int)ireq);
+        }
         last_src.push_back({(int)g, v, q, kind});
-        const double *out = frags_buf + (ireq++) * FRAG_STRIDE;
+        const double *out = frags_buf + (frag_base + ireq++) * FRAG_STRIDE;
         if (!record_plan) { if (v >= 0) { req_stamp[key] = req_launch; req_ptr[key] = out; } else bucket->push_back({tbits, out}); }
         return out;
     };
@@ -818,6 +886,7 @@
         const int mp = G.aln.mpad;
         GeneRun &run = hruns[nruns++];
         run.op_begin = (int)nout;
+        pass_build.clear();
         max_mpad = std::max(max_mpad, mp);
         static const int chain_env = std::getenv("PML_CHAIN") ? std::atoi(std::getenv("PML_CHAIN")) : 2;
         const bool chain_reads = chain_env == 2 || (chain_env == 1 && record_plan), chain_nostore = chain_env >= 1 && record_plan && !record_stored;
@@ -872,7 +941,7 @@
                 std::memcpy(nr.rates, G.rates, sizeof nr.rates);
                 nr.t0 = t.t0; nr.tol = newton_tol; nr.out = result; nr.mpad = mp; nr.max_iter = t.max_iter;
                 nr.t_dev0 = t.t_dev0; nr.t_dev1 = t.t_dev1; nr.patlnl = t.patlnl_dev;
-                nr.sync = nsync_buf + (size_t)in * NEWTON_SYNC_DOUBLES; newton_maxm = std::max(newton_maxm, mp);
+                nr.sync = nsync_buf + (sync_base + (size_t)in) * NEWTON_SYNC_DOUBLES; newton_maxm = std::max(newton_maxm, mp);
                 algo_bytes += (double)G.aln.npat * (L.bytes + R.bytes + 640);
                 algo_flops += (double)G.aln.npat * (6480 + L.flops + R.flops);
                 in++;
@@ -926,6 +995,17 @@
         }
         if (int rc = flush_tails(true)) return rc;
         run.op_end = (int)nout;
+        if (pass_step) {
+            if (part != 0 || run.op_end <= run.op_begin || !(hops[run.op_end - 1].flags & OPF_FUSED_NEWTON) || nbl + pass_build.size() > nreq_max)
+                return ctx->fail(-5, "internal: a pass step must end every gene's run in its fused Newton operation");
+            PassSeg &sg = hseg[nruns - 1];
+            sg.ops_off = (long long)(base + o_ops); sg.reqs_off = 0; sg.frags = frags_buf + frag_base * FRAG_STRIDE; sg.next_off = 0;
+            sg.build_off = (long long)(base + o_bl + nbl * sizeof(int));
+            sg.op_begin = run.op_begin; sg.op_end = run.op_end; sg.nbuild = (int)pass_build.size();
+            sg.step = deferred.empty() ? 0 : (int)(my_serial - deferred.front().serial);
+            for (int b : pass_build) hbl[nbl++] = b;
+            run_gene.push_back((int)g);
+        }
         static const int nt_policy = std::getenv("PML_NT_STORE") ? std::atoi(std::getenv("PML_NT_STORE")) : 1;
         const bool small_gene = mp <= 16 * TILE_PAT;
         for (int i = run.op_begin; i < run.op_end; ++i) {
@@ -964,7 +1044,13 @@
     L.nreq = ireq; L.nruns = nruns; L.neval = neval; L.nnewton = nnewton; L.max_mpad = max_mpad; L.newton_maxm = newton_maxm;
     L.any_pitch = any_pitch; L.any_chain = any_chain; L.algo_bytes = algo_bytes; L.algo_flops = algo_flops; L.newton_bytes = newton_bytes; L.lane = lane; L.stagger = record_stagger;
     record_stagger = false;
-    deferred.push_back(L);
+    L.pass = pass_step; L.serial = my_serial; L.frag_base = frag_base; L.o_seg = o_seg; L.run_gene = std::move(run_gene);
+    last_serial = my_serial;
+    if (pass_step) {
+        if (nt_reg + nt_stream > 0 || nruns != nnewton) return ctx->fail(-5, "internal: a pass step with an un-fused Newton request");
+        frag_off += ireq; nsync_off += nnewton;
+    }
+    deferred.push_back(std::move(L));
     const bool defer = chain && !lanes_active;
     if (!defer || deferred.size() >= flush_quota) { if (int rc = flush_deferred()) return rc; }
     ctx->tic_stream = nullptr;
@@ -1177,11 +1263,13 @@
     for (int attempt = 0; attempt < 2; ++attempt) {
     done.clear();
     if (!no_chain) { if (int rc = chain_begin(nres)) return rc; }
-    auto fail_out = [&](int rc) { if (chain) { chain_sync(); chain = false; } return rc; };
+    auto fail_out = [&](int rc) { if (chain) { chain_sync(); chain = false; } pass_allowed = false; return rc; };
     static const bool lanes_on = std::getenv("PML_LANES") != nullptr;
     int nact = 0; for (int g = 0; g < n; ++g) nact += active[g] && !order[g].empty();
     const bool two_lanes = chain && lanes_on && nact >= 16;
     lanes_active = two_lanes;
+    pass_allowed = chain && !two_lanes;
+    for (int g = 0; g < n; ++g) if (active[g] && !order[g].empty() && !newton_reg_form(genes[g].aln.mpad)) pass_allowed = false;
     for (size_t step = 0; step < maxlen; ++step) {
         ++cnt_smooth;
         const size_t first = done.size();
@@ -1216,6 +1304,7 @@
             for (size_t i = first; i < done.size(); ++i) {
                 Gene &G = genes[done[i].gene]; const int v = done[i].v, w = done[i].w;
                 G.len_pending[(size_t)v * 3 + G.tree.slot(v, w)] = 1; G.len_pending[(size_t)w * 3 + G.tree.slot(w, v)] = 1;
+                G.len_step[(size_t)v * 3 + G.tree.slot(v, w)] = last_serial; G.len_step[(size_t)w * 3 + G.tree.slot(w, v)] = last_serial;
                 branch_changed(done[i].gene, v, w);
             }
         } else {
@@ -1234,7 +1323,7 @@
         if (int rc = chain_sync()) { chain = false; return rc; }
         ctx->stats[K_HOST_WAIT].launches++; ctx->stats[K_HOST_WAIT].ms += now_ms() - t0;
         host_phase_ms[HP_PASS_SYNC] += now_ms() - t0; hp_t = now_ms();
-        chain = false; lanes_active = false;
+        chain = false; lanes_active = false; pass_allowed = false;
         bool gave_up = false;
         for (auto &d : done) gave_up = gave_up || !std::isfinite(h_chain[4 * d.idx + 1]);
         if (gave_up) {
diff --git a/pepr_amd/csrc/engine.hpp b/pepr_amd/csrc/engine.hpp
--- a/pepr_amd/csrc/engine.hpp
+++ b/pepr_amd/csrc/engine.hpp
@@ -68,6 +68,7 @@
     std::vector<uint8_t> dirty;
     double *d_len = nullptr;
     std::vector<uint8_t> len_pending;
+    std::vector<unsigned long long> len_step;
     void mark_node(int v) { for (int k = 0; k < 3; ++k) { const int w = tree.nbr[v][k]; if (w < 0) continue; dirty[v * 3 + k] = 1; dirty[w * 3 + tree.slot(w, v)] = 1; } }
     void mark_all() { dirty.assign((size_t)tree.nnodes() * 3, 1); }
     void mark_none() { dirty.assign((size_t)tree.nnodes() * 3, 0); }
@@ -148,8 +149,12 @@
     double *d_lenpool = nullptr;
     double *d_chain = nullptr, *h_chain = nullptr; size_t chain_cap = 0;
     struct Deferred { size_t base, bytes, o_req, o_ops, o_runs, o_red, o_newt, o_tick, nreq, nruns, neval, nnewton; int nt_reg, nt_stream; bool seq, fused;
-                      int max_mpad, newton_maxm, lane; bool any_pitch, any_chain, stagger; double algo_bytes, newton_bytes, algo_flops; };
+                      int max_mpad, newton_maxm, lane; bool any_pitch, any_chain, stagger; double algo_bytes, newton_bytes, algo_flops;
+                      bool pass = false; unsigned long long serial = 0; size_t frag_base = 0, o_seg = 0; std::vector<int> run_gene; };
     std::vector<Deferred> deferred; size_t flush_quota = 1; bool lanes_active = false;
+    size_t frag_off = 0, nsync_off = 0; unsigned long long step_serial = 0, last_serial = 0; bool pass_allowed = false;
+    std::vector<int> pass_build;
+    std::vector<PassSeg *> pass_last;
     int flush_deferred();
     int chain_begin(size_t nresults);
     int ensure_results(size_t nresults);
diff --git a/pepr_amd/csrc/kernels.h b/pepr_amd/csrc/kernels.h
--- a/pepr_amd/csrc/kernels.h
+++ b/pepr_amd/csrc/kernels.h
@@ -29,7 +29,7 @@
     double t;
     double rates[NCAT];
     int kind;
-    int pad;
+    int in_pass;
     const double *tp;
     const ModelDev *md;
 };
@@ -64,6 +64,19 @@
 struct GeneRun {
     int op_begin, op_end;
 };
+
+constexpr int PASS_MAX_STEPS = 32;
+struct PassSeg {
+    long long ops_off;
+    long long reqs_off;
+    double *frags;
+    long long next_off;
+    long long build_off;
+    int op_begin, op_end;
+    int nbuild;
+    int step;
+};
+static_assert(sizeof(PassSeg) == 56, "PassSeg layout");
 
 struct ReduceReq {
     const double *patlnl;
@@ -127,7 +140,8 @@
 void launch_pmat(const ModelDev *model, const PmatReq *reqs, double *frags, int n, hipStream_t s, bool per_request = false);
 void launch_eigfrags(const ModelDev *model, double *frags2, hipStream_t s);
 void launch_eigfrags_n(const ModelDev *models, double *frags2, int n, hipStream_t s);
-void launch_oplist(const NvOp *ops, const GeneRun *runs, int nruns, int max_mpad, bool any_pitch, bool chained, hipStream_t s, NewtonCtl *ctl = nullptr);
+void launch_oplist(const NvOp *ops, const GeneRun *runs, int nruns, int max_mpad, bool any_pitch, bool chained, hipStream_t s, NewtonCtl *ctl = nullptr,
+                   const long long *pass = nullptr);
 int fused_oplist_capacity();
 bool fuse_big_genes();
 void launch_reduce(const ReduceReq *reqs, int n, hipStream_t s);
diff --git a/pepr_amd/csrc/kernels.hip b/pepr_amd/csrc/kernels.hip
--- a/pepr_amd/csrc/kernels.hip
+++ b/pepr_amd/csrc/kernels.hip
@@ -37,6 +37,77 @@
 }
 
 constexpr int PMAT_THREADS = 256;
+struct PmatModel {
+    double Au[5][5], Bu[5][5];
+    double lam0, lam1, pi_row[5];
+};
+__device__ __forceinline__ void pmat_load_model(PmatModel &m, const ModelDev *__restrict__ md, int lane) {
+    const int i4 = lane & 3, k4 = lane >> 4;
+#pragma unroll
+    for (int a = 0; a < 5; ++a)
+#pragma unroll
+        for (int b = 0; b < 5; ++b) {
+            m.Au[a][b] = md->U[(4 * a + i4) * NS + 4 * b + k4];
+            m.Bu[a][b] = md->Uinv[(4 * a + k4) * NS + 4 * b + i4];
+        }
+    m.lam0 = md->eval[lane % NS]; m.lam1 = md->eval[(64 + (lane & 15)) % NS];
+#pragma unroll
+    for (int a = 0; a < 5; ++a) m.pi_row[a] = md->pi[4 * a + k4];
+}
+__device__ __forceinline__ void pmat_build(const PmatModel &m, double tlen, const double *__restrict__ rates, int kind,
+                                           double *sEw, double *__restrict__ out, int lane) {
+    const int i4 = lane & 3, k4 = lane >> 4, cb = (lane >> 2) & 3;
+    const int cat0 = lane / NS, cat1 = (64 + (lane & 15)) / NS;
+    sEw[lane] = exp(m.lam0 * (tlen * rates[cat0]));
+    if (lane < 16) sEw[64 + lane] = exp(m.lam1 * (tlen * rates[cat1]));
+    __builtin_amdgcn_fence(__ATOMIC_RELEASE, "wavefront");
+    __builtin_amdgcn_wave_barrier();
+    double ek[5];
+#pragma unroll
+    for (int kk = 0; kk < 5; ++kk) ek[kk] = sEw[cb * NS + 4 * kk + k4];
+    __builtin_amdgcn_wave_barrier();
+    double T[5][5];
+#pragma unroll
+    for (int st = 0; st < 5; ++st) {
+        double a[5];
+#pragma unroll
+        for (int kk = 0; kk < 5; ++kk) a[kk] = m.Au[st][kk] * ek[kk];
+#pragma unroll
+        for (int nt = 0; nt < 5; ++nt) {
+            double d = 0.0;
+#pragma unroll
+            for (int kk = 0; kk < 5; ++kk) d = mfma4(a[kk], m.Bu[kk][nt], d);
+            T[st][nt] = d < 0.0 ? 0.0 : d;
+        }
+    }
+    if (kind != PM_TIPTABLE) {
+#pragma unroll
+        for (int st = 0; st < 5; ++st) {
+            const double scale = kind == PM_FRAGS_PI ? m.pi_row[st] : 1.0;
+#pragma unroll
+            for (int nt = 0; nt < 5; ++nt)
+                out[((cb * 25 + st * 5 + nt) << 4) + (i4 << 2) + k4] = T[st][nt] * scale;
+        }
+    } else {
+        auto put = [&](int code, double v0, double v1, double v2, double v3, double v4) {
+            typedef double dv2 __attribute__((ext_vector_type(2)));
+            dv2 *rec = reinterpret_cast<dv2 *>(out + ((cb * NCODES + code) * 4 + k4) * TIPTAB_KK);
+            rec[0] = (dv2){v0, v1}; rec[1] = (dv2){v2, v3}; rec[2] = (dv2){v4, 0.0};
+        };
+#pragma unroll
+        for (int nt = 0; nt < 5; ++nt) put(4 * nt + i4, T[0][nt], T[1][nt], T[2][nt], T[3][nt], T[4][nt]);
+        double bz[5], zq[5], any[5];
+#pragma unroll
+        for (int st = 0; st < 5; ++st) {
+            bz[st] = T[st][0] + quad_swap<0xB1>(T[st][0]);
+            zq[st] = T[st][1] + quad_swap<0xD8>(T[st][1]);
+            any[st] = quad_sum(T[st][0] + T[st][1] + T[st][2] + T[st][3] + T[st][4]);
+        }
+        if (i4 == 2) put(20, bz[0], bz[1], bz[2], bz[3], bz[4]);
+        if (i4 == 1) put(21, zq[0], zq[1], zq[2], zq[3], zq[4]);
+        if (i4 == 0) put(22, any[0], any[1], any[2], any[3], any[4]);
+    }
+}
 template <bool PER_REQ>
 __global__ __launch_bounds__(PMAT_THREADS, 2) void k_pmat(const ModelDev *__restrict__ md0,
                                                           const PmatReq *__restrict__ reqs,
@@ -44,80 +115,15 @@
     __shared__ double sE[PMAT_THREADS / 64][NCAT * NS];
     const int lane = threadIdx.x & 63;
     const int wv = __builtin_amdgcn_readfirstlane(threadIdx.x >> 6);
-    const int i4 = lane & 3, k4 = lane >> 4, cb = (lane >> 2) & 3;
-    double Au[5][5], Bu[5][5];
-    double lam0, lam1, pi_row[5];
-    const int cat0 = lane / NS, cat1 = (64 + (lane & 15)) / NS;
-    auto load_model = [&](const ModelDev *__restrict__ md) {
-#pragma unroll
-        for (int a = 0; a < 5; ++a)
-#pragma unroll
-            for (int b = 0; b < 5; ++b) {
-                Au[a][b] = md->U[(4 * a + i4) * NS + 4 * b + k4];
-                Bu[a][b] = md->Uinv[(4 * a + k4) * NS + 4 * b + i4];
-            }
-        lam0 = md->eval[lane % NS]; lam1 = md->eval[(64 + (lane & 15)) % NS];
-#pragma unroll
-        for (int a = 0; a < 5; ++a) pi_row[a] = md->pi[4 * a + k4];
-    };
-    if (!PER_REQ) load_model(md0);
+    PmatModel m;
+    if (!PER_REQ) pmat_load_model(m, md0, lane);
     const int nwaves = gridDim.x * (PMAT_THREADS / 64);
     for (int rq = blockIdx.x * (PMAT_THREADS / 64) + wv; rq < n; rq += nwaves) {
         const PmatReq &req = reqs[rq];
-        if (PER_REQ) load_model(req.md);
+        if (req.in_pass != 0) continue;
+        if (PER_REQ) pmat_load_model(m, req.md, lane);
         const double tlen = req.tp ? *req.tp : req.t;
-        const int kind = req.kind;
-        double *sEw = sE[wv];
-        sEw[lane] = exp(lam0 * (tlen * req.rates[cat0]));
-        if (lane < 16) sEw[64 + lane] = exp(lam1 * (tlen * req.rates[cat1]));
-        __builtin_amdgcn_fence(__ATOMIC_RELEASE, "wavefront");
-        __builtin_amdgcn_wave_barrier();
-        double ek[5];
-#pragma unroll
-        for (int kk = 0; kk < 5; ++kk) ek[kk] = sEw[cb * NS + 4 * kk + k4];
-        __builtin_amdgcn_wave_barrier();
-        double *out = frags + (size_t)rq * FRAG_STRIDE;
-        double T[5][5];
-#pragma unroll
-        for (int st = 0; st < 5; ++st) {
-            double a[5];
-#pragma unroll
-            for (int kk = 0; kk < 5; ++kk) a[kk] = Au[st][kk] * ek[kk];
-#pragma unroll
-            for (int nt = 0; nt < 5; ++nt) {
-                double d = 0.0;
-#pragma unroll
-                for (int kk = 0; kk < 5; ++kk) d = mfma4(a[kk], Bu[kk][nt], d);
-                T[st][nt] = d < 0.0 ? 0.0 : d;
-            }
-        }
-        if (kind != PM_TIPTABLE) {
-#pragma unroll
-            for (int st = 0; st < 5; ++st) {
-                const double scale = kind == PM_FRAGS_PI ? pi_row[st] : 1.0;
-#pragma unroll
-                for (int nt = 0; nt < 5; ++nt)
-                    out[((cb * 25 + st * 5 + nt) << 4) + (i4 << 2) + k4] = T[st][nt] * scale;
-            }
-        } else {
-            auto put = [&](int code, double v0, double v1, double v2, double v3, double v4) {
-                typedef double dv2 __attribute__((ext_vector_type(2)));
-                dv2 *rec = reinterpret_cast<dv2 *>(out + ((cb * NCODES + code) * 4 + k4) * TIPTAB_KK);
-                rec[0] = (dv2){v0, v1}; rec[1] = (dv2){v2, v3}; rec[2] = (dv2){v4, 0.0};
-            };
-#pragma unroll
-            for (int nt = 0; nt < 5; ++nt) put(4 * nt + i4, T[0][nt], T[1][nt], T[2][nt], T[3][nt], T[4][nt]);
-            double bz[5], zq[5], any[5];
-#pragma unroll
-            for (int st = 0; st < 5; ++st) {
-                bz[st] = T[st][0] + quad_swap<0xB1>(T[st][0]);
-                zq[st] = T[st][1] + quad_swap<0xD8>(T[st][1]);
-                any[st] = quad_sum(T[st][0] + T[st][1] + T[st][2] + T[st][3] + T[st][4]);
-            }
-            if (i4 == 2) put(20, bz[0], bz[1], bz[2], bz[3], bz[4]);
-            if (i4 == 1) put(21, zq[0], zq[1], zq[2], zq[3], zq[4]);
-            if (i4 == 0) put(22, any[0], any[1], any[2], any[3], any[4]);
-        }
+        pmat_build(m, tlen, req.rates, req.kind, sE[wv], frags + (size_t)rq * FRAG_STRIDE, lane);
     }
 }
 
@@ -406,6 +412,12 @@
 #ifndef PML_TIPLOOK
 #define PML_TIPLOOK 1
 #endif
+template <class T>
+__device__ __forceinline__ T *uni_ptr(T *p) {
+    const unsigned long long v = (unsigned long long)p;
+    const unsigned lo = __builtin_amdgcn_readfirstlane((unsigned)v), hi = __builtin_amdgcn_readfirstlane((unsigned)(v >> 32));
+    return (T *)(((unsigned long long)hi << 32) | (unsigned long long)lo);
+}
 template <bool PREFETCH, bool CHAIN, bool FUSE>
 __device__ __forceinline__ void chunk_op(const NvOp &op, const double *__restrict__ sP, const unsigned char *__restrict__ sT,
                                          int p, int lane, Operand (&X)[4], ivec2 &xsc) {
@@ -427,7 +439,7 @@
     OpSide sdl = op.l, sdr = op.r;
     const int *l_scl = op.l_scl, *r_scl = op.r_scl; int *out_scl = op.out_scl; double *outp = op.out;
 #if PML_PIN_DESC
-#define PML_PIN(x) asm volatile("" : "+s"(x))
+#define PML_PIN(x) do { if constexpr (FUSE) x = uni_ptr(x); asm volatile("" : "+s"(x)); } while (0)
     PML_PIN(sdl.p0); PML_PIN(sdl.p1); PML_PIN(sdl.p2); PML_PIN(sdl.t0); PML_PIN(sdl.t1); PML_PIN(sdl.t2); PML_PIN(sdl.f);
     PML_PIN(sdr.p0); PML_PIN(sdr.p1); PML_PIN(sdr.p2); PML_PIN(sdr.t0); PML_PIN(sdr.t1); PML_PIN(sdr.t2); PML_PIN(sdr.f);
     PML_PIN(l_scl); PML_PIN(r_scl); PML_PIN(out_scl); PML_PIN(outp);
@@ -640,8 +652,8 @@
     double bc[4];
 };
 static_assert(sizeof(FusedShared) <= PFRAG * sizeof(double), "fused Newton scratch fits one fragment region");
-__device__ __forceinline__ void newton_fused(const NvOp &op, double *scratch, const Operand (&X)[4], const ivec2 xsc,
-                                             bool active, int blk, NewtonCtl *ctl, long long timeout_ticks) {
+__device__ __forceinline__ bool newton_fused(const NvOp &op, double *scratch, const Operand (&X)[4], const ivec2 xsc,
+                                             bool active, int blk, NewtonCtl *ctl, long long timeout_ticks, double &t_out) {
     const NewtonReq &r = *reinterpret_cast<const NewtonReq *>(op.aux);
     FusedShared &sh = *reinterpret_cast<FusedShared *>(scratch);
     const int tid = threadIdx.x, lane = tid & 63, wave = tid >> 6, q = lane >> 4, pl = wave * PAT_PER_WAVE + 2 * (lane & 15);
@@ -708,6 +720,13 @@
         r.out[0] = t; r.out[1] = L; r.out[2] = d1; r.out[3] = d2;
         if (r.t_dev0) { *r.t_dev0 = t; *r.t_dev1 = t; }
     }
+    t_out = t;
+    return ok;
+}
+
+__device__ __forceinline__ long long uni_off(long long v) {
+    const unsigned lo = __builtin_amdgcn_readfirstlane((unsigned)(u64)v), hi = __builtin_amdgcn_readfirstlane((unsigned)((u64)v >> 32));
+    return (long long)(((u64)hi << 32) | (u64)lo);
 }
 
 #ifdef PML_OPTIME
@@ -723,7 +742,7 @@
 template <int VARIANT>
 __global__ __launch_bounds__(256, (VARIANT == 1) ? 4 : (VARIANT >= 8) ? PML_CHAIN_WAVES : 3) void k_oplist(
         const NvOp *__restrict__ ops, const GeneRun *__restrict__ runs, int nruns, int blocks_per_gene, int any_pitch,
-        NewtonCtl *ctl, long long timeout_ticks) {
+        NewtonCtl *ctl, long long timeout_ticks, const long long *__restrict__ pass) {
 #ifdef PML_OPTIME
     const long long t_life0 = clock64();
 #endif
@@ -767,7 +786,12 @@
     };
     const int gi = one_part ? slot / blocks_per_gene : xcd + 8 * (slot / blocks_per_gene), blk = slot % blocks_per_gene;
     if (gi >= nruns) { leave(); return; }
-    const GeneRun run = runs[gi];
+    const bool passing = FUSE && pass != nullptr;
+    const char *const dbase = reinterpret_cast<const char *>(ops);
+    const PassSeg *seg = passing ? reinterpret_cast<const PassSeg *>(dbase + uni_off(pass[gi])) : nullptr;
+    GeneRun run;
+    if (passing) { ops = reinterpret_cast<const NvOp *>(dbase + seg->ops_off); run.op_begin = seg->op_begin; run.op_end = seg->op_end; }
+    else run = runs[gi];
     if (run.op_begin >= run.op_end) { leave(); return; }
     const int mpad = ops[run.op_begin].mpad;
     if (blk * PAT_PER_WG >= mpad) { leave(); return; }
@@ -778,11 +802,16 @@
     const long long t_start1 = clock64();
 #endif
     for (int i = tid; i < TIPTAB; i += 256) sT[i] = (unsigned char)((code_mask(i / NS) >> (i % NS)) & 1u);
+    __shared__ double s_tlen[FUSE ? PASS_MAX_STEPS : 1];
+#ifdef PML_OPTIME
+    long long t_start2 = 0, t_newton = 0, t_bar = 0, t_ops = 0;
+#endif
+    for (;;) {
     if (DBUF) { if (DBUF3) stage_frags_dma3(ops[run.op_begin], sP, lane, wave); else stage_frags_dma(ops[run.op_begin], sP, lane, wave); }
     __syncthreads();
+    bool gave_up = false;
 #ifdef PML_OPTIME
-    const long long t_start2 = clock64();
-    long long t_newton = 0, t_bar = 0, t_ops = 0;
+    if (t_start2 == 0) t_start2 = clock64();
 #endif
     for (int oi = run.op_begin; oi < run.op_end; ++oi) {
         const NvOp &op = ops[oi];
@@ -828,10 +857,15 @@
         const long long t_n0 = clock64();
 #endif
         if (FUSE && (op.flags & OPF_FUSED_NEWTON) != 0) {
-            if (__hip_atomic_load(&ctl->abort, __ATOMIC_RELAXED, __HIP_MEMORY_SCOPE_AGENT) != 0) {
+            if (__syncthreads_or(__hip_atomic_load(&ctl->abort, __ATOMIC_RELAXED, __HIP_MEMORY_SCOPE_AGENT) != 0)) {
                 const NewtonReq &r = *reinterpret_cast<const NewtonReq *>(op.aux);
                 if (tid == 0 && blk == 0) { r.out[0] = r.t0; r.out[1] = __builtin_nan(""); r.out[2] = 0.0; r.out[3] = 0.0; }
-            } else newton_fused(op, const_cast<double *>(buf), X, xsc, active, blk, ctl, timeout_ticks);
+                gave_up = true;
+            } else {
+                double t_new;
+                gave_up = !newton_fused(op, const_cast<double *>(buf), X, xsc, active, blk, ctl, timeout_ticks, t_new);
+                if (passing && tid == 0) s_tlen[seg->step] = t_new;
+            }
         }
 #ifdef PML_OPTIME
         const long long t_b0 = clock64(); t_newton += t_b0 - t_n0;
@@ -842,6 +876,37 @@
 #ifdef PML_OPTIME
         t_bar += clock64() - t_b0;
 #endif
+    }
+    if (!passing) break;
+    if (FUSE) {
+        if (__builtin_amdgcn_readfirstlane((int)gave_up)) {
+            if (tid == 0 && blk == 0)
+                for (long long o2 = seg->next_off; o2 != 0;) {
+                    const PassSeg *s2 = reinterpret_cast<const PassSeg *>(dbase + o2); o2 = s2->next_off;
+                    const NewtonReq &r = *reinterpret_cast<const NewtonReq *>(reinterpret_cast<const NvOp *>(dbase + s2->ops_off)[s2->op_end - 1].aux);
+                    r.out[0] = r.t0; r.out[1] = __builtin_nan(""); r.out[2] = 0.0; r.out[3] = 0.0;
+                }
+            break;
+        }
+        const long long nx = uni_off(seg->next_off);
+        if (nx == 0) break;
+        seg = reinterpret_cast<const PassSeg *>(dbase + nx);
+        ops = reinterpret_cast<const NvOp *>(dbase + seg->ops_off); run.op_begin = seg->op_begin; run.op_end = seg->op_end;
+        const int nb = seg->nbuild;
+        for (int b = __builtin_amdgcn_readfirstlane(wave); b < nb; b += 4) {
+            const int ri = reinterpret_cast<const int *>(dbase + seg->build_off)[b];
+            const PmatReq &req = reinterpret_cast<const PmatReq *>(dbase + seg->reqs_off)[ri];
+            PmatModel pm;
+            pmat_load_model(pm, req.md, lane);
+            pmat_build(pm, s_tlen[req.in_pass - 1], req.rates, req.kind, sP + __builtin_amdgcn_readfirstlane(wave) * (NCAT * NS), seg->frags + (size_t)ri * FRAG_STRIDE, lane);
+        }
+        xsc = (ivec2){0, 0};
+#pragma unroll
+        for (int c = 0; c < 4; ++c)
+#pragma unroll
+            for (int k = 0; k < 5; ++k) X[c].v[k] = (dvec2){0.0, 0.0};
+        __syncthreads();
+    }
     }
 #ifdef PML_OPTIME
     if (lane == 0 && active) {
@@ -1419,19 +1484,19 @@
     return v;
 }
 static long long newton_timeout_ticks();
-static void launch_oplist_one(const NvOp *ops, const GeneRun *runs, int nruns, int bpg, bool one_part, bool any_pitch, bool chained, hipStream_t s, NewtonCtl *ctl);
+static void launch_oplist_one(const NvOp *ops, const GeneRun *runs, int nruns, int bpg, bool one_part, bool any_pitch, bool chained, hipStream_t s, NewtonCtl *ctl, const long long *pass);
 int fused_oplist_capacity();
 bool fuse_big_genes();
-void launch_oplist(const NvOp *ops, const GeneRun *runs, int nruns, int max_mpad, bool any_pitch, bool chained, hipStream_t s, NewtonCtl *ctl) {
+void launch_oplist(const NvOp *ops, const GeneRun *runs, int nruns, int max_mpad, bool any_pitch, bool chained, hipStream_t s, NewtonCtl *ctl, const long long *pass) {
     if (nruns <= 0) return;
     const int bpg = (max_mpad + PAT_PER_WG - 1) / PAT_PER_WG;
-    if (!ctl) { launch_oplist_one(ops, runs, nruns, bpg, false, any_pitch, chained, s, nullptr); return; }
-    if (bpg <= 32) { launch_oplist_one(ops, runs, nruns, bpg, false, any_pitch, true, s, ctl); return; }
-    if (fuse_big_genes()) { launch_oplist_one(ops, runs, nruns, bpg, true, any_pitch, true, s, ctl); return; }
+    if (!ctl) { launch_oplist_one(ops, runs, nruns, bpg, false, any_pitch, chained, s, nullptr, nullptr); return; }
+    if (bpg <= 32) { launch_oplist_one(ops, runs, nruns, bpg, false, any_pitch, true, s, ctl, pass); return; }
+    if (fuse_big_genes()) { launch_oplist_one(ops, runs, nruns, bpg, true, any_pitch, true, s, ctl, pass); return; }
     const int cap = fused_oplist_capacity();
     const int genes_per_launch = std::max(1, cap / bpg);
     for (int off = 0; off < nruns; off += genes_per_launch)
-        launch_oplist_one(ops, runs + off, std::min(genes_per_launch, nruns - off), bpg, true, any_pitch, true, s, ctl);
+        launch_oplist_one(ops, pass ? runs : runs + off, std::min(genes_per_launch, nruns - off), bpg, true, any_pitch, true, s, ctl, pass ? pass + off : nullptr);
 }
 bool fuse_big_genes() {
     static const bool on = !(std::getenv("PML_FUSE_BIG") && std::atoi(std::getenv("PML_FUSE_BIG")) == 0);
@@ -1449,7 +1514,7 @@
     }();
     return cap;
 }
-static void launch_oplist_one(const NvOp *ops, const GeneRun *runs, int nruns, int bpg_in, bool one_part, bool any_pitch, bool chained, hipStream_t s, NewtonCtl *ctl) {
+static void launch_oplist_one(const NvOp *ops, const GeneRun *runs, int nruns, int bpg_in, bool one_part, bool any_pitch, bool chained, hipStream_t s, NewtonCtl *ctl, const long long *pass) {
     const long long to = newton_timeout_ticks();
     const int bpg = one_part ? -bpg_in : bpg_in;
     const dim3 grid((unsigned)(one_part ? nruns * bpg_in : ((nruns + 7) / 8) * 8 * bpg_in)), block(256);
@@ -1485,15 +1550,15 @@
     }
     const int ap = any_pitch ? 1 : 0;
     switch (v) {
-        case 0: hipLaunchKernelGGL(k_oplist<0>, grid, block, lds, s, ops, runs, nruns, bpg, ap, ctl, to); break;
-        case 2: hipLaunchKernelGGL(k_oplist<2>, grid, block, lds, s, ops, runs, nruns, bpg, ap, ctl, to); break;
-        case 3: hipLaunchKernelGGL(k_oplist<3>, grid, block, lds, s, ops, runs, nruns, bpg, ap, ctl, to); break;
-        case 5: hipLaunchKernelGGL(k_oplist<5>, grid, block, lds, s, ops, runs, nruns, bpg, ap, ctl, to); break;
-        case 9: hipLaunchKernelGGL(k_oplist<9>, grid, block, lds, s, ops, runs, nruns, bpg, ap, ctl, to); break;
-        case 10: hipLaunchKernelGGL(k_oplist<10>, grid, block, lds, s, ops, runs, nruns, bpg, ap, ctl, to); break;
-        case 11: hipLaunchKernelGGL(k_oplist<11>, grid, block, lds, s, ops, runs, nruns, bpg, ap, ctl, to); break;
-        case 15: hipLaunchKernelGGL(k_oplist<15>, grid, block, lds, s, ops, runs, nruns, bpg, ap, ctl, to); break;
-        default: hipLaunchKernelGGL(k_oplist<1>, grid, block, lds, s, ops, runs, nruns, bpg, ap, ctl, to); break;
+        case 0: hipLaunchKernelGGL(k_oplist<0>, grid, block, lds, s, ops, runs, nruns, bpg, ap, ctl, to, pass); break;
+        case 2: hipLaunchKernelGGL(k_oplist<2>, grid, block, lds, s, ops, runs, nruns, bpg, ap, ctl, to, pass); break;
+        case 3: hipLaunchKernelGGL(k_oplist<3>, grid, block, lds, s, ops, runs, nruns, bpg, ap, ctl, to, pass); break;
+        case 5: hipLaunchKernelGGL(k_oplist<5>, grid, block, lds, s, ops, runs, nruns, bpg, ap, ctl, to, pass); break;
+        case 9: hipLaunchKernelGGL(k_oplist<9>, grid, block, lds, s, ops, runs, nruns, bpg, ap, ctl, to, pass); break;
+        case 10: hipLaunchKernelGGL(k_oplist<10>, grid, block, lds, s, ops, runs, nruns, bpg, ap, ctl, to, pass); break;
+        case 11: hipLaunchKernelGGL(k_oplist<11>, grid, block, lds, s, ops, runs, nruns, bpg, ap, ctl, to, pass); break;
+        case 15: hipLaunchKernelGGL(k_oplist<15>, grid, block, lds, s, ops, runs, nruns, bpg, ap, ctl, to, pass); break;
+        default: hipLaunchKernelGGL(k_oplist<1>, grid, block, lds, s, ops, runs, nruns, bpg, ap, ctl, to, pass); break;
     }
 }
 void launch_reduce(const ReduceReq *reqs, int n, hipStream_t s) {
diff --git a/pepr_amd/csrc/parsimony.hip b/pepr_amd/csrc/parsimony.hip
--- a/pepr_amd/csrc/parsimony.hip
+++ b/pepr_amd/csrc/parsimony.hip
@@ -168,6 +168,7 @@
 
 int parsimony_batch(Ctx *ctx, int n, const pml_alignment_view *alns, unsigned seed, int radius,
                     std::vector<Tree> &trees_out, std::vector<EncodedAlignment> &alns_out, std::vector<long long> &lengths_out, std::vector<int> &moves_out) {
+    if (hipSetDevice(ctx->device) != hipSuccess) return ctx->fail(-5, "hipSetDevice failed");
     std::vector<PGene> G(n);
     Stage st{ctx}, sc{ctx};
     size_t total_blocks = 0;
```

Result: no change. 167.8, median of 6 (+0.0%).
